# AWehenkel/Graphical-Normalizing-Flows

Hardware: NVIDIA B200
Metric: train_samples_per_s (higher is better)
Workload: dtype f32

## Files before the change

graphical-normalizing-flows_b200/_lib.py:

```python
import ctypes as C
import os

import torch

_HERE = os.path.dirname(os.path.abspath(__file__))
LIB_NAME = "libgnf_sm100.so"
LIB_PATH = os.path.join(_HERE, LIB_NAME)

GNF_MAX_LAYERS = 8
GATE_TABLE, GATE_GUMBEL, GATE_NOISER = 0, 1, 2
IMP_RAW, IMP_SOFT, IMP_HARD_SOFT, IMP_HARD_SQ = 0, 1, 2, 3

_lib = None
_SIMULATOR = False


class GateT(C.Structure):
    _fields_ = [("mode", C.c_int32), ("temperature", C.c_float), ("seed", C.c_uint64), ("offset", C.c_uint64),
                ("noise1", C.c_void_p), ("noise2", C.c_void_p), ("offset_dev", C.c_void_p)]


class MlpT(C.Structure):
    _fields_ = [("n_layers", C.c_int32), ("dims", C.c_int32 * (GNF_MAX_LAYERS + 1)),
                ("W", C.c_void_p * GNF_MAX_LAYERS), ("b", C.c_void_p * GNF_MAX_LAYERS)]


class AdamTensorT(C.Structure):
    _fields_ = [("param", C.c_void_p), ("grad", C.c_void_p), ("exp_avg", C.c_void_p), ("exp_avg_sq", C.c_void_p),
                ("numel", C.c_int64)]


class MlpGradT(C.Structure):
    _fields_ = [("dW", C.c_void_p * GNF_MAX_LAYERS), ("db", C.c_void_p * GNF_MAX_LAYERS)]


_P, _I, _F, _SZ = C.c_void_p, C.c_int, C.c_float, C.c_size_t

_PROTOS = {
    "gnf_version": ([], C.c_int),
    "gnf_last_error": ([], C.c_char_p),
    "gnf_has_device_code": ([], C.c_int),
    "gnf_affine_fwd": ([_P, _P, _I, _P, _P, _P, _P, _P, _I, _I, _P], C.c_int),
    "gnf_affine_bwd": ([_P, _P, _I, _P, _P, _P, _P, _P, _P, _P, _I, _I, _P], C.c_int),
    "gnf_normal_ll_fwd": ([_P, _P, _P, _I, _I, _P], C.c_int),
    "gnf_normal_ll_bwd": ([_P, _P, _P, _I, _I, _P], C.c_int),
    "gnf_power_trace_workspace_bytes": ([_I], _SZ),
    "gnf_power_trace_fwd": ([_P, _I, _F, _I, _P, _P, _SZ, _P], C.c_int),
    "gnf_power_trace_bwd": ([_P, _I, _F, _I, _P, _P, _P, _SZ, _P], C.c_int),
    "gnf_power_trace_fwd_save": ([_P, _I, _F, _I, _P, _P, _P], C.c_int),
    "gnf_power_trace_bwd_saved": ([_P, _P, _I, _F, _I, _P, _P, _P], C.c_int),
    "gnf_linear_fwd": ([_P, _I, _P, _I, _P, _I, _P, _I, _I, _I, _I, _I, _P], C.c_int),
    "gnf_linear_dgrad": ([_P, _I, _P, _I, _P, _I, _P, _I, _I, _I, _I, _P], C.c_int),
    "gnf_linear_wgrad": ([_P, _I, _P, _I, _P, _I, _I, _I, _I, _P], C.c_int),
    "gnf_linear_fwd_tc": ([_P, _I, _P, _I, _P, _I, _P, _I, _I, _I, _I, _I, _I, _P], C.c_int),
    "gnf_linear_dgrad_tc": ([_P, _I, _P, _I, _P, _I, _P, _I, _I, _I, _I, _I, _P], C.c_int),
    "gnf_linear_wgrad_tc": ([_P, _I, _P, _I, _P, _I, _I, _I, _I, _I, _P], C.c_int),
    "gnf_linear_wgrad_bias_tc": ([_P, _I, _P, _I, _P, _I, _P, _I, _I, _I, _P], C.c_int),
    "gnf_split_tf32": ([_P, _I, _P, _P, _I, _I, _I, _P], C.c_int),
    "gnf_linear_fwd_tc_ps": ([_P, _I, _P, _P, _I, _P, _I, _P, _I, _I, _I, _I, _I, _P], C.c_int),
    "gnf_linear_dgrad_tc_ps": ([_P, _I, _P, _P, _I, _P, _I, _P, _I, _I, _I, _I, _P], C.c_int),
    "gnf_colsum": ([_P, _I, _P, _I, _I, _I, _P], C.c_int),
    "gnf_pack_rows": ([_P, _P, _P, _P, _I, _I, _P], C.c_int),
    "gnf_unpack_rows": ([_P, _P, _P, _P, _I, _I, _I, _P], C.c_int),
    "gnf_unpack_vec": ([_P, _P, _P, _I, _I, _P], C.c_int),
    "gnf_dag_importance": ([_P, _I, _I, _F, _P, _P, _P], C.c_int),
    "gnf_dag_bias_table": ([_P, _I, _P, _P, _I, _I, _I, _P], C.c_int),
    "gnf_dag_bias_table_bwd": ([_P, _P, _I, _P, _I, _I, _I, _P], C.c_int),
    "gnf_dag_l1_fwd": ([_P, _P, C.POINTER(GateT), _P, _I, _P, _I, _P, _I, _I, _I, _I, _I, _P], C.c_int),
    "gnf_dag_l1_wgrad": ([_P, _I, _P, _P, C.POINTER(GateT), _P, _I, _I, _I, _I, _P], C.c_int),
    "gnf_dag_l1_dgrad": ([_P, _I, _P, _I, _P, _P, C.POINTER(GateT), _P, _P, _I, _I, _I, _P], C.c_int),
    "gnf_dag_l1_fwd_save": ([_P, _P, C.POINTER(GateT), _P, _I, _P, _I, _P, _I, _P, _P, _P, _I, _I, _I, _I, _P], C.c_int),
    "gnf_dag_l1_wgrad_saved": ([_P, _I, _P, _P, _I, _I, _I, _I, _P], C.c_int),
    "gnf_dag_l1_dgrad_saved": ([_P, _I, _P, _I, _P, _P, _P, _P, _I, _I, _I, _P], C.c_int),
    "gnf_linear_fwd_splitk_workspace_bytes": ([_I, _I, _I], _SZ),
    "gnf_linear_fwd_splitk": ([_P, _I, _P, _I, _P, _P, _I, _I, _I, _I, _I, _P, _SZ, _P], C.c_int),
    "gnf_dag_bias_table_ld": ([_P, _I, _P, _P, _I, _I, _I, _I, _P], C.c_int),
    "gnf_linear_fwd_tc_ps_tb": ([_P, _I, _P, _P, _I, _P, _I, _I, _P, _I, _I, _I, _I, _I, _P], C.c_int),
    "gnf_dag_gate_planes": ([_P, _P, C.POINTER(GateT), _P, _P, _P, _I, _I, _P], C.c_int),
    "gnf_dag_l1_reduce_saved": ([_P, _P, _P, _P, _P, _I, _I, _P], C.c_int),
    "gnf_nll_loss_work_floats": ([_I], _SZ),
    "gnf_nll_loss_fwd": ([_P, _P, _P, _P, _P, _I, _I, _P], C.c_int),
    "gnf_nll_loss_bwd": ([_P, _P, _P, _P, _I, _I, _P], C.c_int),
    "gnf_peer_alloc": ([_SZ, C.POINTER(C.c_void_p)], C.c_int),
    "gnf_peer_free": ([_P], C.c_int),
    "gnf_peer_export": ([_P, C.c_char_p], C.c_int),
    "gnf_peer_import": ([C.c_char_p, C.POINTER(C.c_void_p)], C.c_int),
    "gnf_peer_close": ([_P], C.c_int),
    "gnf_peer_flag_bytes": ([], _SZ),
    "gnf_peer_allreduce_avg": ([C.POINTER(C.c_void_p), C.POINTER(C.c_void_p), _I, _I, C.c_longlong, _P], C.c_int),
    "gnf_dag_embed_fwd": ([_P, _P, C.POINTER(GateT), _P, _P, _P, _I, _I, _I, _P], C.c_int),
    "gnf_dag_embed_bwd": ([_P, _I, _P, _P, C.POINTER(GateT), _P, _P, _P, _P, _I, _I, _P], C.c_int),
    "gnf_dag_finish_dA": ([_P, _P, _P, _I, _I, _P], C.c_int),
    "gnf_dag_dump_noise": ([C.POINTER(GateT), _P, _P, _I, _I, _P], C.c_int),
    "gnf_umnn_workspace_bytes": ([C.POINTER(MlpT)], _SZ),
    "gnf_umnn_saved_floats_per_node_row": ([C.POINTER(MlpT)], _SZ),
    "gnf_umnn_fwd": ([_P, _P, C.POINTER(MlpT), _I, _P, _P, _P, _P, _P, _P, _P, _I, _I, _P, _SZ, _P], C.c_int),
    "gnf_umnn_invert": ([_P, _P, C.POINTER(MlpT), _I, _P, _P, _P, _I, _F, _F, _I, _P, _SZ, _P], C.c_int),
    "gnf_umnn_bwd": ([_P, _P, C.POINTER(MlpT), _I, _P, _P, _P, _P, _P, _P, _P, _P, _P, _P, C.POINTER(MlpGradT), _I, _I,
                      _P, _SZ, _P], C.c_int),
    "gnf_umnn_tc_workspace_bytes": ([C.POINTER(MlpT)], _SZ),
    "gnf_umnn_fwd_tc": ([_P, _P, C.POINTER(MlpT), _I, _P, _P, _P, _P, _P, _P, _I, _I, _P, _SZ, _P], C.c_int),
    "gnf_umnn_lw_saved_floats": ([C.POINTER(MlpT), _I, _I, _I], _SZ),
    "gnf_umnn_lw_workspace_bytes": ([C.POINTER(MlpT), _I, _I, _I], _SZ),
    "gnf_umnn_fwd_lw": ([_P, _P, C.POINTER(MlpT), _I, _P, _P, _P, _P, _P, _P, _P, _I, _I, _I, _I, _P, _SZ, _P], C.c_int),
    "gnf_umnn_bwd_lw": ([_P, _P, C.POINTER(MlpT), _I, _P, _P, _P, _P, _P, _P, _P, _P, _P, _P, C.POINTER(MlpGradT), _I, _I, _I,
                         _P, _SZ, _P], C.c_int),
    "gnf_umnn_tc3_workspace_bytes": ([C.POINTER(MlpT), _I], _SZ),
    "gnf_umnn_tc3_saved_floats": ([C.POINTER(MlpT), _I, _I], _SZ),
    "gnf_umnn_bwd_tc3_workspace_bytes": ([C.POINTER(MlpT), _I, _I], _SZ),
    "gnf_umnn_bwd_tc3": ([_P, _P, C.POINTER(MlpT), _I, _P, _P, _P, _P, _P, _P, _P, _P, _P, _P, C.POINTER(MlpGradT), _I, _I,
                          _P, _SZ, _P], C.c_int),
    "gnf_umnn_fwd_tc3": ([_P, _P, C.POINTER(MlpT), _I, _P, _P, _P, _P, _P, _P, _P, _I, _I, _I, _I, _P, _SZ, _P], C.c_int),
    "gnf_linear_rw_workspace_bytes": ([_I, _I], _SZ),
    "gnf_linear_wgrad_rw_workspace_bytes": ([_I, _I], _SZ),
    "gnf_linear_wgrad_rw": ([_P, _I, _P, _I, _P, _I, _I, _I, _I, _I, _P, _SZ, _P], C.c_int),
    "gnf_linear_fwd_rw": ([_P, _I, _P, _I, _P, _P, _I, _P, _I, _I, _I, _I, _I, _P, _SZ, _P], C.c_int),
    "gnf_linear_dgrad_rw": ([_P, _I, _P, _I, _P, _I, _P, _P, _I, _I, _I, _I, _I, _P, _SZ, _P], C.c_int),
    "gnf_tc_gemm_plan": ([_I, _I, _I, _I, _I, _P, _P], C.c_int),
    "gnf_tc_selftest": ([_P, _P, _P, _I, _I, _I, _P], C.c_int),
    "gnf_reverse_cols": ([_P, _P, _I, _I, _P], C.c_int),
    "gnf_broadcast_rows": ([_P, _P, _I, _I, _I, _I, _P], C.c_int),
    "gnf_counter_add": ([_P, C.c_uint64, _P], C.c_int),
    "gnf_adam_step": ([C.POINTER(AdamTensorT), _I, _P, _F, _F, _F, _F, _F, _P], C.c_int),
    "gnf_dag_loss_fwd": ([_P, _I, _P, _P, _P, _P, _P, _P, _P], C.c_int),
    "gnf_dag_loss_bwd": ([_P, _I, _P, _P, _P, _P, _P, _P, _P, _P, _P], C.c_int),
}

EXPORTED_SYMBOLS = tuple(_PROTOS)


def _bind(lib):
    for name, (argtypes, restype) in _PROTOS.items():
        fn = getattr(lib, name)
        fn.argtypes = argtypes
        fn.restype = restype
    return lib


def load_library(path=LIB_PATH):
    if not os.path.isfile(path):
        raise RuntimeError(
            f"{LIB_NAME} not found at {path}: the CUDA library is the only backend of this package "
            f"(no CPU / eager fallback). Build it with `python -c 'import __graft_entry__ as g; g.build()'`.")
    return _bind(C.CDLL(path))


def lib():
    global _lib
    if _lib is None:
        _lib = load_library()
    return _lib


def check(rc):
    if rc != 0:
        msg = lib().gnf_last_error()
        raise RuntimeError(f"libgnf error {rc}: {msg.decode() if msg else '?'}")


def stream_ptr():
    if _SIMULATOR:
        return None
    return C.c_void_p(torch.cuda.current_stream().cuda_stream)


def ptr(t):
    if t is None:
        return None
    return C.c_void_p(t.data_ptr())


def require(t, name, dtype=torch.float32):
    if not isinstance(t, torch.Tensor):
        raise TypeError(f"{name}: expected a torch.Tensor, got {type(t).__name__}")
    if t.dtype != dtype:
        raise TypeError(f"{name}: expected dtype {dtype}, got {t.dtype}")
    if not _SIMULATOR and not t.is_cuda:
        raise TypeError(f"{name}: expected a CUDA tensor (this package has no CPU path)")
    if not t.is_contiguous():
        raise TypeError(f"{name}: expected a contiguous tensor")
    return t
```

graphical-normalizing-flows_b200/csrc/tc_umnn3.cu:

```cuda
#include "tc_common.cuh"

#ifndef GNF_EMU
namespace gnf {

constexpr int kU3Rows = 128;
constexpr int kU3Stages = 4;
constexpr int kU3StageBlock = 32 * 16;
constexpr int kU3PRows = 12;
constexpr int kU3MaxNodes = 256;

__device__ __forceinline__ uint32_t u3_rn_tf32(uint32_t u) { return (u + 0x1000u) & 0xffffe000u; }
__device__ __forceinline__ void u3_arrive(uint64_t* bar) {
  asm volatile("mbarrier.arrive.shared::cta.b64 _, [%0];" ::"r"(tc::smem_u32(bar)) : "memory");
}

struct U3Plan {
  int L, NP, E, N1;
  int kp[GNF_MAX_LAYERS], nch[GNF_MAX_LAYERS];
  size_t off_img[GNF_MAX_LAYERS];
  size_t chunk_floats, off_tail, image_floats, off_P, total_floats;
};

static int u3_plan(const gnf_mlp_t* net, int R, U3Plan* pl) {
  if (!net || net->n_layers < 3 || net->n_layers > GNF_MAX_LAYERS) return fail(GNF_ERR_UNSUPPORTED, "umnn tc3: integrand needs 3..%d linear layers", GNF_MAX_LAYERS);
  if (net->dims[net->n_layers] != 1) return fail(GNF_ERR_UNSUPPORTED, "umnn tc3: integrand output size must be 1");
  if (net->dims[0] < 2) return fail(GNF_ERR_UNSUPPORTED, "umnn tc3: needs at least one conditioning feature");
  const int L = net->n_layers - 1;
  int maxh = 0;
  for (int l = 1; l <= L; ++l) maxh = net->dims[l] > maxh ? net->dims[l] : maxh;
  const int NP = (maxh + 31) / 32 * 32;
  if (NP > 160) return fail(GNF_ERR_UNSUPPORTED, "umnn tc3: hidden width %d > 160 (A_hi + A_lo + D must fit 512 TMEM columns)", maxh);
  pl->L = L; pl->NP = NP; pl->E = net->dims[0] - 1; pl->N1 = net->dims[1];
  pl->chunk_floats = (size_t)2 * 8 * NP * 4;
  size_t off = 0;
  for (int l = 0; l < GNF_MAX_LAYERS; ++l) { pl->kp[l] = 0; pl->nch[l] = 0; pl->off_img[l] = 0; }
  for (int l = 1; l < L; ++l) {
    pl->kp[l] = (net->dims[l] + 7) / 8 * 8;
    pl->nch[l] = (pl->kp[l] + 31) / 32;
    pl->off_img[l] = off;
    off += (size_t)pl->nch[l] * pl->chunk_floats;
  }
  pl->off_tail = off;
  off += (size_t)(L + 1) * NP;
  pl->image_floats = off;
  pl->off_P = (off + 3) / 4 * 4;
  pl->total_floats = pl->off_P + (size_t)(R > 0 ? R : 0) * NP;
  return 0;
}

struct U3PackArgs {
  const float* W[GNF_MAX_LAYERS];
  const float* b[GNF_MAX_LAYERS];
  int dims[GNF_MAX_LAYERS + 1], nch[GNF_MAX_LAYERS];
  unsigned off_img[GNF_MAX_LAYERS], chunk_floats, off_tail, total;
  int L, NP;
};

__global__ void u3_pack_kernel(U3PackArgs a, float* __restrict__ img) {
  for (unsigned i = blockIdx.x * blockDim.x + threadIdx.x; i < a.total; i += gridDim.x * blockDim.x) {
    float out = 0.f;
    if (i >= a.off_tail) {
      const int e = (int)(i - a.off_tail), j = e / a.NP, n = e % a.NP;
      if (j < a.L - 1) { if (n < a.dims[j + 2]) out = a.b[j + 1][n]; }
      else if (j == a.L - 1) { if (n < a.dims[a.L]) out = a.W[a.L][n]; }
      else { if (n < a.dims[1]) out = a.W[0][(size_t)n * a.dims[0]]; }
    } else {
      int l = 1;
      while (l + 1 < a.L && i >= a.off_img[l + 1]) ++l;
      const unsigned e = i - a.off_img[l];
      const unsigned c = e / a.chunk_floats, e2 = e % a.chunk_floats;
      const unsigned half = 8u * a.NP * 4u;
      const unsigned part = e2 / half, e3 = e2 % half;
      const int k4 = (int)(e3 / (a.NP * 4u)), n = (int)((e3 / 4u) % a.NP), kk = (int)(e3 % 4u);
      const int k = (int)c * 32 + k4 * 4 + kk;
      float v = 0.f;
      if (n < a.dims[l + 1] && k < a.dims[l]) v = a.W[l][(size_t)n * a.dims[l] + k];
      const float hi = __uint_as_float(u3_rn_tf32(__float_as_uint(v)));
      out = part ? __uint_as_float(u3_rn_tf32(__float_as_uint(v - hi))) : hi;
    }
    img[i] = out;
  }
}

struct U3Params {
  const float *x, *h, *ccw, *ccn, *P, *image, *blast;
  float *z, *zrev, *jac, *logdet, *saved;
  int R, d, E, S, nodes, L, N1, train, order, p_smem, debug;
  long long Q;
  int kp[GNF_MAX_LAYERS], nch[GNF_MAX_LAYERS];
  unsigned off_img[GNF_MAX_LAYERS], off_tail, chunk_floats;
  long long* trace;
};

#ifdef GNF_DEVTOOLS
#define U3_STAMP(row) do { if (tr_on && tr_n < 256) p.trace[(row) * 256 + tr_n++] = clock64(); } while (0)
#else
#define U3_STAMP(row) do { } while (0)
#endif

template <int NB>
__global__ void __launch_bounds__((4 * NB + 2) * 32, 1) umnn_fwd_tc3_kernel(U3Params p) {
  using namespace tc;
  constexpr int NP = NB * 32;
  constexpr int EW = 4 * NB;
  constexpr int NT = (EW + 2) * 32;
  constexpr uint32_t kChunkBytes = 2u * 8u * NP * 16u;
  constexpr uint32_t kHalfBytes = 8u * NP * 16u;
  GNF_SMEM(float, smem);
  float* ring = smem;
  float* tail = ring + (size_t)kU3Stages * (kChunkBytes / 4);
  float* stage_all = tail + (GNF_MAX_LAYERS + 1) * NP;
  float* pbuf = stage_all + EW * kU3StageBlock;
  float* ypart = pbuf + 2 * kU3PRows * NP;
  float* red = ypart + NB * kU3Rows;
  float* ccs = red + kU3Rows;
  uint64_t* bars = reinterpret_cast<uint64_t*>(ccs + 2 * kU3MaxNodes);
  uint64_t* w_full = bars;
  uint64_t* w_empty = w_full + kU3Stages;
  uint64_t* a_full = w_empty + kU3Stages;
  uint64_t* a_free = a_full + NB;
  uint64_t* d_full = a_free + NB;
  uint64_t* d_empty = d_full + 1;
  uint64_t* p_full = d_empty + 1;
  uint64_t* p_empty = p_full + 2;
  uint32_t* tmem_slot = reinterpret_cast<uint32_t*>(p_empty + 2);
  const int tid = threadIdx.x, warp = tid >> 5, lane = tid & 31;

  if (warp == 0) tmem_alloc(tmem_slot, 512);
  if (tid == 32) {
    for (int s = 0; s < kU3Stages; ++s) { mbar_init(&w_full[s], 1); mbar_init(&w_empty[s], 1); }
    for (int c = 0; c < NB; ++c) { mbar_init(&a_full[c], 4); mbar_init(&a_free[c], 1); }
    mbar_init(d_full, 1);
    mbar_init(d_empty, EW);
    for (int b = 0; b < 2; ++b) { mbar_init(&p_full[b], 1); mbar_init(&p_empty[b], EW); }
    fence_mbar_init();
  }
  pdl_prologue_done();
  for (int i = tid; i < (p.L + 1) * NP; i += NT) tail[i] = __ldg(p.image + p.off_tail + i);
  for (int i = tid; i <= p.S; i += NT) { ccs[i] = __ldg(p.ccn + i); ccs[kU3MaxNodes + i] = __ldg(p.ccw + i); }
  fence_before_sync();
  __syncthreads();
  fence_after_sync();
  const uint32_t tmem_base = *tmem_slot;

  const int Q = (int)p.Q, nodes = p.nodes;
  const int ntiles = (Q + kU3Rows - 1) / kU3Rows;
  const int n_local = (ntiles > (int)blockIdx.x) ? (ntiles - (int)blockIdx.x + (int)gridDim.x - 1) / (int)gridDim.x : 0;
  const int L = p.L;
#ifdef GNF_DEVTOOLS
  int tr_n = 0;
  const bool tr_on = p.trace != nullptr && blockIdx.x == 0 && lane == 0 && (warp == 0 || warp == 4 * (NB - 1) || warp >= EW);
#endif

  if (warp == EW + 1) {
    if (lane == 0) {
      auto issue_P = [&](int tl) {
        const int q0 = ((int)blockIdx.x + tl * (int)gridDim.x) * kU3Rows;
        const int q1 = (q0 + kU3Rows - 1 < Q - 1) ? q0 + kU3Rows - 1 : Q - 1;
        const int r0 = q0 / nodes, r1 = q1 / nodes;
        const uint32_t bytes = (uint32_t)(r1 - r0 + 1) * NP * 4u;
        const int b = tl & 1;
        if (tl >= 2) mbar_wait(&p_empty[b], (uint32_t)(((tl >> 1) - 1) & 1));
        mbar_expect_tx(&p_full[b], bytes);
        bulk_g2s(pbuf + (size_t)b * kU3PRows * NP, p.P + (size_t)r0 * NP, bytes, &p_full[b]);
      };
      if (p.p_smem && n_local > 0) issue_P(0);
      int g = 0;
      for (int tl = 0; tl < n_local; ++tl) {
        if (p.p_smem && tl + 1 < n_local) issue_P(tl + 1);
        for (int l = 1; l < L; ++l) {
          const int nch = p.nch[l], nseq = p.order ? 2 * nch : nch, nk = p.kp[l] / 8;
          const char* src0 = reinterpret_cast<const char*>(p.image + p.off_img[l]);
          for (int i = 0; i < nseq; ++i, ++g) {
            const int c = i < nch ? i : i - nch;
            const bool want_lo = !(p.order && i >= nch);
            const int ks = (nk - c * 4 < 4) ? nk - c * 4 : 4;
            const uint32_t bytes = (uint32_t)ks * 2u * NP * 16u;
            const int s = g % kU3Stages;
            if (g >= kU3Stages) mbar_wait(&w_empty[s], (uint32_t)(((g / kU3Stages) - 1) & 1));
            char* dst = reinterpret_cast<char*>(ring) + (size_t)s * kChunkBytes;
            const char* src = src0 + (size_t)c * kChunkBytes;
            mbar_expect_tx(&w_full[s], want_lo ? 2u * bytes : bytes);
            bulk_g2s(dst, src, bytes, &w_full[s]);
            if (want_lo) bulk_g2s(dst + kHalfBytes, src + kHalfBytes, bytes, &w_full[s]);
            U3_STAMP(2);
          }
        }
      }
    }
  } else if (warp == EW) {
    constexpr uint32_t idesc = make_idesc_tf32(kU3Rows, NP);
    constexpr uint32_t dstep = (2u * NP * 16u) >> 4;
    const uint32_t tAhi = tmem_base, tAlo = tmem_base + NP, tD = tmem_base + 2 * NP;
    const uint32_t ring_addr = smem_u32(ring);
    int g = 0, it = 0;
    for (int tl = 0; tl < n_local; ++tl)
      for (int l = 1; l < L; ++l, ++it) {
        const int nch = p.nch[l], nseq = p.order ? 2 * nch : nch, nk = p.kp[l] / 8;
        const bool release_a = (l == L - 1) && (tl + 1 < n_local);
        if (it > 0) mbar_wait(d_empty, (uint32_t)((it - 1) & 1));
        U3_STAMP(0);
        uint32_t acc = 0u;
        for (int i = 0; i < nseq; ++i, ++g) {
          const int c = i < nch ? i : i - nch;
          const int kind = p.order ? (i < nch ? 0 : 1) : 2;
          const int ks = (nk - c * 4 < 4) ? nk - c * 4 : 4;
          const int s = g % kU3Stages;
          if (i < nch) mbar_wait(&a_full[c], (uint32_t)(it & 1));
          mbar_wait(&w_full[s], (uint32_t)((g / kU3Stages) & 1));
          fence_after_sync();
          U3_STAMP(0);
          const uint32_t base = ring_addr + (uint32_t)s * kChunkBytes;
          const uint64_t dhi = make_smem_desc(base, NP * 16u, 128u), dlo = make_smem_desc(base + kHalfBytes, NP * 16u, 128u);
          const uint32_t a0 = (uint32_t)c * 32u;
          if (kind != 1) {
#pragma unroll 4
            for (int kk = 0; kk < ks; ++kk) { mma_tf32_ts_w(tD, tAlo + a0 + kk * 8, dhi + (uint64_t)(dstep * kk), idesc, acc); acc = 1u; }
#pragma unroll 4
            for (int kk = 0; kk < ks; ++kk) mma_tf32_ts_w(tD, tAhi + a0 + kk * 8, dlo + (uint64_t)(dstep * kk), idesc, 1u);
          }
          if (kind != 0) {
#pragma unroll 4
            for (int kk = 0; kk < ks; ++kk) { mma_tf32_ts_w(tD, tAhi + a0 + kk * 8, dhi + (uint64_t)(dstep * kk), idesc, acc); acc = 1u; }
          }
          mma_commit_w(&w_empty[s]);
          if (release_a && kind != 0) mma_commit_w(&a_free[c]);
        }
        if (release_a)
          for (int c = nch; c < NB; ++c) mma_commit_w(&a_free[c]);
        mma_commit_w(d_full);
        U3_STAMP(0);
      }
  } else {
    const int quarter = warp & 3, ci = warp >> 2, c = ci * 32;
    const int t = quarter * 32 + lane;
    const uint32_t lane_sel = (uint32_t)(quarter * 32) << 16;
    const uint32_t tAhi = tmem_base + lane_sel + c, tAlo = tAhi + NP, tD = tAhi + 2 * NP;
    float* stage = stage_all + warp * kU3StageBlock;
    const float* bias = tail + c;
    const float* wlast = tail + (L - 1) * NP + c;
    const float* w0col = tail + L * NP + c;
    const float blast = __ldg(p.blast);
    const size_t plane = (size_t)Q * NP;
    float* ysave = p.saved ? p.saved + (size_t)L * plane : nullptr;
    uint32_t* bits = (p.saved && p.train && L > 1) ? reinterpret_cast<uint32_t*>(p.saved + (size_t)L * plane + Q) : nullptr;
#ifdef GNF_DEVTOOLS
    if (p.debug & 4) { bits = nullptr; ysave = nullptr; }
#endif
    const bool full_block = c + 32 <= p.N1;

    struct Row { int q, r, kn, r_first; float xv; };
    auto row_of = [&](int tl) {
      Row w;
      const int q0 = ((int)blockIdx.x + tl * (int)gridDim.x) * kU3Rows;
      w.q = q0 + t;
      const int qc = w.q < Q ? w.q : Q - 1;
      w.r = qc / nodes; w.kn = qc - w.r * nodes;
      w.r_first = q0 / nodes;
      w.xv = ldg_pinned(p.x + w.r);
      return w;
    };
    auto store_block = [&](float* dstplane, const uint32_t* v, int q_row) {
#ifdef GNF_DEVTOOLS
      if (p.debug & 2) return;
#endif
      const int sub = lane >> 2, piece = lane & 3;
      const int row0 = q_row - lane + sub;
#pragma unroll
      for (int hb = 0; hb < 2; ++hb) {
#pragma unroll
        for (int j4 = 0; j4 < 4; ++j4)
          *reinterpret_cast<uint4*>(stage + lane * 16 + 4 * (j4 ^ ((lane >> 1) & 3))) =
              make_uint4(v[16 * hb + 4 * j4], v[16 * hb + 4 * j4 + 1], v[16 * hb + 4 * j4 + 2], v[16 * hb + 4 * j4 + 3]);
        __syncwarp();
#pragma unroll
        for (int i = 0; i < 4; ++i) {
          const int Rr = 8 * i + sub;
          const uint4 o = *reinterpret_cast<const uint4*>(stage + Rr * 16 + 4 * (piece ^ ((Rr >> 1) & 3)));
#ifdef GNF_DEVTOOLS
          if (p.debug & 1) continue;
#endif
          if (row0 + 8 * i < Q) *reinterpret_cast<uint4*>(dstplane + (size_t)(row0 + 8 * i) * NP + c + 16 * hb + 4 * piece) = o;
        }
        __syncwarp();
      }
    };
    auto split_store = [&](const uint32_t* v) {
#pragma unroll
      for (int hb = 0; hb < 2; ++hb) {
        uint32_t hi[16], lo[16];
#pragma unroll
        for (int j = 0; j < 16; ++j) {
          hi[j] = u3_rn_tf32(v[16 * hb + j]);
          lo[j] = __float_as_uint(__uint_as_float(v[16 * hb + j]) - __uint_as_float(hi[j])) + 0x1000u;
        }
        tmem_st16p(tAhi + 16 * hb, hi);
        tmem_st16p(tAlo + 16 * hb, lo);
      }
    };
    auto mask_word = [&](const uint32_t* v) {
      uint32_t w = 0u;
#pragma unroll
      for (int j = 0; j < 32; ++j) w |= (v[j] != 0u ? 1u : 0u) << j;
      return w;
    };
    auto gen_a1 = [&](int tl, const Row& w) {
      const float tq = (w.kn <= p.S) ? (w.xv * (ccs[w.kn] + 1.f)) / 2.f : w.xv;
      const float* Prow;
      if (p.p_smem) {
        mbar_wait(&p_full[tl & 1], (uint32_t)((tl >> 1) & 1));
        Prow = pbuf + (size_t)(tl & 1) * kU3PRows * NP + (size_t)(w.r - w.r_first) * NP + c;
      } else {
        Prow = p.P + (size_t)w.r * NP + c;
      }
      uint32_t v[32];
#pragma unroll
      for (int j4 = 0; j4 < 8; ++j4) {
        const float4 pv = p.p_smem ? *reinterpret_cast<const float4*>(Prow + 4 * j4) : __ldg(reinterpret_cast<const float4*>(Prow + 4 * j4));
        const float4 w4 = *reinterpret_cast<const float4*>(w0col + 4 * j4);
        v[4 * j4 + 0] = __float_as_uint(fmaxf(fmaf(tq, w4.x, pv.x), 0.f));
        v[4 * j4 + 1] = __float_as_uint(fmaxf(fmaf(tq, w4.y, pv.y), 0.f));
        v[4 * j4 + 2] = __float_as_uint(fmaxf(fmaf(tq, w4.z, pv.z), 0.f));
        v[4 * j4 + 3] = __float_as_uint(fmaxf(fmaf(tq, w4.w, pv.w), 0.f));
      }
      if (!full_block) {
#pragma unroll
        for (int j = 0; j < 32; ++j) v[j] = (c + j < p.N1) ? v[j] : 0u;
      }
      split_store(v);
      tmem_wait_st();
      fence_before_sync();
      __syncwarp();
      if (lane == 0) {
        u3_arrive(&a_full[ci]);
        if (p.p_smem) u3_arrive(&p_empty[tl & 1]);
      }
      if (bits && w.q < Q) bits[(size_t)w.q * NB + ci] = mask_word(v);
      if (p.saved) store_block(p.saved, v, w.q);
    };

    Row cur = {0, 0, 0, 0, 0.f};
    if (n_local > 0) { cur = row_of(0); gen_a1(0, cur); }
    int it = 0;
    for (int tl = 0; tl < n_local; ++tl) {
      for (int l = 1; l < L; ++l, ++it) {
        const float* bl = bias + (l - 1) * NP;
        Row nxt = cur;
        const bool gen_next = (l == L - 1) && (tl + 1 < n_local);
        const bool gen_late = gen_next && ci >= p.nch[l] - 1;
        if (gen_next) nxt = row_of(tl + 1);
        if (gen_next && !gen_late) {
          mbar_wait(&a_free[ci], (uint32_t)(tl & 1));
          fence_after_sync();
          gen_a1(tl + 1, nxt);
        }
        mbar_wait(d_full, (uint32_t)(it & 1));
        fence_after_sync();
        U3_STAMP(warp == 0 ? 1 : 3);
        uint32_t v[32];
        tmem_ld32p(tD, v);
        tmem_wait_ld();
        fence_before_sync();
        __syncwarp();
        if (lane == 0) u3_arrive(d_empty);
        if (gen_late) {
          mbar_wait(&a_free[ci], (uint32_t)(tl & 1));
          fence_after_sync();
          gen_a1(tl + 1, nxt);
        }
        if (l < L - 1) {
#pragma unroll
          for (int j4 = 0; j4 < 32; j4 += 4) {
            const float4 b4 = *reinterpret_cast<const float4*>(bl + j4);
            v[j4 + 0] = __float_as_uint(fmaxf(__uint_as_float(v[j4 + 0]) + b4.x, 0.f));
            v[j4 + 1] = __float_as_uint(fmaxf(__uint_as_float(v[j4 + 1]) + b4.y, 0.f));
            v[j4 + 2] = __float_as_uint(fmaxf(__uint_as_float(v[j4 + 2]) + b4.z, 0.f));
            v[j4 + 3] = __float_as_uint(fmaxf(__uint_as_float(v[j4 + 3]) + b4.w, 0.f));
          }
          split_store(v);
          tmem_wait_st();
          fence_before_sync();
          __syncwarp();
          if (lane == 0) u3_arrive(&a_full[ci]);
          U3_STAMP(warp == 0 ? 1 : 3);
          if (bits && cur.q < Q) bits[(size_t)l * Q * NB + (size_t)cur.q * NB + ci] = mask_word(v);
          if (p.saved) store_block(p.saved + (size_t)l * plane, v, cur.q);
        } else {
          float y0 = 0.f, y1 = 0.f, y2 = 0.f, y3 = 0.f;
#pragma unroll
          for (int j4 = 0; j4 < 32; j4 += 4) {
            const float4 b4 = *reinterpret_cast<const float4*>(bl + j4);
            const float4 w4 = *reinterpret_cast<const float4*>(wlast + j4);
            const float a0 = fmaxf(__uint_as_float(v[j4 + 0]) + b4.x, 0.f), a1 = fmaxf(__uint_as_float(v[j4 + 1]) + b4.y, 0.f);
            const float a2 = fmaxf(__uint_as_float(v[j4 + 2]) + b4.z, 0.f), a3 = fmaxf(__uint_as_float(v[j4 + 3]) + b4.w, 0.f);
            y0 = fmaf(a0, w4.x, y0); y1 = fmaf(a1, w4.y, y1); y2 = fmaf(a2, w4.z, y2); y3 = fmaf(a3, w4.w, y3);
            v[j4 + 0] = __float_as_uint(a0); v[j4 + 1] = __float_as_uint(a1); v[j4 + 2] = __float_as_uint(a2); v[j4 + 3] = __float_as_uint(a3);
          }
          ypart[ci * kU3Rows + t] = (y0 + y1) + (y2 + y3);
          if (bits && cur.q < Q) bits[(size_t)l * Q * NB + (size_t)cur.q * NB + ci] = mask_word(v);
          if (p.saved) store_block(p.saved + (size_t)l * plane, v, cur.q);
          named_bar_sync(1, EW * 32);
          const bool cur_valid = cur.q < Q;
          if (ci == 0) {
            float y = blast;
#pragma unroll
            for (int k = 0; k < NB; ++k) y += ypart[k * kU3Rows + t];
            const float f = (y > 0.f ? y : expm1f(y)) + 1.05f;
            float wv = 0.f;
            if (cur_valid) {
              if (ysave) ysave[cur.q] = y;
              if (cur.kn <= p.S) wv = ccs[kU3MaxNodes + cur.kn] * f;
              if (cur.kn == 0) {
                p.jac[cur.r] = f;
                if (p.logdet) atomicAdd(p.logdet + cur.r / p.d, logf(f));
              }
            }
            red[t] = wv;
          }
          named_bar_sync(1, EW * 32);
          if (ci == 0 && cur_valid && (cur.kn == 0 || t == 0)) {
            float sacc = 0.f;
            int rem = nodes - cur.kn;
            if (rem > kU3Rows - t) rem = kU3Rows - t;
            for (int k = 0; k < rem; ++k) sacc += red[t + k];
            float cz = sacc * cur.xv / 2.f;
            if (cur.kn == 0) cz += __ldg(p.h + (size_t)cur.r * p.E);
            atomicAdd(p.z + cur.r, cz);
            if (p.zrev) { const int b = cur.r / p.d, ii = cur.r % p.d; atomicAdd(p.zrev + (size_t)b * p.d + (p.d - 1 - ii), cz); }
          }
          U3_STAMP(warp == 0 ? 1 : 3);
        }
        cur = nxt;
      }
    }
  }
  fence_before_sync();
  __syncthreads();
  if (warp == 0) tmem_dealloc(tmem_base, 512);
}

struct U3BParams {
  const float *x, *ccw, *ccn, *jac, *gz, *gzrev, *gjac, *glogdet, *image, *saved;
  float* dplanes;
  float *D, *dx, *dW0;
  float* db[GNF_MAX_LAYERS];
  int R, d, E, S, nodes, L, ldw0;
  long long Q;
  int dims[GNF_MAX_LAYERS + 1];
  int kp[GNF_MAX_LAYERS], nch[GNF_MAX_LAYERS];
  unsigned off_img[GNF_MAX_LAYERS], off_tail, chunk_floats;
};

__device__ __forceinline__ float u3_colsum16(float (&w)[16], int lane) {
#pragma unroll
  for (int i = 0; i < 16; ++i) w[i] += __shfl_xor_sync(0xffffffffu, w[i], 16);
#pragma unroll
  for (int o = 8; o >= 1; o >>= 1) {
    const bool up = (lane & o) != 0;
#pragma unroll
    for (int i = 0; i < o; ++i) {
      const float send = up ? w[i] : w[i + o];
      const float keep = up ? w[i + o] : w[i];
      w[i] = keep + __shfl_xor_sync(0xffffffffu, send, o);
    }
  }
  return w[0];
}

template <int NB>
__global__ void __launch_bounds__((4 * NB + 2) * 32, 1) umnn_bwd_tc3_kernel(U3BParams p) {
  using namespace tc;
  constexpr int NP = NB * 32;
  constexpr int EW = 4 * NB;
  constexpr int NT = (EW + 2) * 32;
  constexpr uint32_t kChunkBytes = 2u * 8u * NP * 16u;
  constexpr uint32_t kHalfBytes = 8u * NP * 16u;
  GNF_SMEM(float, smem);
  float* ring = smem;
  float* tail = ring + (size_t)kU3Stages * (kChunkBytes / 4);
  float* stage_all = tail + 2 * NP;
  float* ccs = stage_all + EW * kU3StageBlock;
  uint64_t* bars = reinterpret_cast<uint64_t*>(ccs + 2 * kU3MaxNodes);
  uint64_t* w_full = bars;
  uint64_t* w_empty = w_full + kU3Stages;
  uint64_t* a_full = w_empty + kU3Stages;
  uint64_t* a_free = a_full + NB;
  uint64_t* d_full = a_free + NB;
  uint64_t* d_empty = d_full + 1;
  uint32_t* tmem_slot = reinterpret_cast<uint32_t*>(d_empty + 1);
  const int tid = threadIdx.x, warp = tid >> 5, lane = tid & 31;

  if (warp == 0) tmem_alloc(tmem_slot, 512);
  if (tid == 32) {
    for (int s = 0; s < kU3Stages; ++s) { mbar_init(&w_full[s], 1); mbar_init(&w_empty[s], 1); }
    for (int c = 0; c < NB; ++c) { mbar_init(&a_full[c], 4); mbar_init(&a_free[c], 1); }
    mbar_init(d_full, 1);
    mbar_init(d_empty, EW);
    fence_mbar_init();
  }
  pdl_prologue_done();
  for (int i = tid; i < 2 * NP; i += NT) tail[i] = __ldg(p.image + p.off_tail + i);
  for (int i = tid; i <= p.S; i += NT) { ccs[i] = __ldg(p.ccn + i); ccs[kU3MaxNodes + i] = __ldg(p.ccw + i); }
  fence_before_sync();
  __syncthreads();
  fence_after_sync();
  const uint32_t tmem_base = *tmem_slot;

  const int Q = (int)p.Q, nodes = p.nodes;
  const int ntiles = (Q + kU3Rows - 1) / kU3Rows;
  const int n_local = (ntiles > (int)blockIdx.x) ? (ntiles - (int)blockIdx.x + (int)gridDim.x - 1) / (int)gridDim.x : 0;
  const int L = p.L;

  if (warp == EW + 1) {
    if (lane == 0) {
      int g = 0;
      for (int tl = 0; tl < n_local; ++tl)
        for (int l = L - 1; l >= 1; --l) {
          const int nch = p.nch[l], nk = p.kp[l] / 8;
          const char* src0 = reinterpret_cast<const char*>(p.image + p.off_img[l]);
          for (int i = 0; i < 2 * nch; ++i, ++g) {
            const int c = i < nch ? i : i - nch;
            const bool want_lo = i < nch;
            const int ks = (nk - c * 4 < 4) ? nk - c * 4 : 4;
            const uint32_t bytes = (uint32_t)ks * 2u * NP * 16u;
            const int s = g % kU3Stages;
            if (g >= kU3Stages) mbar_wait(&w_empty[s], (uint32_t)(((g / kU3Stages) - 1) & 1));
            char* dst = reinterpret_cast<char*>(ring) + (size_t)s * kChunkBytes;
            const char* src = src0 + (size_t)c * kChunkBytes;
            mbar_expect_tx(&w_full[s], want_lo ? 2u * bytes : bytes);
            bulk_g2s(dst, src, bytes, &w_full[s]);
            if (want_lo) bulk_g2s(dst + kHalfBytes, src + kHalfBytes, bytes, &w_full[s]);
          }
        }
    }
  } else if (warp == EW) {
    constexpr uint32_t idesc = make_idesc_tf32(kU3Rows, NP);
    constexpr uint32_t dstep = (2u * NP * 16u) >> 4;
    const uint32_t tAhi = tmem_base, tAlo = tmem_base + NP, tD = tmem_base + 2 * NP;
    const uint32_t ring_addr = smem_u32(ring);
    int g = 0, it = 0;
    for (int tl = 0; tl < n_local; ++tl)
      for (int l = L - 1; l >= 1; --l, ++it) {
        const int nch = p.nch[l], nk = p.kp[l] / 8;
        const bool release_a = (l == 1) && (tl + 1 < n_local);
        if (it > 0) mbar_wait(d_empty, (uint32_t)((it - 1) & 1));
        uint32_t acc = 0u;
        for (int i = 0; i < 2 * nch; ++i, ++g) {
          const int c = i < nch ? i : i - nch;
          const bool corr = i < nch;
          const int ks = (nk - c * 4 < 4) ? nk - c * 4 : 4;
          const int s = g % kU3Stages;
          if (corr) mbar_wait(&a_full[c], (uint32_t)(it & 1));
          mbar_wait(&w_full[s], (uint32_t)((g / kU3Stages) & 1));
          fence_after_sync();
          const uint32_t base = ring_addr + (uint32_t)s * kChunkBytes;
          const uint64_t dhi = make_smem_desc(base, NP * 16u, 128u), dlo = make_smem_desc(base + kHalfBytes, NP * 16u, 128u);
          const uint32_t a0 = (uint32_t)c * 32u;
          if (corr) {
#pragma unroll 4
            for (int kk = 0; kk < ks; ++kk) { mma_tf32_ts_w(tD, tAlo + a0 + kk * 8, dhi + (uint64_t)(dstep * kk), idesc, acc); acc = 1u; }
#pragma unroll 4
            for (int kk = 0; kk < ks; ++kk) mma_tf32_ts_w(tD, tAhi + a0 + kk * 8, dlo + (uint64_t)(dstep * kk), idesc, 1u);
          } else {
#pragma unroll 4
            for (int kk = 0; kk < ks; ++kk) mma_tf32_ts_w(tD, tAhi + a0 + kk * 8, dhi + (uint64_t)(dstep * kk), idesc, 1u);
          }
          mma_commit_w(&w_empty[s]);
          if (release_a && !corr) mma_commit_w(&a_free[c]);
        }
        if (release_a)
          for (int c = nch; c < NB; ++c) mma_commit_w(&a_free[c]);
        mma_commit_w(d_full);
      }
  } else {
    const int quarter = warp & 3, ci = warp >> 2, c = ci * 32;
    const int t = quarter * 32 + lane;
    const uint32_t lane_sel = (uint32_t)(quarter * 32) << 16;
    const uint32_t tAhi = tmem_base + lane_sel + c, tAlo = tAhi + NP, tD = tAhi + 2 * NP;
    float* stage = stage_all + warp * kU3StageBlock;
    const float* wL = tail + c;
    const float* w0col = tail + NP + c;
    const size_t plane = (size_t)Q * NP;
    const float* ysave = p.saved + (size_t)L * plane;
    const uint32_t* bits = reinterpret_cast<const uint32_t*>(p.saved + (size_t)L * plane + Q);
    const size_t bplane = (size_t)Q * NB;

    struct Row { int q, r, kn; float gq, tq, jg; uint32_t mtop; };
    auto row_of = [&](int tl) {
      Row w;
      const int q0 = ((int)blockIdx.x + tl * (int)gridDim.x) * kU3Rows;
      w.q = q0 + t;
      const bool valid = w.q < Q;
      const int qc = valid ? w.q : Q - 1;
      w.r = qc / nodes; w.kn = qc - w.r * nodes;
      const int r = w.r;
      const float xv = ldg_pinned(p.x + r);
      float gzt = p.gz ? ldg_pinned(p.gz + r) : 0.f;
      if (p.gzrev) { const int b = r / p.d, i = r - b * p.d; gzt += ldg_pinned(p.gzrev + (size_t)b * p.d + (p.d - 1 - i)); }
      const float y = ldg_pinned(ysave + qc);
      float gq;
      if (w.kn <= p.S) {
        gq = (gzt * xv / 2.f) * ccs[kU3MaxNodes + w.kn];
        w.tq = (xv * (ccs[w.kn] + 1.f)) / 2.f;
      } else {
        gq = p.gjac ? ldg_pinned(p.gjac + r) : 0.f;
        if (p.glogdet) gq += ldg_pinned(p.glogdet + r / p.d) / ldg_pinned(p.jac + r);
        w.tq = xv;
      }
      gq *= (y > 0.f) ? 1.f : expf(y);
      w.gq = valid ? gq : 0.f;
      w.jg = ldg_pinned(p.jac + r) * gzt;
      w.mtop = valid ? __ldg(bits + (size_t)(L - 1) * bplane + (size_t)qc * NB + ci) : 0u;
      return w;
    };
    auto store_block = [&](float* dstplane, const uint32_t* v, int q_row) {
      const int sub = lane >> 2, piece = lane & 3;
      const int row0 = q_row - lane + sub;
#pragma unroll
      for (int hb = 0; hb < 2; ++hb) {
#pragma unroll
        for (int j4 = 0; j4 < 4; ++j4)
          *reinterpret_cast<uint4*>(stage + lane * 16 + 4 * (j4 ^ ((lane >> 1) & 3))) =
              make_uint4(v[16 * hb + 4 * j4], v[16 * hb + 4 * j4 + 1], v[16 * hb + 4 * j4 + 2], v[16 * hb + 4 * j4 + 3]);
        __syncwarp();
#pragma unroll
        for (int i = 0; i < 4; ++i) {
          const int Rr = 8 * i + sub;
          const uint4 o = *reinterpret_cast<const uint4*>(stage + Rr * 16 + 4 * (piece ^ ((Rr >> 1) & 3)));
          if (row0 + 8 * i < Q) *reinterpret_cast<uint4*>(dstplane + (size_t)(row0 + 8 * i) * NP + c + 16 * hb + 4 * piece) = o;
        }
        __syncwarp();
      }
    };
    auto split_store = [&](const uint32_t* v) {
#pragma unroll
      for (int hb = 0; hb < 2; ++hb) {
        uint32_t hi[16], lo[16];
#pragma unroll
        for (int j = 0; j < 16; ++j) {
          hi[j] = u3_rn_tf32(v[16 * hb + j]);
          lo[j] = __float_as_uint(__uint_as_float(v[16 * hb + j]) - __uint_as_float(hi[j])) + 0x1000u;
        }
        tmem_st16p(tAhi + 16 * hb, hi);
        tmem_st16p(tAlo + 16 * hb, lo);
      }
    };
    auto gen_top = [&](const Row& w) {
      uint32_t v[32];
#pragma unroll
      for (int j4 = 0; j4 < 8; ++j4) {
        const float4 w4 = *reinterpret_cast<const float4*>(wL + 4 * j4);
        v[4 * j4 + 0] = ((w.mtop >> (4 * j4 + 0)) & 1u) ? __float_as_uint(w.gq * w4.x) : 0u;
        v[4 * j4 + 1] = ((w.mtop >> (4 * j4 + 1)) & 1u) ? __float_as_uint(w.gq * w4.y) : 0u;
        v[4 * j4 + 2] = ((w.mtop >> (4 * j4 + 2)) & 1u) ? __float_as_uint(w.gq * w4.z) : 0u;
        v[4 * j4 + 3] = ((w.mtop >> (4 * j4 + 3)) & 1u) ? __float_as_uint(w.gq * w4.w) : 0u;
      }
      split_store(v);
      tmem_wait_st();
      fence_before_sync();
      __syncwarp();
      if (lane == 0) u3_arrive(&a_full[ci]);
    };

    Row cur;
    cur.q = 0; cur.r = 0; cur.kn = 0; cur.gq = 0.f; cur.tq = 0.f; cur.jg = 0.f; cur.mtop = 0u;
    if (n_local > 0) { cur = row_of(0); gen_top(cur); }
    int it = 0;
    for (int tl = 0; tl < n_local; ++tl) {
      for (int l = L - 1; l >= 1; --l, ++it) {
        Row nxt = cur;
        const bool gen_next = (l == 1) && (tl + 1 < n_local);
        const bool gen_late = gen_next && ci >= p.nch[l] - 1;
        const bool valid = cur.q < Q;
        const uint32_t m = valid ? __ldg(bits + (size_t)(l - 1) * bplane + (size_t)cur.q * NB + ci) : 0u;
        if (gen_next) nxt = row_of(tl + 1);
        if (gen_next && !gen_late) {
          mbar_wait(&a_free[ci], (uint32_t)(tl & 1));
          fence_after_sync();
          gen_top(nxt);
        }
        mbar_wait(d_full, (uint32_t)(it & 1));
        fence_after_sync();
        uint32_t v[32];
        tmem_ld32p(tD, v);
        tmem_wait_ld();
        fence_before_sync();
        __syncwarp();
        if (lane == 0) u3_arrive(d_empty);
        if (gen_late) {
          mbar_wait(&a_free[ci], (uint32_t)(tl & 1));
          fence_after_sync();
          gen_top(nxt);
        }
#pragma unroll
        for (int j = 0; j < 32; ++j) v[j] = ((m >> j) & 1u) ? v[j] : 0u;
        if (l > 1) {
          split_store(v);
          tmem_wait_st();
          fence_before_sync();
          __syncwarp();
          if (lane == 0) u3_arrive(&a_full[ci]);
#pragma unroll
          for (int hb = 0; hb < 2; ++hb) {
            float w16[16];
#pragma unroll
            for (int j = 0; j < 16; ++j) w16[j] = __uint_as_float(v[16 * hb + j]);
            const float sum = u3_colsum16(w16, lane);
            const int n = c + 16 * hb + (lane & 15);
            if (lane < 16 && n < p.dims[l]) atomicAdd(p.db[l - 1] + n, sum);
          }
          store_block(p.dplanes + (size_t)(L - 1 - l) * plane, v, cur.q);
        } else {
          float dot = 0.f;
#pragma unroll
          for (int j4 = 0; j4 < 8; ++j4) {
            const float4 w4 = *reinterpret_cast<const float4*>(w0col + 4 * j4);
            dot = fmaf(__uint_as_float(v[4 * j4 + 0]), w4.x, dot); dot = fmaf(__uint_as_float(v[4 * j4 + 1]), w4.y, dot);
            dot = fmaf(__uint_as_float(v[4 * j4 + 2]), w4.z, dot); dot = fmaf(__uint_as_float(v[4 * j4 + 3]), w4.w, dot);
          }
          if (valid && cur.kn == p.S + 1) atomicAdd(p.dx + cur.r, dot + (ci == 0 ? cur.jg : 0.f));
          const int r_lo = __shfl_sync(0xffffffffu, cur.r, 0), r_hi = __shfl_sync(0xffffffffu, cur.r, 31);
#pragma unroll
          for (int hb = 0; hb < 2; ++hb) {
            const int n = c + 16 * hb + (lane & 15);
            const bool col_ok = lane < 16 && n < p.dims[1];
            float w16[16];
#pragma unroll
            for (int j = 0; j < 16; ++j) w16[j] = __uint_as_float(v[16 * hb + j]) * cur.tq;
            const float st = u3_colsum16(w16, lane);
            if (col_ok) atomicAdd(p.dW0 + (size_t)n * p.ldw0, st);
            for (int rr = r_lo; rr <= r_hi; ++rr) {
#pragma unroll
              for (int j = 0; j < 16; ++j) w16[j] = (cur.r == rr) ? __uint_as_float(v[16 * hb + j]) : 0.f;
              const float sd = u3_colsum16(w16, lane);
              if (col_ok) atomicAdd(p.D + (size_t)rr * NP + n, sd);
            }
          }
        }
        cur = nxt;
      }
    }
  }
  fence_before_sync();
  __syncthreads();
  if (warp == 0) tmem_dealloc(tmem_base, 512);
}

static size_t u3b_smem_bytes(int NP) {
  const int NB = NP / 32, EW = 4 * NB;
  return ((size_t)kU3Stages * 2 * 8 * NP * 4 + (size_t)2 * NP + (size_t)EW * kU3StageBlock + 2 * kU3MaxNodes) * sizeof(float) +
         (2 * kU3Stages + 2 * NB + 2) * sizeof(uint64_t) + 16;
}

struct U3BPlan {
  int L, NP;
  int kp[GNF_MAX_LAYERS], nch[GNF_MAX_LAYERS];
  size_t off_img[GNF_MAX_LAYERS], chunk_floats, off_tail, image_floats;
};
static int u3b_plan(const gnf_mlp_t* net, U3BPlan* pl) {
  U3Plan f;
  if (int e = u3_plan(net, 0, &f)) return e;
  pl->L = f.L; pl->NP = f.NP; pl->chunk_floats = f.chunk_floats;
  size_t off = 0;
  for (int l = 0; l < GNF_MAX_LAYERS; ++l) { pl->kp[l] = 0; pl->nch[l] = 0; pl->off_img[l] = 0; }
  for (int l = 1; l < f.L; ++l) {
    pl->kp[l] = (net->dims[l + 1] + 7) / 8 * 8;
    pl->nch[l] = (pl->kp[l] + 31) / 32;
    pl->off_img[l] = off;
    off += (size_t)pl->nch[l] * pl->chunk_floats;
  }
  pl->off_tail = off;
  pl->image_floats = off + (size_t)2 * f.NP;
  return 0;
}

__global__ void u3_pack_bwd_kernel(U3PackArgs a, float* __restrict__ img) {
  for (unsigned i = blockIdx.x * blockDim.x + threadIdx.x; i < a.total; i += gridDim.x * blockDim.x) {
    float out = 0.f;
    if (i >= a.off_tail) {
      const int e = (int)(i - a.off_tail), j = e / a.NP, n = e % a.NP;
      if (j == 0) { if (n < a.dims[a.L]) out = a.W[a.L][n]; }
      else { if (n < a.dims[1]) out = a.W[0][(size_t)n * a.dims[0]]; }
    } else {
      int l = 1;
      while (l + 1 < a.L && i >= a.off_img[l + 1]) ++l;
      const unsigned e = i - a.off_img[l];
      const unsigned c = e / a.chunk_floats, e2 = e % a.chunk_floats;
      const unsigned half = 8u * a.NP * 4u;
      const unsigned part = e2 / half, e3 = e2 % half;
      const int k4 = (int)(e3 / (a.NP * 4u)), n = (int)((e3 / 4u) % a.NP), kk = (int)(e3 % 4u);
      const int k = (int)c * 32 + k4 * 4 + kk;
      float v = 0.f;
      if (n < a.dims[l] && k < a.dims[l + 1]) v = a.W[l][(size_t)k * a.dims[l] + n];
      const float hi = __uint_as_float(u3_rn_tf32(__float_as_uint(v)));
      out = part ? __uint_as_float(u3_rn_tf32(__float_as_uint(v - hi))) : hi;
    }
    img[i] = out;
  }
}

size_t u3_bwd_image_floats(const gnf_mlp_t* net) {
  U3BPlan pl;
  if (u3b_plan(net, &pl)) return 0;
  return (pl.image_floats + 3) / 4 * 4;
}

int launch_u3_bwd_chain(const float* x, const gnf_mlp_t* net, int S, const float* ccw, const float* ccn, const float* jac, const float* gz,
                        const float* gzrev, const float* gjac, const float* glogdet, const float* saved, float* image, float* dplanes, float* D,
                        float* dx, const gnf_mlp_grad_t* grads, int R, int d, cudaStream_t s, const Branches* br, int side, cudaStream_t pack_stream) {
  U3BPlan pl;
  if (int e = u3b_plan(net, &pl)) return e;
  const int NP = pl.NP, L = pl.L;
  const int nodes = S + 2;
  const long long Q = (long long)R * nodes;
  if (Q > 0x7fffffffLL - 2 * kU3Rows || S + 1 > kU3MaxNodes) return fail(GNF_ERR_UNSUPPORTED, "umnn tc3 backward: problem size out of range");
  U3PackArgs a;
  for (int l = 0; l < GNF_MAX_LAYERS; ++l) { a.W[l] = nullptr; a.b[l] = nullptr; a.nch[l] = pl.nch[l]; a.off_img[l] = (unsigned)pl.off_img[l]; }
  for (int l = 0; l <= L; ++l) { a.W[l] = net->W[l]; a.b[l] = net->b[l]; }
  for (int l = 0; l <= net->n_layers; ++l) a.dims[l] = net->dims[l];
  a.chunk_floats = (unsigned)pl.chunk_floats; a.off_tail = (unsigned)pl.off_tail; a.total = (unsigned)pl.image_floats; a.L = L; a.NP = NP;
  int blocks = (int)((pl.image_floats + 255) / 256);
  if (blocks > 2 * kNumSMs) blocks = 2 * kNumSMs;
  GNF_LAUNCH(u3_pack_bwd_kernel, blocks, 256, 0, (br && pack_stream) ? pack_stream : s, a, image);
  if (br && pack_stream) br->end(s, side);
  U3BParams p;
  p.x = x; p.ccw = ccw; p.ccn = ccn; p.jac = jac; p.gz = gz; p.gzrev = gzrev; p.gjac = gjac; p.glogdet = glogdet; p.image = image; p.saved = saved;
  p.dplanes = dplanes; p.D = D; p.dx = dx; p.dW0 = grads->dW[0]; p.ldw0 = net->dims[0];
  for (int l = 0; l < GNF_MAX_LAYERS; ++l) p.db[l] = grads->db[l];
  p.R = R; p.d = d; p.E = net->dims[0] - 1; p.S = S; p.nodes = nodes; p.L = L; p.Q = Q;
  for (int l = 0; l <= GNF_MAX_LAYERS; ++l) p.dims[l] = l <= net->n_layers ? net->dims[l] : 0;
  for (int l = 0; l < GNF_MAX_LAYERS; ++l) { p.kp[l] = pl.kp[l]; p.nch[l] = pl.nch[l]; p.off_img[l] = (unsigned)pl.off_img[l]; }
  p.off_tail = (unsigned)pl.off_tail; p.chunk_floats = (unsigned)pl.chunk_floats;
  const size_t smem = u3b_smem_bytes(NP);
  const long long ntiles = (Q + kU3Rows - 1) / kU3Rows;
  const int grid = (int)(ntiles < kNumSMs ? ntiles : kNumSMs);
#define U3B_CASE(nb)                                                                                             \
  case nb:                                                                                                       \
    cudaFuncSetAttribute(umnn_bwd_tc3_kernel<nb>, cudaFuncAttributeMaxDynamicSharedMemorySize, (int)smem);       \
    GNF_LAUNCH_PDL(umnn_bwd_tc3_kernel<nb>, grid, (4 * nb + 2) * 32, smem, s, p);                                    \
    break;
  switch (NP / 32) { U3B_CASE(1) U3B_CASE(2) U3B_CASE(3) U3B_CASE(4) U3B_CASE(5) default: return fail(GNF_ERR_UNSUPPORTED, "umnn tc3 backward: width"); }
#undef U3B_CASE
  return 0;
}

static size_t u3_smem_bytes(int NP) {
  const int NB = NP / 32, EW = 4 * NB;
  return ((size_t)kU3Stages * 2 * 8 * NP * 4 + (size_t)(GNF_MAX_LAYERS + 1) * NP + (size_t)EW * kU3StageBlock + (size_t)2 * kU3PRows * NP +
          (size_t)(NB + 1) * kU3Rows + 2 * kU3MaxNodes) * sizeof(float) + (2 * kU3Stages + 2 * NB + 6) * sizeof(uint64_t) + 16;
}

#ifdef GNF_DEVTOOLS
static long long* g_u3_trace = nullptr;
static int g_u3_debug = 0;
#endif

}
using namespace gnf;
#endif

extern "C" {

size_t gnf_umnn_tc3_workspace_bytes(const gnf_mlp_t* net, int R) {
#ifdef GNF_EMU
  (void)net; (void)R;
  gnf::set_error("tensor-core kernels have no host-simulator flavour");
  return 0;
#else
  U3Plan pl;
  if (u3_plan(net, R, &pl)) return 0;
  return pl.total_floats * sizeof(float);
#endif
}

int gnf_umnn_fwd_tc3(const float* x, const float* h, const gnf_mlp_t* net, int S, const float* ccw, const float* ccn, float* z,
                     float* zrev, float* jac, float* logdet, float* saved, int train, int order, int R, int d, void* work,
                     size_t work_bytes, gnf_stream_t stream) {
#ifdef GNF_EMU
  return gnf::fail(GNF_ERR_UNSUPPORTED, "tensor-core kernels have no host-simulator flavour");
#else
  if (!x || !h || !net || !ccw || !ccn || !z || !jac || R < 0 || d <= 0 || S < 1 || (R % d) != 0) return fail(GNF_ERR_INVALID, "gnf_umnn_fwd_tc3: bad arguments");
  if (train && !saved) return fail(GNF_ERR_INVALID, "gnf_umnn_fwd_tc3: training needs the saved-activation buffer");
  U3Plan pl;
  if (int e = u3_plan(net, R, &pl)) return e;
  if (!work || work_bytes < pl.total_floats * sizeof(float)) return fail(GNF_ERR_WORKSPACE, "gnf_umnn_fwd_tc3: workspace too small (%zu < %zu)", work_bytes, pl.total_floats * sizeof(float));
  if ((reinterpret_cast<uintptr_t>(work) & 15) != 0 || (saved && (reinterpret_cast<uintptr_t>(saved) & 15) != 0)) return fail(GNF_ERR_INVALID, "gnf_umnn_fwd_tc3: workspace / saved must be 16-byte aligned");
  const int nodes = S + 1 + (train ? 1 : 0);
  const long long Q = (long long)R * nodes;
  if (Q > 0x7fffffffLL - 2 * kU3Rows) return fail(GNF_ERR_UNSUPPORTED, "gnf_umnn_fwd_tc3: %lld node-rows exceed the index range", Q);
  if (S + 1 > kU3MaxNodes) return fail(GNF_ERR_UNSUPPORTED, "gnf_umnn_fwd_tc3: more than %d quadrature nodes", kU3MaxNodes);
  cudaStream_t s = (cudaStream_t)stream;
  if (R == 0) return 0;
  float* ws = (float*)work;
  const int NP = pl.NP, L = pl.L, E = pl.E;
  U3PackArgs a;
  for (int l = 0; l < GNF_MAX_LAYERS; ++l) { a.W[l] = nullptr; a.b[l] = nullptr; a.nch[l] = pl.nch[l]; a.off_img[l] = (unsigned)pl.off_img[l]; }
  for (int l = 0; l <= L; ++l) { a.W[l] = net->W[l]; a.b[l] = net->b[l]; }
  for (int l = 0; l <= net->n_layers; ++l) a.dims[l] = net->dims[l];
  a.chunk_floats = (unsigned)pl.chunk_floats; a.off_tail = (unsigned)pl.off_tail; a.total = (unsigned)pl.image_floats; a.L = L; a.NP = NP;
  int blocks = (int)((pl.image_floats + 255) / 256);
  if (blocks > 2 * kNumSMs) blocks = 2 * kNumSMs;
  const Branches& br = branches();
  cudaStream_t s0 = br.begin(s, 0);
  GNF_LAUNCH(u3_pack_kernel, blocks, 256, 0, s0, a, ws);
  ZeroList zl;
  zl.add(z, (size_t)R);
  zl.add(zrev, (size_t)R);
  zl.add(logdet, (size_t)(R / d));
  zero_many(zl, s0);
  float* P = ws + pl.off_P;
  if (int e = gnf_linear_fwd(h, E, net->W[0] + 1, 1 + E, net->b[0], 1, P, NP, R, net->dims[1], E, 0, stream)) return e;
  br.end(s, 0);
  U3Params p;
  p.x = x; p.h = h; p.ccw = ccw; p.ccn = ccn; p.P = P; p.image = ws; p.blast = net->b[L];
  p.z = z; p.zrev = zrev; p.jac = jac; p.logdet = logdet; p.saved = saved;
  p.R = R; p.d = d; p.E = E; p.S = S; p.nodes = nodes; p.L = L; p.N1 = pl.N1; p.train = train; p.order = order ? 1 : 0;
  p.Q = Q;
  p.p_smem = ((kU3Rows - 1) / nodes + 2 <= kU3PRows) ? 1 : 0;
  for (int l = 0; l < GNF_MAX_LAYERS; ++l) { p.kp[l] = pl.kp[l]; p.nch[l] = pl.nch[l]; p.off_img[l] = (unsigned)pl.off_img[l]; }
  p.off_tail = (unsigned)pl.off_tail; p.chunk_floats = (unsigned)pl.chunk_floats;
#ifdef GNF_DEVTOOLS
  p.trace = g_u3_trace; p.debug = g_u3_debug;
#else
  p.trace = nullptr; p.debug = 0;
#endif
  const size_t smem = u3_smem_bytes(NP);
  const long long ntiles = (Q + kU3Rows - 1) / kU3Rows;
  const int grid = (int)(ntiles < kNumSMs ? ntiles : kNumSMs);
#define U3_CASE(nb)                                                                                              \
  case nb:                                                                                                       \
    cudaFuncSetAttribute(umnn_fwd_tc3_kernel<nb>, cudaFuncAttributeMaxDynamicSharedMemorySize, (int)smem);       \
    GNF_LAUNCH_PDL(umnn_fwd_tc3_kernel<nb>, grid, (4 * nb + 2) * 32, smem, s, p);                                           \
    break;
  switch (NP / 32) { U3_CASE(1) U3_CASE(2) U3_CASE(3) U3_CASE(4) U3_CASE(5) default: return fail(GNF_ERR_UNSUPPORTED, "gnf_umnn_fwd_tc3: width"); }
#undef U3_CASE
  return check_launch("gnf_umnn_fwd_tc3");
#endif
}

#ifdef GNF_DEVTOOLS
int gnf_umnn_tc3_set_trace(long long* buf) {
#ifndef GNF_EMU
  gnf::g_u3_trace = buf;
#else
  (void)buf;
#endif
  return 0;
}
int gnf_umnn_tc3_set_debug(int bits) {
#ifndef GNF_EMU
  gnf::g_u3_debug = bits;
#else
  (void)bits;
#endif
  return 0;
}
#endif

}
```

graphical-normalizing-flows_b200/csrc/tc_umnn3.h:

```cpp
#pragma once
#include "common.cuh"

#ifndef GNF_EMU
namespace gnf {
size_t u3_bwd_image_floats(const gnf_mlp_t* net);
int launch_u3_bwd_chain(const float* x, const gnf_mlp_t* net, int S, const float* ccw, const float* ccn, const float* jac, const float* gz,
                        const float* gzrev, const float* gjac, const float* glogdet, const float* saved, float* image, float* dplanes, float* D,
                        float* dx, const gnf_mlp_grad_t* grads, int R, int d, cudaStream_t s, const Branches* br = nullptr, int side = 0,
                        cudaStream_t pack_stream = nullptr);
}
#endif
```

graphical-normalizing-flows_b200/csrc/umnn_lw.cu:

```cuda
#include "common.cuh"
#include "tc_gemm.h"
#include "tc_rw.h"
#include "tc_umnn3.h"

namespace gnf {

constexpr int kLwRL = 8;
constexpr int kOutBwdU = 3;

struct LwGeom {
  int R, d, E, S, nodes, NP, L;
  long long Q;
};

__device__ __forceinline__ float lw_node_abscissa(float xv, const float* __restrict__ ccn, int kn, int S) {
  return (kn <= S) ? (xv * (__ldg(ccn + kn) + 1.f)) / 2.f : xv;
}

__global__ void lw_pad_weight_kernel(const float* __restrict__ W, int N, int K, float* __restrict__ Wp, int NP, int rows) {
  const int total = rows * NP;
  for (int i = blockIdx.x * blockDim.x + threadIdx.x; i < total; i += gridDim.x * blockDim.x) {
    const int n = i / NP, k = i % NP;
    Wp[i] = (n < N && k < K) ? W[(size_t)n * K + k] : 0.f;
  }
}

__global__ void lw_layer1_fwd_kernel(const float* __restrict__ x, const float* __restrict__ ccn, const float* __restrict__ P,
                                     const float* __restrict__ W0, int ldw0, int N1, float* __restrict__ a1,
                                     uint32_t* __restrict__ bits, LwGeom g) {
  const int C4 = g.NP / 4;
  const int c4 = threadIdx.x % C4, rl = threadIdx.x / C4, c = 4 * c4;
  float w[4];
#pragma unroll
  for (int e = 0; e < 4; ++e) w[e] = (c + e < N1) ? __ldg(W0 + (size_t)(c + e) * ldw0) : 0.f;
  const int Q = (int)g.Q;
  for (int q0 = blockIdx.x * kLwRL; q0 < Q; q0 += gridDim.x * kLwRL) {
    const int q = q0 + rl;
    const bool valid = q < Q;
    float4 o = make_float4(0.f, 0.f, 0.f, 0.f);
    if (valid) {
      const int r = q / g.nodes, kn = q - r * g.nodes;
      const float t = lw_node_abscissa(__ldg(x + r), ccn, kn, g.S);
      const float4 pv = __ldg(reinterpret_cast<const float4*>(P + (size_t)r * g.NP + c));
      o.x = (c + 0 < N1) ? fmaxf(fmaf(t, w[0], pv.x), 0.f) : 0.f;
      o.y = (c + 1 < N1) ? fmaxf(fmaf(t, w[1], pv.y), 0.f) : 0.f;
      o.z = (c + 2 < N1) ? fmaxf(fmaf(t, w[2], pv.z), 0.f) : 0.f;
      o.w = (c + 3 < N1) ? fmaxf(fmaf(t, w[3], pv.w), 0.f) : 0.f;
      *reinterpret_cast<float4*>(a1 + (size_t)q * g.NP + c) = o;
    }
    if (bits) {
      uint32_t wv = ((o.x > 0.f ? 1u : 0u) | (o.y > 0.f ? 2u : 0u) | (o.z > 0.f ? 4u : 0u) | (o.w > 0.f ? 8u : 0u)) << (4 * (threadIdx.x & 7));
      wv |= __shfl_xor_sync(0xffffffffu, wv, 1);
      wv |= __shfl_xor_sync(0xffffffffu, wv, 2);
      wv |= __shfl_xor_sync(0xffffffffu, wv, 4);
      if (valid && (threadIdx.x & 7) == 0) bits[(size_t)q * (g.NP / 32) + (c >> 5)] = wv;
    }
  }
}

template <int J>
__global__ void __launch_bounds__(256, 4) lw_out_fwd_kernel(const float* __restrict__ aL, const float* __restrict__ wl, const float* __restrict__ bl,
                                                             int NL, const float* __restrict__ x, const float* __restrict__ h,
                                                             const float* __restrict__ ccw, float* __restrict__ z, float* __restrict__ zrev,
                                                             float* __restrict__ jac, float* __restrict__ logdet, float* __restrict__ ysave,
                                                             LwGeom g) {
  const int lane = threadIdx.x & 31, grp = lane >> 3, sub = lane & 7;
  float4 w[J];
#pragma unroll
  for (int j = 0; j < J; ++j) {
    const int c = (j * 8 + sub) * 4;
    w[j].x = (c + 0 < NL) ? __ldg(wl + c + 0) : 0.f;
    w[j].y = (c + 1 < NL) ? __ldg(wl + c + 1) : 0.f;
    w[j].z = (c + 2 < NL) ? __ldg(wl + c + 2) : 0.f;
    w[j].w = (c + 3 < NL) ? __ldg(wl + c + 3) : 0.f;
  }
  const float blast = __ldg(bl);
  const int wpb = blockDim.x >> 5;
  for (int r = blockIdx.x * wpb + (threadIdx.x >> 5); r < g.R; r += gridDim.x * wpb) {
    const float xv = __ldg(x + r);
    float s = 0.f;
    for (int kn0 = 0; kn0 < g.nodes; kn0 += 4) {
      const int kn = kn0 + grp;
      const bool valid = kn < g.nodes;
      const long long q = (long long)r * g.nodes + kn;
      float4 v[J];
      if (valid) {
        const float4* row = reinterpret_cast<const float4*>(aL + (size_t)q * g.NP) + sub;
#pragma unroll
        for (int j = 0; j < J; ++j) v[j] = __ldg(row + 8 * j);
      } else {
#pragma unroll
        for (int j = 0; j < J; ++j) v[j] = make_float4(0.f, 0.f, 0.f, 0.f);
      }
      float acc = 0.f;
#pragma unroll
      for (int j = 0; j < J; ++j) {
        const int c = (j * 8 + sub) * 4;
        if (c + 0 < NL) acc = fmaf(v[j].x, w[j].x, acc);
        if (c + 1 < NL) acc = fmaf(v[j].y, w[j].y, acc);
        if (c + 2 < NL) acc = fmaf(v[j].z, w[j].z, acc);
        if (c + 3 < NL) acc = fmaf(v[j].w, w[j].w, acc);
      }
      acc += __shfl_xor_sync(0xffffffffu, acc, 1);
      acc += __shfl_xor_sync(0xffffffffu, acc, 2);
      acc += __shfl_xor_sync(0xffffffffu, acc, 4);
      if (valid && sub == 0) {
        const float y = acc + blast;
        const float f = (y > 0.f ? y : expm1f(y)) + 1.05f;
        if (ysave) ysave[q] = y;
        if (kn <= g.S) s = fmaf(__ldg(ccw + kn), f, s);
        if (kn == 0) {
          jac[r] = f;
          if (logdet) atomicAdd(logdet + r / g.d, logf(f));
        }
      }
    }
    s += __shfl_xor_sync(0xffffffffu, s, 8);
    s += __shfl_xor_sync(0xffffffffu, s, 16);
    if (lane == 0) {
      const float zv = s * xv / 2.f + __ldg(h + (size_t)r * g.E);
      z[r] = zv;
      if (zrev) { const int b = r / g.d, i = r % g.d; zrev[(size_t)b * g.d + (g.d - 1 - i)] = zv; }
    }
  }
}

__device__ __forceinline__ float lw_gz_total(const float* __restrict__ gz, const float* __restrict__ gzrev, int r, int d) {
  float v = gz ? __ldg(gz + r) : 0.f;
  if (gzrev) { const int b = r / d, i = r % d; v += __ldg(gzrev + (size_t)b * d + (d - 1 - i)); }
  return v;
}

__global__ void lw_out_bwd_kernel(const float* __restrict__ aL, const float* __restrict__ ysave, const float* __restrict__ wl, int NL,
                                  const float* __restrict__ x, const float* __restrict__ ccw, const float* __restrict__ jac,
                                  const float* __restrict__ gz, const float* __restrict__ gzrev, const float* __restrict__ gjac,
                                  const float* __restrict__ glogdet, float* __restrict__ dL, float* __restrict__ gq_out, float* __restrict__ dWl,
                                  float* __restrict__ dbl, float* __restrict__ dbprev, LwGeom g) {
  GNF_SMEM(float, red);
  const int C4 = g.NP / 4;
  const int c4 = threadIdx.x % C4, rl = threadIdx.x / C4, c = 4 * c4;
  float w[4], sW[4] = {0.f, 0.f, 0.f, 0.f}, sB[4] = {0.f, 0.f, 0.f, 0.f}, sy = 0.f;
#pragma unroll
  for (int e = 0; e < 4; ++e) w[e] = (c + e < NL) ? __ldg(wl + c + e) : 0.f;
  const int Q = (int)g.Q;
  const int per = (Q + gridDim.x - 1) / gridDim.x;
  const int q0 = blockIdx.x * per;
  const int q1 = (q0 + per < Q) ? q0 + per : Q;
  int q = q0 + rl;
  int r = q / g.nodes, kn = q - r * g.nodes;
  const int dr = kLwRL / g.nodes, dk = kLwRL - dr * g.nodes;
  for (; q < q1; q += kOutBwdU * kLwRL) {
    int rr[kOutBwdU], kk[kOutBwdU];
    float4 av[kOutBwdU];
    float ys[kOutBwdU];
    bool ok[kOutBwdU];
#pragma unroll
    for (int u = 0; u < kOutBwdU; ++u) {
      rr[u] = r; kk[u] = kn;
      ok[u] = q + u * kLwRL < q1;
      const int qq = ok[u] ? q + u * kLwRL : q;
      av[u] = __ldg(reinterpret_cast<const float4*>(aL + (size_t)qq * g.NP + c));
      ys[u] = __ldg(ysave + qq);
      r += dr; kn += dk;
      if (kn >= g.nodes) { kn -= g.nodes; ++r; }
    }
#pragma unroll
    for (int u = 0; u < kOutBwdU; ++u) {
      if (!ok[u]) continue;
      const int ru = rr[u];
      float gq;
      if (kk[u] <= g.S) {
        gq = (lw_gz_total(gz, gzrev, ru, g.d) * __ldg(x + ru) / 2.f) * __ldg(ccw + kk[u]);
      } else {
        gq = gjac ? __ldg(gjac + ru) : 0.f;
        if (glogdet) gq += __ldg(glogdet + ru / g.d) / __ldg(jac + ru);
      }
      const float y = ys[u];
      gq *= (y > 0.f) ? 1.f : expf(y);
      const float a[4] = {c + 0 < NL ? av[u].x : 0.f, c + 1 < NL ? av[u].y : 0.f, c + 2 < NL ? av[u].z : 0.f, c + 3 < NL ? av[u].w : 0.f};
      float o[4];
#pragma unroll
      for (int e = 0; e < 4; ++e) {
        sW[e] = fmaf(gq, a[e], sW[e]);
        o[e] = a[e] > 0.f ? gq * w[e] : 0.f;
        sB[e] += o[e];
      }
      if (gq_out) { if (c4 == 0) gq_out[q + u * kLwRL] = gq; }
      else *reinterpret_cast<float4*>(dL + (size_t)(q + u * kLwRL) * g.NP + c) = make_float4(o[0], o[1], o[2], o[3]);
      if (c4 == 0) sy += gq;
    }
  }
  float* ry = red + kLwRL * g.NP;
  for (int pass = 0; pass < 2; ++pass) {
    const float* src = pass == 0 ? sW : sB;
#pragma unroll
    for (int e = 0; e < 4; ++e) red[rl * g.NP + c + e] = src[e];
    if (pass == 0 && c4 == 0) ry[rl] = sy;
    __syncthreads();
    if (rl == 0) {
      float* dst = pass == 0 ? dWl : dbprev;
#pragma unroll
      for (int e = 0; e < 4; ++e) {
        if (c + e < NL) {
          float s = 0.f;
          for (int k = 0; k < kLwRL; ++k) s += red[k * g.NP + c + e];
          atomicAdd(dst + c + e, s);
        }
      }
      if (pass == 0 && c4 == 0) {
        float s = 0.f;
        for (int k = 0; k < kLwRL; ++k) s += ry[k];
        atomicAdd(dbl, s);
      }
    }
    __syncthreads();
  }
}

__global__ void lw_layer1_bwd_kernel(const float* __restrict__ d1, const float* __restrict__ x, const float* __restrict__ ccn,
                                     const float* __restrict__ W0, int ldw0, int N1, const float* __restrict__ jac,
                                     const float* __restrict__ gz, const float* __restrict__ gzrev, float* __restrict__ D,
                                     float* __restrict__ dW0, float* __restrict__ db0, float* __restrict__ dx, LwGeom g) {
  GNF_SMEM(float, red);
  const int C4 = g.NP / 4;
  const int c4 = threadIdx.x % C4, rl = threadIdx.x / C4, c = 4 * c4;
  float w[4], sT[4] = {0.f, 0.f, 0.f, 0.f}, sD[4] = {0.f, 0.f, 0.f, 0.f};
#pragma unroll
  for (int e = 0; e < 4; ++e) w[e] = (c + e < N1) ? __ldg(W0 + (size_t)(c + e) * ldw0) : 0.f;
  const bool m0 = c + 0 < N1, m1 = c + 1 < N1, m2 = c + 2 < N1, m3 = c + 3 < N1;
  const int per = ((g.R + gridDim.x - 1) / gridDim.x + kLwRL - 1) / kLwRL * kLwRL;
  const int r0 = blockIdx.x * per, r1 = (r0 + per < g.R) ? r0 + per : g.R;
  int it = 0;
  for (int rb = r0; rb < r1; rb += kLwRL, ++it) {
    const int r = rb + rl;
    const bool valid = r < r1;
    float dot = 0.f;
    if (valid) {
      const float xv = __ldg(x + r);
      const float* row = d1 + (size_t)r * g.nodes * g.NP + c;
      float Dp[4] = {0.f, 0.f, 0.f, 0.f};
      for (int kn0 = 0; kn0 < g.nodes; kn0 += 4) {
        float4 dv[4];
#pragma unroll
        for (int u = 0; u < 4; ++u) {
          const int kn = (kn0 + u < g.nodes) ? kn0 + u : g.nodes - 1;
          dv[u] = __ldg(reinterpret_cast<const float4*>(row + (size_t)kn * g.NP));
        }
#pragma unroll
        for (int u = 0; u < 4; ++u) {
          const int kn = kn0 + u;
          if (kn < g.nodes) {
            const float t = lw_node_abscissa(xv, ccn, kn, g.S);
            const float v[4] = {m0 ? dv[u].x : 0.f, m1 ? dv[u].y : 0.f, m2 ? dv[u].z : 0.f, m3 ? dv[u].w : 0.f};
#pragma unroll
            for (int e = 0; e < 4; ++e) { Dp[e] += v[e]; sT[e] = fmaf(v[e], t, sT[e]); }
            if (kn == g.S + 1) dot = (v[0] * w[0] + v[1] * w[1]) + (v[2] * w[2] + v[3] * w[3]);
          }
        }
      }
#pragma unroll
      for (int e = 0; e < 4; ++e) sD[e] += Dp[e];
      *reinterpret_cast<float4*>(D + (size_t)r * g.NP + c) = make_float4(Dp[0], Dp[1], Dp[2], Dp[3]);
    }
    float* part = red + (it & 1) * (kLwRL * C4);
    part[rl * C4 + c4] = dot;
    __syncthreads();
    if (valid && c4 == 0) {
      float s = 0.f;
      for (int k = 0; k < C4; ++k) s += part[rl * C4 + k];
      dx[r] = s + __ldg(jac + r) * lw_gz_total(gz, gzrev, r, g.d);
    }
  }
  for (int pass = 0; pass < 2; ++pass) {
    __syncthreads();
    const float* src = pass == 0 ? sT : sD;
#pragma unroll
    for (int e = 0; e < 4; ++e) red[rl * g.NP + c + e] = src[e];
    __syncthreads();
    if (rl == 0) {
#pragma unroll
      for (int e = 0; e < 4; ++e) {
        if (c + e < N1) {
          float s = 0.f;
          for (int k = 0; k < kLwRL; ++k) s += red[k * g.NP + c + e];
          if (pass == 0) atomicAdd(dW0 + (size_t)(c + e) * ldw0, s);
          else atomicAdd(db0 + c + e, s);
        }
      }
    }
  }
}

__global__ void lw_finish_dh_kernel(float* __restrict__ dh, int E, const float* __restrict__ gz, const float* __restrict__ gzrev, int R, int d) {
  for (int r = blockIdx.x * blockDim.x + threadIdx.x; r < R; r += gridDim.x * blockDim.x) dh[(size_t)r * E] += lw_gz_total(gz, gzrev, r, d);
}

static int g_lw_use_rw_wgrad = 1;
static int g_lw_use_rw = 1;

struct LwPlan {
  int L, NP, E, nodes;
  int rw;
  long long Q;
  size_t off_P, off_Wp[GNF_MAX_LAYERS], off_dA, off_dB, off_D, off_part, total;
};

static int lw_plan(const gnf_mlp_t* net, int R, int S, int train, int backward, LwPlan* pl) {
  if (!net || net->n_layers < 2 || net->n_layers > GNF_MAX_LAYERS) return fail(GNF_ERR_UNSUPPORTED, "umnn (layer-wise): integrand needs 2..%d linear layers", GNF_MAX_LAYERS);
  if (net->dims[net->n_layers] != 1) return fail(GNF_ERR_UNSUPPORTED, "umnn (layer-wise): integrand output size must be 1");
  if (net->dims[0] < 2) return fail(GNF_ERR_UNSUPPORTED, "umnn (layer-wise): needs at least one conditioning feature");
  if (R < 0 || S < 1) return fail(GNF_ERR_INVALID, "umnn (layer-wise): bad R / S");
  const int L = net->n_layers - 1;
  int maxh = 0;
  for (int l = 1; l <= L; ++l) maxh = net->dims[l] > maxh ? net->dims[l] : maxh;
  if (maxh < 1 || maxh > 256) return fail(GNF_ERR_UNSUPPORTED, "umnn (layer-wise): hidden widths must be in 1..256 (got %d)", maxh);
  pl->L = L;
  pl->NP = (maxh + 31) / 32 * 32;
  pl->E = net->dims[0] - 1;
  pl->nodes = S + 1 + (train ? 1 : 0);
  pl->Q = (long long)R * pl->nodes;
  if (pl->Q > 0x7fffffffLL) return fail(GNF_ERR_UNSUPPORTED, "umnn (layer-wise): %lld node-rows exceed the GEMM engine's row index range", pl->Q);
  size_t off = 0;
  const size_t plane = (size_t)pl->Q * pl->NP;
  pl->off_P = off; off += (size_t)R * pl->NP;
  pl->off_D = pl->off_P;
#ifdef GNF_EMU
  pl->rw = 0;
#else
  pl->rw = 1;
  for (int l = 1; l < L; ++l)
    if (!rw_supported(net->dims[l + 1], net->dims[l]) || !rw_supported(net->dims[l], net->dims[l + 1])) pl->rw = 0;
#endif
  for (int l = 1; l < L; ++l) { pl->off_Wp[l] = off; off += (size_t)2 * pl->NP * pl->NP + pl->NP; }
  pl->off_dA = pl->off_dB = 0;
  pl->off_part = 0;
  if (backward) {
    pl->off_dA = off; off += plane;
    pl->off_dB = off; off += plane;
#ifndef GNF_EMU
    if (pl->rw) { pl->off_part = off; off += rw_wgrad_partial_floats(pl->NP); }
#endif
  }
  pl->total = off;
  return 0;
}

static inline int lw_blocks(long long work_items, int per_block, int max_per_sm) {
  long long b = (work_items + per_block - 1) / per_block;
  const long long cap = (long long)kNumSMs * max_per_sm;
  if (b > cap) b = cap;
  return b < 1 ? 1 : (int)b;
}

static int lw_fwd_gemm(const float* X, int ldx, const float* W, int ldw, const float* bias, float* Y, int ldy, int M, int N, int K,
                       int relu, uint32_t* bits_out, int bits_ld, int passes, int rw_np, cudaStream_t s) {
  if (passes == 0) return gnf_linear_fwd(X, ldx, W, ldw, bias, 1, Y, ldy, M, N, K, relu, (gnf_stream_t)s);
#ifdef GNF_EMU
  return fail(GNF_ERR_UNSUPPORTED, "tensor-core kernels have no host-simulator flavour");
#else
  if (rw_np) {
    RwGemmParams r = {};
    r.A = X; r.lda = ldx; r.C = Y; r.ldc = ldy; r.image = W;
    r.M = M; r.NP = rw_np; r.KP = (K + 7) / 8 * 8; r.passes = passes; r.epi = RW_EPI_BIAS_ACT; r.relu = relu;
    r.bits_out = bits_out; r.bits_ld = bits_ld;
    if (int e = launch_rw_gemm(r, s)) return e;
    return check_launch("gnf_umnn_fwd_lw (resident-weight GEMM)");
  }
  TcGemmParams p = {};
  p.A = X; p.lda = ldx; p.a_src = TCG_SRC_K;
  p.B = W; p.ldb = ldw; p.b_src = TCG_SRC_K;
  p.M = M; p.N = N; p.K = K; p.passes = passes;
  p.epi = TCG_EPI_BIAS_ACT; p.C = Y; p.ldc = ldy; p.bias = bias; p.bias_ld = N; p.bias_period = 1; p.relu = relu;
  p.bits_out = bits_out; p.bits_ld = bits_ld;
  if (int e = launch_tc_gemm(p, s)) return e;
  return check_launch("gnf_umnn_fwd_lw (GEMM)");
#endif
}
static int lw_dgrad_gemm(const float* dY, int lddy, const float* W, int ldw, const float* act, int ldact, const uint32_t* mask_bits,
                         int mask_ld, float* dX, int lddx, int M, int N, int K, int passes, int rw_np, cudaStream_t s) {
  if (passes == 0) return gnf_linear_dgrad(dY, lddy, W, ldw, act, ldact, dX, lddx, M, N, K, (gnf_stream_t)s);
#ifdef GNF_EMU
  return fail(GNF_ERR_UNSUPPORTED, "tensor-core kernels have no host-simulator flavour");
#else
  if (rw_np) {
    RwGemmParams r = {};
    r.A = dY; r.lda = lddy; r.C = dX; r.ldc = lddx; r.image = W;
    r.M = M; r.NP = rw_np; r.KP = (N + 7) / 8 * 8; r.passes = passes; r.epi = RW_EPI_MASK;
    r.mask_bits = mask_bits; r.mask_ld = mask_ld; r.act = act; r.ldact = ldact;
    if (int e = launch_rw_gemm(r, s)) return e;
    return check_launch("gnf_umnn_bwd_lw (resident-weight GEMM)");
  }
  TcGemmParams p = {};
  p.A = dY; p.lda = lddy; p.a_src = TCG_SRC_K;
  p.B = W; p.ldb = ldw; p.b_src = TCG_SRC_MN;
  p.M = M; p.N = K; p.K = N; p.passes = passes;
  p.epi = TCG_EPI_MASK; p.C = dX; p.ldc = lddx; p.act = act; p.ldact = ldact; p.mask_bits = mask_bits; p.mask_ld = mask_ld;
  if (int e = launch_tc_gemm(p, s)) return e;
  return check_launch("gnf_umnn_bwd_lw (GEMM)");
#endif
}
static int lw_wgrad_gemm(const float* dY, int lddy, const float* X, int ldx, float* dW, int lddw, int M, int N, int K, int passes,
                         float* rw_partial, cudaStream_t s) {
  if (passes == 0) return gnf_linear_wgrad(dY, lddy, X, ldx, dW, lddw, M, N, K, (gnf_stream_t)s);
#ifndef GNF_EMU
  if (rw_partial) {
    if (int e = launch_rw_wgrad(dY, lddy, X, ldx, dW, lddw, M, N, K, passes, rw_partial, s)) return e;
    return check_launch("gnf_umnn_bwd_lw (resident wgrad)");
  }
#endif
  return gnf_linear_wgrad_tc(dY, lddy, X, ldx, dW, lddw, M, N, K, passes, (gnf_stream_t)s);
}

static void lw_pad_weights(const gnf_mlp_t* net, const LwPlan& pl, float* ws, int use_rw, int transpose, cudaStream_t s) {
  for (int l = 1; l < pl.L; ++l) {
#ifndef GNF_EMU
    if (use_rw) {
      if (transpose) rw_pack_image(net->W[l], net->dims[l], net->dims[l], net->dims[l + 1], 1, nullptr, ws + pl.off_Wp[l], pl.NP, (net->dims[l + 1] + 7) / 8 * 8, s);
      else rw_pack_image(net->W[l], net->dims[l], net->dims[l + 1], net->dims[l], 0, net->b[l], ws + pl.off_Wp[l], pl.NP, (net->dims[l] + 7) / 8 * 8, s);
      continue;
    }
#endif
    GNF_LAUNCH(lw_pad_weight_kernel, lw_blocks((long long)pl.NP * pl.NP, 256, 2), 256, 0, s, net->W[l], net->dims[l + 1], net->dims[l],
               ws + pl.off_Wp[l], pl.NP, pl.NP);
  }
}

}

using namespace gnf;

extern "C" {

#ifdef GNF_DEVTOOLS
int gnf_umnn_lw_set_rw(int enable) {
  g_lw_use_rw = (enable & 1) != 0;
  g_lw_use_rw_wgrad = (enable & 1) != 0 && (enable & 2) == 0;
  return 0;
}
#endif

size_t gnf_umnn_lw_saved_floats(const gnf_mlp_t* net, int R, int S, int train) {
  LwPlan pl;
  if (lw_plan(net, R, S, train, 0, &pl)) return 0;
  return (size_t)pl.L * pl.Q * pl.NP + (size_t)pl.Q + (train ? (size_t)(pl.L - 1) * pl.Q * (pl.NP / 32) : 0);
}

size_t gnf_umnn_lw_workspace_bytes(const gnf_mlp_t* net, int R, int S, int backward) {
  LwPlan pl;
  if (lw_plan(net, R, S, 1, backward, &pl)) return 0;
  return (pl.total + 4) * sizeof(float);
}

int gnf_umnn_fwd_lw(const float* x, const float* h, const gnf_mlp_t* net, int S, const float* ccw, const float* ccn, float* z,
                    float* zrev, float* jac, float* logdet, float* saved, int train, int passes, int R, int d, void* work,
                    size_t work_bytes, gnf_stream_t stream) {
  if (!x || !h || !net || !ccw || !ccn || !z || !jac || !saved || R < 0 || d <= 0 || S < 1 || (R % d) != 0) return fail(GNF_ERR_INVALID, "gnf_umnn_fwd_lw: bad arguments");
  if (passes != 0 && passes != 1 && passes != 3) return fail(GNF_ERR_INVALID, "gnf_umnn_fwd_lw: passes must be 0 (FFMA), 1 (TF32) or 3 (3xTF32)");
  LwPlan pl;
  if (int e = lw_plan(net, R, S, train, 0, &pl)) return e;
  if (!work || work_bytes < pl.total * sizeof(float)) return fail(GNF_ERR_WORKSPACE, "gnf_umnn_fwd_lw: workspace too small (%zu < %zu)", work_bytes, pl.total * sizeof(float));
  cudaStream_t s = (cudaStream_t)stream;
  if (R == 0) return 0;
  float* ws = (float*)work;
  const int NP = pl.NP, L = pl.L, E = pl.E;
  const size_t plane = (size_t)pl.Q * NP;
  LwGeom g;
  g.R = R; g.d = d; g.E = E; g.S = S; g.nodes = pl.nodes; g.NP = NP; g.L = L; g.Q = pl.Q;
  if (logdet) cudaMemsetAsync(logdet, 0, (size_t)(R / d) * sizeof(float), s);
  float* P = ws + pl.off_P;
  if (int e = gnf_linear_fwd(h, E, net->W[0] + 1, 1 + E, net->b[0], 1, P, NP, R, net->dims[1], E, 0, stream)) return e;
  const int use_rw = (pl.rw && passes != 0 && g_lw_use_rw) ? 1 : 0;
  lw_pad_weights(net, pl, ws, use_rw, 0, s);
  const int WB = NP / 32;
  const size_t bplane = (size_t)pl.Q * WB;
  uint32_t* bits = (train && passes != 0 && L > 1) ? reinterpret_cast<uint32_t*>(saved + (size_t)L * plane + pl.Q) : nullptr;
  GNF_LAUNCH(lw_layer1_fwd_kernel, lw_blocks(pl.Q, kLwRL * 4, 6), (NP / 4) * kLwRL, 0, s, x, ccn, P, net->W[0], 1 + E,
             net->dims[1], saved, bits, g);
  for (int l = 1; l < L; ++l) {
    uint32_t* bo = (bits && l + 1 < L) ? bits + (size_t)l * bplane : nullptr;
    if (int e = lw_fwd_gemm(saved + (size_t)(l - 1) * plane, NP, ws + pl.off_Wp[l], NP, net->b[l], saved + (size_t)l * plane, NP,
                            (int)pl.Q, net->dims[l + 1], net->dims[l], 1, bo, WB, passes, use_rw ? NP : 0, s)) return e;
  }
  float* ysave = saved + (size_t)L * plane;
  {
    const float* aLp = saved + (size_t)(L - 1) * plane;
    const int nb = lw_blocks(R, 8, 8);
#define LW_OUT_FWD(J) case J: GNF_LAUNCH(lw_out_fwd_kernel<J>, nb, 256, 0, s, aLp, net->W[L], net->b[L], net->dims[L], x, h, ccw, z, zrev, jac, logdet, ysave, g); break;
    switch (NP / 32) { LW_OUT_FWD(1) LW_OUT_FWD(2) LW_OUT_FWD(3) LW_OUT_FWD(4) LW_OUT_FWD(5) LW_OUT_FWD(6) LW_OUT_FWD(7) default: LW_OUT_FWD(8) }
#undef LW_OUT_FWD
  }
  return check_launch("gnf_umnn_fwd_lw");
}

int gnf_umnn_bwd_lw(const float* x, const float* h, const gnf_mlp_t* net, int S, const float* ccw, const float* ccn, const float* jac,
                    const float* gz, const float* gzrev, const float* gjac, const float* glogdet, const float* saved, float* dx,
                    float* dh, const gnf_mlp_grad_t* grads, int passes, int R, int d, void* work, size_t work_bytes,
                    gnf_stream_t stream) {
  if (!x || !h || !net || !ccw || !ccn || !jac || !saved || !dx || !dh || !grads || R < 0 || d <= 0 || S < 1 || (R % d) != 0) return fail(GNF_ERR_INVALID, "gnf_umnn_bwd_lw: bad arguments");
  if (passes != 0 && passes != 1 && passes != 3) return fail(GNF_ERR_INVALID, "gnf_umnn_bwd_lw: passes must be 0 (FFMA), 1 (TF32) or 3 (3xTF32)");
  LwPlan pl;
  if (int e = lw_plan(net, R, S, 1, 1, &pl)) return e;
  if (!work || work_bytes < pl.total * sizeof(float)) return fail(GNF_ERR_WORKSPACE, "gnf_umnn_bwd_lw: workspace too small (%zu < %zu)", work_bytes, pl.total * sizeof(float));
  cudaStream_t s = (cudaStream_t)stream;
  const int NP = pl.NP, L = pl.L, E = pl.E;
  for (int l = 0; l < net->n_layers; ++l) {
    if (!grads->dW[l] || !grads->db[l]) return fail(GNF_ERR_INVALID, "gnf_umnn_bwd_lw: gradient pointer %d is NULL", l);
    cudaMemsetAsync(grads->dW[l], 0, (size_t)net->dims[l] * net->dims[l + 1] * sizeof(float), s);
    cudaMemsetAsync(grads->db[l], 0, (size_t)net->dims[l + 1] * sizeof(float), s);
  }
  if (R == 0) return check_launch("gnf_umnn_bwd_lw");
  float* ws = (float*)work;
  const size_t plane = (size_t)pl.Q * NP;
  LwGeom g;
  g.R = R; g.d = d; g.E = E; g.S = S; g.nodes = pl.nodes; g.NP = NP; g.L = L; g.Q = pl.Q;
  const int use_rw = (pl.rw && passes != 0 && g_lw_use_rw) ? 1 : 0;
  lw_pad_weights(net, pl, ws, use_rw, 1, s);
  float* dcur = ws + pl.off_dA;
  float* dnxt = ws + pl.off_dB;
  const int red_threads = (NP / 4) * kLwRL;
  const size_t red_smem = ((size_t)kLwRL * NP + kLwRL + 4) * sizeof(float);
  const float* ysave = saved + (size_t)L * plane;
  const int out_bwd_per_sm = 65536 / (64 * red_threads) < 1 ? 1 : (65536 / (64 * red_threads) > 4 ? 4 : 65536 / (64 * red_threads));
  GNF_LAUNCH(lw_out_bwd_kernel, lw_blocks(pl.Q, 64, out_bwd_per_sm), red_threads, red_smem, s, saved + (size_t)(L - 1) * plane, ysave, net->W[L],
             net->dims[L], x, ccw, jac, gz, gzrev, gjac, glogdet, dcur, (float*)nullptr, grads->dW[L], grads->db[L], grads->db[L - 1], g);
  for (int l = L - 1; l >= 1; --l) {
    const float* a_l = saved + (size_t)(l - 1) * plane;
    if (int e = lw_wgrad_gemm(dcur, NP, a_l, NP, grads->dW[l], net->dims[l], (int)pl.Q, net->dims[l + 1], net->dims[l], passes,
                              (use_rw && g_lw_use_rw_wgrad) ? ws + pl.off_part : nullptr, s)) return e;
    const uint32_t* mb = passes != 0 ? reinterpret_cast<const uint32_t*>(saved + (size_t)L * plane + pl.Q) + (size_t)(l - 1) * pl.Q * (NP / 32) : nullptr;
    if (int e = lw_dgrad_gemm(dcur, NP, ws + pl.off_Wp[l], NP, a_l, NP, mb, NP / 32, dnxt, NP, (int)pl.Q, net->dims[l + 1], net->dims[l], passes, use_rw ? NP : 0, s)) return e;
    if (l > 1) {
      if (int e = gnf_colsum(dnxt, NP, grads->db[l - 1], (int)pl.Q, net->dims[l], 1, stream)) return e;
    }
    float* t = dcur; dcur = dnxt; dnxt = t;
  }
  float* D = ws + pl.off_D;
  cudaMemsetAsync(grads->db[0], 0, (size_t)net->dims[1] * sizeof(float), s);
  GNF_LAUNCH(lw_layer1_bwd_kernel, lw_blocks(R, kLwRL, 6), red_threads, red_smem, s, dcur, x, ccn, net->W[0], 1 + E, net->dims[1], jac, gz,
             gzrev, D, grads->dW[0], grads->db[0], dx, g);
  if (int e = gnf_linear_wgrad(D, NP, h, E, grads->dW[0] + 1, 1 + E, R, net->dims[1], E, stream)) return e;
  if (int e = gnf_linear_dgrad(D, NP, net->W[0] + 1, 1 + E, nullptr, 0, dh, E, R, net->dims[1], E, stream)) return e;
  GNF_LAUNCH(lw_finish_dh_kernel, lw_blocks(R, 256, 4), 256, 0, s, dh, E, gz, gzrev, R, d);
  return check_launch("gnf_umnn_bwd_lw");
}


size_t gnf_umnn_bwd_tc3_workspace_bytes(const gnf_mlp_t* net, int R, int S) {
#ifdef GNF_EMU
  (void)net; (void)R; (void)S;
  gnf::set_error("tensor-core kernels have no host-simulator flavour");
  return 0;
#else
  LwPlan pl;
  if (lw_plan(net, R, S, 1, 1, &pl)) return 0;
  const size_t img = u3_bwd_image_floats(net);
  if (img == 0) return 0;
  if (!pl.rw) { set_error("umnn tc3 backward: the hidden layers do not fit the resident weight-gradient kernel"); return 0; }
  const size_t plane = (size_t)pl.Q * pl.NP;
  return ((size_t)R * pl.NP + (size_t)(pl.L - 1) * plane + 2 * (rw_wgrad_partial_floats(pl.NP) + 4) + img + 8) * sizeof(float);
#endif
}

int gnf_umnn_bwd_tc3(const float* x, const float* h, const gnf_mlp_t* net, int S, const float* ccw, const float* ccn, const float* jac,
                     const float* gz, const float* gzrev, const float* gjac, const float* glogdet, const float* saved, float* dx,
                     float* dh, const gnf_mlp_grad_t* grads, int R, int d, void* work, size_t work_bytes, gnf_stream_t stream) {
#ifdef GNF_EMU
  return gnf::fail(GNF_ERR_UNSUPPORTED, "tensor-core kernels have no host-simulator flavour");
#else
  if (!x || !h || !net || !ccw || !ccn || !jac || !saved || !dx || !dh || !grads || R < 0 || d <= 0 || S < 1 || (R % d) != 0) return fail(GNF_ERR_INVALID, "gnf_umnn_bwd_tc3: bad arguments");
  LwPlan pl;
  if (int e = lw_plan(net, R, S, 1, 1, &pl)) return e;
  const size_t need = gnf_umnn_bwd_tc3_workspace_bytes(net, R, S);
  if (need == 0) return GNF_ERR_UNSUPPORTED;
  if (!work || work_bytes < need) return fail(GNF_ERR_WORKSPACE, "gnf_umnn_bwd_tc3: workspace too small (%zu < %zu)", work_bytes, need);
  if ((reinterpret_cast<uintptr_t>(work) & 15) != 0) return fail(GNF_ERR_INVALID, "gnf_umnn_bwd_tc3: workspace must be 16-byte aligned");
  cudaStream_t s = (cudaStream_t)stream;
  const int NP = pl.NP, L = pl.L, E = pl.E;
  ZeroList zl;
  for (int l = 0; l < net->n_layers; ++l) {
    if (!grads->dW[l] || !grads->db[l]) return fail(GNF_ERR_INVALID, "gnf_umnn_bwd_tc3: gradient pointer %d is NULL", l);
    zl.add(grads->dW[l], (size_t)net->dims[l] * net->dims[l + 1]);
    zl.add(grads->db[l], (size_t)net->dims[l + 1]);
  }
  if (R == 0) { zero_many(zl, s); return check_launch("gnf_umnn_bwd_tc3"); }
  float* ws = (float*)work;
  const size_t plane = (size_t)pl.Q * NP;
  float* D = ws;
  float* dplanes = ws + (((size_t)R * NP + 3) / 4) * 4;
  float* part = dplanes + (size_t)(L - 1) * plane;
  const size_t part_floats = ((rw_wgrad_partial_floats(NP) + 3) / 4) * 4;
  float* image = part + 2 * part_floats;
  LwGeom g;
  g.R = R; g.d = d; g.E = E; g.S = S; g.nodes = pl.nodes; g.NP = NP; g.L = L; g.Q = pl.Q;
  const int red_threads = (NP / 4) * kLwRL;
  const size_t red_smem = ((size_t)kLwRL * NP + kLwRL + 4) * sizeof(float);
  const float* ysave = saved + (size_t)L * plane;
  zl.add(D, (size_t)R * NP);
  zl.add(dx, (size_t)R);
  const Branches& br = branches();
  cudaStream_t pack_stream = br.ok ? br.begin(s, 0) : nullptr;
  zero_many(zl, s);
  float* gq = dplanes;
  const uint32_t* bits_top = reinterpret_cast<const uint32_t*>(saved + (size_t)L * plane + pl.Q) + (size_t)(L - 1) * pl.Q * (NP / 32);
  const int out_bwd_per_sm = 65536 / (64 * red_threads) < 1 ? 1 : (65536 / (64 * red_threads) > 4 ? 4 : 65536 / (64 * red_threads));
  GNF_LAUNCH(lw_out_bwd_kernel, lw_blocks(pl.Q, 64, out_bwd_per_sm), red_threads, red_smem, s, saved + (size_t)(L - 1) * plane, ysave, net->W[L],
             net->dims[L], x, ccw, jac, gz, gzrev, gjac, glogdet, dplanes, gq, grads->dW[L], grads->db[L], grads->db[L - 1], g);
  if (int e = launch_u3_bwd_chain(x, net, S, ccw, ccn, jac, gz, gzrev, gjac, glogdet, saved, image, dplanes + plane, D, dx, grads, R, d, s, &br, 0, pack_stream)) return e;
  {
    cudaStream_t s0 = br.begin(s, 0);
    gnf_stream_t st0 = (gnf_stream_t)s0;
    if (int e = gnf_colsum(D, NP, grads->db[0], R, net->dims[1], 1, st0)) return e;
    if (int e = gnf_linear_wgrad(D, NP, h, E, grads->dW[0] + 1, 1 + E, R, net->dims[1], E, st0)) return e;
    if (int e = gnf_linear_dgrad(D, NP, net->W[0] + 1, 1 + E, nullptr, 0, dh, E, R, net->dims[1], E, st0)) return e;
    GNF_LAUNCH(lw_finish_dh_kernel, lw_blocks(R, 256, 4), 256, 0, s0, dh, E, gz, gzrev, R, d);
  }
  int k = 0;
  for (int l = L - 1; l >= 1; --l, ++k) {
    const float* dnext = dplanes + (size_t)(L - 1 - l) * plane;
    const float* a_l = saved + (size_t)(l - 1) * plane;
    if (k >= 2) br.end(s, 1);
    const RwRankOne top = {gq, net->W[L], bits_top, NP / 32};
    if (int e = launch_rw_wgrad(dnext, NP, a_l, NP, grads->dW[l], net->dims[l], (int)pl.Q, net->dims[l + 1], net->dims[l], 3,
                                part + (size_t)(k & 1) * part_floats, s, &br, 1, l == L - 1 ? &top : nullptr)) return e;
  }
  br.end(s, 1);
  br.end(s, 0);
  return check_launch("gnf_umnn_bwd_tc3");
#endif
}

size_t gnf_umnn_tc3_saved_floats(const gnf_mlp_t* net, int R, int S) {
  LwPlan pl;
  if (lw_plan(net, R, S, 1, 0, &pl)) return 0;
  return gnf_umnn_lw_saved_floats(net, R, S, 1) + (size_t)pl.Q * (pl.NP / 32);
}

}
```

graphical-normalizing-flows_b200/ops.py:

```python
import ctypes as C
import math
import weakref

import numpy as np
import torch

from . import _lib as L
from ._lib import check, lib, ptr, require, stream_ptr

_LAUNCHES = 0


def _count(n=1):
    global _LAUNCHES
    _LAUNCHES += n


_TIMING = False
_TIMES = {}


def enable_kernel_timing(flag):
    global _TIMING
    _TIMING = bool(flag)
    if flag:
        _TIMES.clear()
        _FLOPS.clear()
        _SHAPES.clear()


def collect_kernel_timing():
    torch.cuda.synchronize()
    return {k: [a.elapsed_time(b) for a, b in v] for k, v in _TIMES.items()}


_FLOPS = {}


def collect_call_flops():
    return {k: list(v) for k, v in _FLOPS.items()}


_SHAPES = {}


def collect_call_shapes():
    return {k: list(v) for k, v in _SHAPES.items()}


def _note_flops(name, flops, shape=None):
    if _TIMING:
        _FLOPS.setdefault(name, []).append(float(flops))
        _SHAPES.setdefault(name, []).append(shape)


def tc_kernel_name(op, M, N, K, passes=3):
    if passes == 3:
        if op == "wgrad":
            return "tc_wgrad2_kernel" if (N >= 256 and (K >= 256 or 32 <= K <= 64) and M >= 2048) else "tc_gemm_kernel"
        n, k = (N, K) if op == "fwd" else (K, N)
        return "tc_gemm2_kernel" if (M >= 1024 and ((n >= 256 and k >= 128) or (32 <= k <= 64 and n >= 256) or (32 <= n <= 64 and k >= 256))) else "tc_gemm_kernel"
    return "tc_gemm_kernel"


_TIMES_ALIAS = {}


def _call(name, *args):
    fn = getattr(lib(), name)
    if _TIMING and not L._SIMULATOR:
        e0, e1 = torch.cuda.Event(enable_timing=True), torch.cuda.Event(enable_timing=True)
        e0.record()
        rc = fn(*args)
        e1.record()
        _TIMES.setdefault(_TIMES_ALIAS.get(name, name), []).append((e0, e1))
    else:
        rc = fn(*args)
    check(rc)


def launch_count():
    return _LAUNCHES


PARALLEL_BRANCHES = True
_SIDE_STREAMS = {}


class _Fork:
    def __init__(self, k, like):
        self.on = PARALLEL_BRANCHES and like.is_cuda and not L._SIMULATOR
        if self.on:
            key = (like.device.index, k)
            if key not in _SIDE_STREAMS:
                _SIDE_STREAMS[key] = torch.cuda.Stream(device=like.device)
            self.side = _SIDE_STREAMS[key]

    def __enter__(self):
        if self.on:
            self.cur = torch.cuda.current_stream()
            self.side.wait_stream(self.cur)
            self.ctx = torch.cuda.stream(self.side)
            self.ctx.__enter__()
        return self

    def __exit__(self, *a):
        if self.on:
            self.ctx.__exit__(*a)

    def join(self):
        if self.on:
            self.cur.wait_stream(self.side)


def _contig(t):
    return t if t.is_contiguous() else t.contiguous()


class AffineFn(torch.autograd.Function):

    @staticmethod
    def forward(ctx, x, h, want_rev):
        require(x, "x"), require(h, "h")
        B, d = x.shape
        H = h.shape[2]
        if h.shape[0] != B or h.shape[1] != d or H < 2:
            raise ValueError(f"AffineNormalizer: h must be [B, d, >=2], got {tuple(h.shape)} for x {tuple(x.shape)}")
        z = torch.empty_like(x)
        jac = torch.empty_like(x)
        zrev = torch.empty_like(x) if want_rev else None
        logdet = torch.empty(B, device=x.device, dtype=x.dtype)
        mask = torch.empty(B, d, device=x.device, dtype=torch.uint8)
        _call("gnf_affine_fwd", ptr(x), ptr(h), H, ptr(z), ptr(zrev), ptr(jac), ptr(logdet), ptr(mask), B, d, stream_ptr())
        _count()
        torch.autograd.graph.increment_version(h)
        ctx.save_for_backward(x, h, mask)
        ctx.want_rev = want_rev
        ctx.set_materialize_grads(False)
        if zrev is None:
            zrev = x.new_empty(0)
            ctx.mark_non_differentiable(zrev)
        return z, jac, logdet, zrev

    @staticmethod
    def backward(ctx, gz, gjac, glogdet, gzrev):
        x, h, mask = ctx.saved_tensors
        B, d = x.shape
        H = h.shape[2]
        gz = _contig(gz) if gz is not None else None
        gjac = _contig(gjac) if gjac is not None else None
        glogdet = _contig(glogdet) if glogdet is not None else None
        gzrev = _contig(gzrev) if (gzrev is not None and ctx.want_rev) else None
        gx = torch.empty_like(x)
        gh = torch.empty_like(h)
        _call("gnf_affine_bwd", ptr(x), ptr(h), H, ptr(mask), ptr(gz), ptr(gzrev), ptr(gjac), ptr(glogdet), ptr(gx), ptr(gh),
                                   B, d, stream_ptr())
        _count()
        return gx, gh, None


class NormalLLFn(torch.autograd.Function):

    @staticmethod
    def forward(ctx, z, logdet):
        require(z, "z")
        B, d = z.shape
        if logdet is not None:
            require(logdet, "logdet")
        out = torch.empty(B, device=z.device, dtype=z.dtype)
        _call("gnf_normal_ll_fwd", ptr(z), ptr(logdet), ptr(out), B, d, stream_ptr())
        _count()
        ctx.save_for_backward(z)
        ctx.has_logdet = logdet is not None
        return out

    @staticmethod
    def backward(ctx, gout):
        (z,) = ctx.saved_tensors
        gout = _contig(gout)
        gz = torch.empty_like(z)
        _call("gnf_normal_ll_bwd", ptr(z), ptr(gout), ptr(gz), z.shape[0], z.shape[1], stream_ptr())
        _count()
        return gz, (gout if ctx.has_logdet else None)


_NLL_WORK = {}


class NllLossFn(torch.autograd.Function):

    @staticmethod
    def forward(ctx, z, logdet, constraint):
        require(z, "z"), require(logdet, "logdet")
        B, d = z.shape
        if constraint is not None:
            require(constraint, "constraint")
        key = (z.device, torch.cuda.current_stream().cuda_stream if z.is_cuda else 0)
        n = lib().gnf_nll_loss_work_floats(B)
        work = _NLL_WORK.get(key)
        if work is None or work.numel() < n or L._SIMULATOR:
            work = torch.zeros(max(n, 256), device=z.device, dtype=torch.float32)
            _NLL_WORK[key] = work
        out = torch.empty((), device=z.device, dtype=z.dtype)
        _call("gnf_nll_loss_fwd", ptr(z), ptr(logdet), ptr(constraint), ptr(out), ptr(work[work.numel() - n:]), B, d, stream_ptr())
        _count()
        ctx.save_for_backward(z)
        ctx.has_constraint = constraint is not None
        return out

    @staticmethod
    def backward(ctx, g):
        (z,) = ctx.saved_tensors
        g = _contig(g)
        gz = torch.empty_like(z)
        glogdet = torch.empty(z.shape[0], device=z.device, dtype=z.dtype)
        _call("gnf_nll_loss_bwd", ptr(z), ptr(g), ptr(gz), ptr(glogdet), z.shape[0], z.shape[1], stream_ptr())
        _count()
        return gz, glogdet, (g if ctx.has_constraint else None)


def reverse_cols(z):
    require(z, "z")
    out = torch.empty_like(z)
    _call("gnf_reverse_cols", ptr(z), ptr(out), z.shape[0], z.shape[1], stream_ptr())
    _count()
    return out


class ReverseColsFn(torch.autograd.Function):
    @staticmethod
    def forward(ctx, z):
        return reverse_cols(z)

    @staticmethod
    def backward(ctx, g):
        return reverse_cols(_contig(g))


def _pt_workspace(d, device):
    n = lib().gnf_power_trace_workspace_bytes(d)
    return torch.empty((n + 3) // 4, device=device, dtype=torch.float32), n


POWER_TRACE_SAVE_MAX_D = 64


class PowerTraceFn(torch.autograd.Function):

    @staticmethod
    def forward(ctx, A, alpha, p):
        require(A, "A")
        d = A.shape[0]
        t = torch.empty((), device=A.device, dtype=A.dtype)
        ctx.alpha, ctx.p = float(alpha), int(p)
        if d <= POWER_TRACE_SAVE_MAX_D and ctx.needs_input_grad[0]:
            G = torch.empty(d, d, device=A.device, dtype=A.dtype)
            _TIMES_ALIAS["gnf_power_trace_fwd_save"] = "gnf_power_trace_fwd"
            _call("gnf_power_trace_fwd_save", ptr(A), d, float(alpha), int(p), ptr(t), ptr(G), stream_ptr())
            _count()
            ctx.save_for_backward(A, G)
            return t
        ws, n = _pt_workspace(d, A.device)
        _call("gnf_power_trace_fwd", ptr(A), d, float(alpha), int(p), ptr(t), ptr(ws), n, stream_ptr())
        _count()
        ctx.save_for_backward(A)
        return t

    @staticmethod
    def backward(ctx, gt):
        A = ctx.saved_tensors[0]
        d = A.shape[0]
        gt = _contig(gt)
        dA = torch.empty_like(A)
        if len(ctx.saved_tensors) == 2:
            _TIMES_ALIAS["gnf_power_trace_bwd_saved"] = "gnf_power_trace_bwd"
            _call("gnf_power_trace_bwd_saved", ptr(A), ptr(ctx.saved_tensors[1]), d, ctx.alpha, ctx.p, ptr(gt), ptr(dA), stream_ptr())
            _count()
            return dA, None, None
        ws, n = _pt_workspace(d, A.device)
        _call("gnf_power_trace_bwd", ptr(A), d, ctx.alpha, ctx.p, ptr(gt), ptr(dA), ptr(ws), n, stream_ptr())
        _count()
        return dA, None, None


class DagLossFn(torch.autograd.Function):

    @staticmethod
    def forward(ctx, A, t, lambd, c, dag_const, l1_weight):
        require(A, "A"), require(t, "t")
        duals = [require(_contig(v.detach()), "dual variable") for v in (lambd, c, dag_const, l1_weight)]
        out = torch.empty((), device=A.device, dtype=A.dtype)
        _call("gnf_dag_loss_fwd", ptr(A), A.shape[0], ptr(t), *[ptr(v) for v in duals], ptr(out), stream_ptr())
        _count()
        ctx.save_for_backward(A, t, *duals)
        return out

    @staticmethod
    def backward(ctx, g):
        A, t, lambd, c, dag_const, l1_weight = ctx.saved_tensors
        g = _contig(g)
        dA = torch.empty_like(A)
        dt = torch.empty_like(t)
        _call("gnf_dag_loss_bwd", ptr(A), A.shape[0], ptr(t), ptr(lambd), ptr(c), ptr(dag_const), ptr(l1_weight), ptr(g), ptr(dA),
              ptr(dt), stream_ptr())
        _count()
        return dA, dt, None, None, None, None


_GEMM_MODE = "ffma"
_GEMM_MODES = ("ffma", "tf32", "tf32x3", "auto", "auto-fast")


def set_gemm_mode(mode):
    global _GEMM_MODE
    if mode not in _GEMM_MODES:
        raise ValueError(f"gemm mode must be one of {_GEMM_MODES}")
    _GEMM_MODE = mode


def get_gemm_mode():
    return _GEMM_MODE


def _gemm_passes(M, N, K, op="fwd"):
    if _GEMM_MODE == "ffma":
        return 0
    if _GEMM_MODE == "tf32":
        return 1
    if _GEMM_MODE == "tf32x3":
        return 3
    if _GEMM_MODE == "auto":
        if op == "wgrad":
            return 3 if (min(N, K) >= 128 and M >= 4096) else 0
        return 3 if (min(N, K) >= 128 and float(M) * N * K >= 4e8) else 0
    return 1 if min(N, K) >= 128 else 0


def _pad4(n):
    return (n + 3) // 4 * 4


def _rows(M, N, like):
    t = torch.empty(M, _pad4(N), device=like.device, dtype=like.dtype)
    return t if t.shape[1] == N else t[:, :N]


def _tma_weight(W):
    if W.stride(0) % 4 == 0 and W.data_ptr() % 16 == 0:
        return W
    Wp = _rows(W.shape[0], W.shape[1], W)
    Wp.copy_(W)
    return Wp


SPLITK_SKINNY = True


_SPLIT_CACHE = {}


def _split_weight(W):
    key = (W.data_ptr(), W._version, tuple(W.shape), torch.cuda.is_current_stream_capturing() if W.is_cuda else False)
    hit = _SPLIT_CACHE.get(key)
    if hit is not None and hit[2]() is W:
        return hit[0], hit[1]
    N, K = W.shape
    hi = torch.empty(N, _pad4(K), device=W.device, dtype=W.dtype)
    lo = torch.empty_like(hi)
    _call("gnf_split_tf32", ptr(W), W.stride(0), ptr(hi), ptr(lo), hi.stride(0), N, K, stream_ptr())
    _count()
    if len(_SPLIT_CACHE) >= 16:
        _SPLIT_CACHE.clear()
    _SPLIT_CACHE[key] = (hi, lo, weakref.ref(W))
    return hi, lo


def _tma_ok(t, ld):
    return t.data_ptr() % 16 == 0 and ld % 4 == 0


def linear_fwd(X, W, bias, relu, bias_period=1, out=None, ldy=None, K=None, ldx=None):
    M = X.shape[0]
    N = W.shape[0]
    K = W.shape[1] if K is None else K
    ldx = X.stride(0) if ldx is None else ldx
    if out is None:
        out = _rows(M, N, X)
        ldy = out.stride(0)
    passes = _gemm_passes(M, N, K)
    if passes == 3 and _tma_ok(X, ldx) and K == W.shape[1]:
        hi, lo = _split_weight(W)
        _note_flops("gnf_linear_fwd_tc", 2. * M * N * K, (M, N, K))
        _TIMES_ALIAS["gnf_linear_fwd_tc_ps"] = "gnf_linear_fwd_tc"
        _call("gnf_linear_fwd_tc_ps", ptr(X), ldx, ptr(hi), ptr(lo), hi.stride(0), ptr(bias), bias_period, ptr(out), ldy, M, N, K,
              int(relu), stream_ptr())
    elif passes:
        W = _tma_weight(W)
        _note_flops("gnf_linear_fwd_tc", 2. * M * N * K, (M, N, K))
        _call("gnf_linear_fwd_tc", ptr(X), ldx, ptr(W), W.stride(0), ptr(bias), bias_period, ptr(out), ldy, M, N, K, int(relu),
              passes, stream_ptr())
    else:
        nbytes = lib().gnf_linear_fwd_splitk_workspace_bytes(M, N, K) if (SPLITK_SKINNY and bias_period <= 1 and (X.is_cuda or L._SIMULATOR)) else 0
        if nbytes:
            work = torch.empty(nbytes // 4, device=X.device, dtype=torch.float32)
            _TIMES_ALIAS["gnf_linear_fwd_splitk"] = "gnf_linear_fwd"
            _call("gnf_linear_fwd_splitk", ptr(X), ldx, ptr(W), W.stride(0), ptr(bias), ptr(out), ldy, M, N, K, int(relu), ptr(work), nbytes,
                  stream_ptr())
            _count()
        else:
            _call("gnf_linear_fwd", ptr(X), ldx, ptr(W), W.stride(0), ptr(bias), bias_period, ptr(out), ldy, M, N, K, int(relu),
                  stream_ptr())
    _count()
    return out


def linear_dgrad(dY, lddy, W, act, M, out=None, lddx=None):
    N, K = W.shape
    if out is None:
        out = _rows(M, K, dY)
        lddx = out.stride(0)
    passes = _gemm_passes(M, N, K)
    if passes == 3 and _tma_ok(dY, lddy):
        hi, lo = _split_weight(W)
        _note_flops("gnf_linear_dgrad_tc", 2. * M * N * K, (M, N, K))
        _TIMES_ALIAS["gnf_linear_dgrad_tc_ps"] = "gnf_linear_dgrad_tc"
        _call("gnf_linear_dgrad_tc_ps", ptr(dY), lddy, ptr(hi), ptr(lo), hi.stride(0), ptr(act), (act.stride(0) if act is not None else 0),
              ptr(out), lddx, M, N, K, stream_ptr())
    elif passes:
        W = _tma_weight(W)
        _note_flops("gnf_linear_dgrad_tc", 2. * M * N * K, (M, N, K))
        _call("gnf_linear_dgrad_tc", ptr(dY), lddy, ptr(W), W.stride(0), ptr(act), (act.stride(0) if act is not None else 0),
              ptr(out), lddx, M, N, K, passes, stream_ptr())
    else:
        _call("gnf_linear_dgrad", ptr(dY), lddy, ptr(W), W.stride(0), ptr(act), (act.stride(0) if act is not None else 0),
              ptr(out), lddx, M, N, K, stream_ptr())
    _count()
    return out


def linear_wgrad(dY, lddy, X, ldx, M, N, K, out=None, lddw=None):
    dW = torch.empty(N, K, device=dY.device, dtype=dY.dtype) if out is None else out
    lddw = K if out is None else lddw
    passes = _gemm_passes(M, N, K, "wgrad")
    if passes:
        _note_flops("gnf_linear_wgrad_tc", 2. * M * N * K, (M, N, K))
        _call("gnf_linear_wgrad_tc", ptr(dY), lddy, ptr(X), ldx, ptr(dW), lddw, M, N, K, passes, stream_ptr())
    else:
        _call("gnf_linear_wgrad", ptr(dY), lddy, ptr(X), ldx, ptr(dW), lddw, M, N, K, stream_ptr())
    _count()
    return dW


def linear_wgrad_bias(dY, lddy, X, ldx, M, N, K):
    if _gemm_passes(M, N, K, "wgrad") == 3 and M > 0:
        dW = torch.empty(N, K, device=dY.device, dtype=dY.dtype)
        db = torch.empty(N, device=dY.device, dtype=dY.dtype)
        _note_flops("gnf_linear_wgrad_tc", 2. * M * N * K, (M, N, K))
        _TIMES_ALIAS["gnf_linear_wgrad_bias_tc"] = "gnf_linear_wgrad_tc"
        _call("gnf_linear_wgrad_bias_tc", ptr(dY), lddy, ptr(X), ldx, ptr(dW), K, ptr(db), M, N, K, stream_ptr())
        _count()
        return dW, db
    db = colsum(dY, lddy, M, N).view(N)
    return linear_wgrad(dY, lddy, X, ldx, M, N, K), db


def colsum(Y, ldy, M, N, period=1):
    out = torch.empty(period, N, device=Y.device, dtype=Y.dtype)
    _call("gnf_colsum", ptr(Y), ldy, ptr(out), M, N, period, stream_ptr())
    _count()
    return out


def _mlp_backward(gout, ldg, acts, x_in, ldx, K0, weights, need_dx, first_layer_done=False):
    n = len(weights)
    M = gout.shape[0]
    dWs, dbs = [None] * n, [None] * n
    delta, ldd = gout, ldg
    for l in range(n - 1, 0, -1):
        W = weights[l]
        N, K = W.shape
        a_prev = acts[l - 1]
        if _gemm_passes(M, N, K, "wgrad") == 0 and M > 0:
            with _Fork(0, delta) as f:
                dWs[l], dbs[l] = linear_wgrad_bias(delta, ldd, a_prev, a_prev.stride(0), M, N, K)
            delta_in, delta = delta, linear_dgrad(delta, ldd, W, a_prev, M)
            f.join()
            del delta_in
        else:
            dWs[l], dbs[l] = linear_wgrad_bias(delta, ldd, a_prev, a_prev.stride(0), M, N, K)
            delta = linear_dgrad(delta, ldd, W, a_prev, M)
        ldd = delta.stride(0)
    if first_layer_done:
        return dWs, dbs, None, delta
    W = weights[0]
    N = W.shape[0]
    dbs[0] = colsum(delta, ldd, M, N).view(N)
    dWs[0] = linear_wgrad(delta, ldd, x_in, ldx, M, N, K0)
    dx = linear_dgrad(delta, ldd, W, None, M) if need_dx else None
    return dWs, dbs, dx, delta


class MlpFn(torch.autograd.Function):

    @staticmethod
    def forward(ctx, x, K0, *params):
        require(x, "x")
        weights = [require(_contig(p), "weight") for p in params[0::2]]
        biases = [require(_contig(p), "bias") for p in params[1::2]]
        n = len(weights)
        _SPLIT_CACHE.clear()
        if weights[0].shape[1] != K0 or x.shape[1] < K0:
            raise ValueError(f"MLP: first layer expects {weights[0].shape[1]} inputs, got {K0} (x has {x.shape[1]} columns)")
        acts = []
        cur, ldx, K = x, x.stride(0), K0
        for l in range(n):
            out = None
            if l == n - 1:
                out = torch.empty(x.shape[0], weights[l].shape[0], device=x.device, dtype=x.dtype)
            cur = linear_fwd(cur, weights[l], biases[l], relu=(l < n - 1), K=K, ldx=ldx, out=out, ldy=weights[l].shape[0])
            ldx, K = cur.stride(0), cur.shape[1]
            if l < n - 1:
                acts.append(cur)
        ctx.save_for_backward(x, *weights, *acts)
        ctx.n, ctx.K0 = n, K0
        ctx.need_dx = x.requires_grad
        return cur

    @staticmethod
    def backward(ctx, gout):
        saved = ctx.saved_tensors
        n = ctx.n
        x, weights, acts = saved[0], list(saved[1:1 + n]), list(saved[1 + n:])
        gout = _contig(gout)
        dWs, dbs, dx, _ = _mlp_backward(gout, gout.stride(0), acts, x, x.stride(0), ctx.K0, weights, ctx.need_dx)
        gx = None
        if dx is not None:
            if x.shape[1] == ctx.K0:
                gx = dx
            else:
                gx = torch.zeros_like(x)
                gx[:, :ctx.K0] = dx
        out = [gx, None]
        for l in range(n):
            out += [dWs[l], dbs[l]]
        return tuple(out)


def pack_rows(W, mask=None, perm=None, R=None):
    R = W.shape[0] if R is None else R
    K = W.shape[1]
    out = torch.empty(R, K, device=W.device, dtype=W.dtype)
    _call("gnf_pack_rows", ptr(W), ptr(mask), ptr(perm), ptr(out), R, K, stream_ptr())
    _count()
    return out


class PackRowsFn(torch.autograd.Function):

    @staticmethod
    def forward(ctx, W, mask, perm):
        W = require(_contig(W), "W")
        ctx.mask, ctx.perm, ctx.shape = mask, perm, W.shape
        return pack_rows(W, mask, perm, R=(perm.numel() if perm is not None else None))

    @staticmethod
    def backward(ctx, g):
        g = _contig(g)
        N, K = ctx.shape
        dW = torch.empty(N, K, device=g.device, dtype=g.dtype)
        _call("gnf_unpack_rows", ptr(g), ptr(ctx.mask), ptr(ctx.perm), ptr(dW), g.shape[0], N, K, stream_ptr())
        _count()
        return dW, None, None


class PackVecFn(torch.autograd.Function):

    @staticmethod
    def forward(ctx, b, perm):
        b = require(_contig(b), "bias")
        ctx.perm, ctx.n = perm, b.numel()
        return pack_rows(b.view(-1, 1), None, perm, R=perm.numel()).view(-1)

    @staticmethod
    def backward(ctx, g):
        g = _contig(g)
        db = torch.empty(ctx.n, device=g.device, dtype=g.dtype)
        _call("gnf_unpack_vec", ptr(g), ptr(ctx.perm), ptr(db), g.numel(), ctx.n, stream_ptr())
        _count()
        return db, None


def broadcast_rows(constants, h, indep):
    B, d, H = h.shape
    _call("gnf_broadcast_rows", ptr(constants), ptr(h), B, d, indep, H, stream_ptr())
    _count()


class GateSpec:

    def __init__(self, mode, imp, h_thresh=0., T=1., seed=0, offset=0, noise=None, offset_dev=None):
        self.mode, self.imp, self.h_thresh, self.T = mode, imp, float(h_thresh), float(T)
        self.seed, self.offset, self.noise = int(seed), int(offset), noise
        self.offset_dev = offset_dev

    def c_struct(self):
        g = L.GateT()
        g.mode, g.temperature, g.seed, g.offset = self.mode, self.T, self.seed, self.offset
        n = self.noise or ()
        g.noise1 = n[0].data_ptr() if len(n) > 0 else None
        g.noise2 = n[1].data_ptr() if len(n) > 1 else None
        g.offset_dev = self.offset_dev.data_ptr() if self.offset_dev is not None else None
        return g


def dag_dump_noise(gate, B, d, device):
    n1 = torch.empty(B, d, d, device=device, dtype=torch.float32)
    n2 = torch.empty(B, d, d, device=device, dtype=torch.float32) if gate.mode == L.GATE_GUMBEL else None
    g = GateSpec(gate.mode, gate.imp, gate.h_thresh, gate.T, gate.seed, gate.offset, None, gate.offset_dev).c_struct()
    _call("gnf_dag_dump_noise", C.byref(g), ptr(n1), ptr(n2), B, d, stream_ptr())
    _count()
    return (n1, n2) if n2 is not None else (n1,)


DAG_L1_PLANE = True
DAG_L1_PLANE_MIN_D = 65
DAG_L1_PLANE_KEEP_DERIVATIVES = True


DAG_L1_KEEP_GATES = True


def _narrow_l1_tc(M, N1, delta):
    return (DAG_L1_NARROW_TC and _GEMM_MODE in ("auto", "tf32x3") and not L._SIMULATOR and M >= 2048 and N1 >= 128
            and _tma_ok(delta, delta.stride(0)))


DAG_L1_NARROW_TC = True
DAG_L1_NARROW_TC_FWD = True


def _dag_l1_plane(M, N1, d):
    return DAG_L1_PLANE and d >= DAG_L1_PLANE_MIN_D and M > 0 and _gemm_passes(M, N1, d) != 0 and not L._SIMULATOR


class DagMlpFn(torch.autograd.Function):

    @staticmethod
    def forward(ctx, x, A, gate, hot, *params):
        require(x, "x")
        A = require(_contig(A), "A")
        weights = [require(_contig(p), "weight") for p in params[0::2]]
        biases = [require(_contig(p), "bias") for p in params[1::2]]
        B, d = x.shape
        n = len(weights)
        _SPLIT_CACHE.clear()
        if weights[0].shape[1] != (2 * d if hot else d):
            raise ValueError(f"DAGConditioner: first layer expects {weights[0].shape[1]} inputs, d={d}, hot_encoding={hot}")
        for t in (gate.noise or ()):
            require(t, "noise")
            if tuple(t.shape) != (B, d, d):
                raise ValueError("replayed gate noise must be [B, d, d]")
        st = stream_ptr()
        P = torch.empty_like(A)
        dPdA = torch.empty_like(A)
        _call("gnf_dag_importance", ptr(A), d, gate.imp, gate.h_thresh, ptr(P), ptr(dPdA), st)
        N1 = weights[0].shape[0]
        tc_fwd = (DAG_L1_NARROW_TC_FWD and DAG_L1_KEEP_GATES and d <= 64 and gate.mode != L.GATE_TABLE and B > 0 and n > 1 and hot
                  and DAG_L1_NARROW_TC and _GEMM_MODE in ("auto", "tf32x3", "auto-fast", "tf32") and not L._SIMULATOR
                  and B * d >= 2048 and N1 >= 256 and d >= 32)
        if tc_fwd:
            T = torch.empty(d, _pad4(N1), device=x.device, dtype=x.dtype)
            _call("gnf_dag_bias_table_ld", ptr(weights[0]), weights[0].stride(0), ptr(biases[0]), ptr(T), T.stride(0), d, N1, 1, st)
        else:
            T = torch.empty(d if hot else 1, N1, device=x.device, dtype=x.dtype)
            _call("gnf_dag_bias_table", ptr(weights[0]), weights[0].stride(0), ptr(biases[0]), ptr(T), d, N1, int(hot), st)
        g = gate.c_struct()
        f_split = None
        if B > 0:
            todo = [weights[l] for l in range(1, n) if _gemm_passes(B * d, weights[l].shape[0], weights[l].shape[1]) == 3]
            if todo:
                with _Fork(0, x) as f_split:
                    for W in todo:
                        _split_weight(W)
        y = _rows(B * d, N1, x) if n > 1 else torch.empty(B * d, N1, device=x.device, dtype=x.dtype)
        E = W1e = narrow = None
        gate_planes = (None, None)
        if _dag_l1_plane(B * d, N1, d):
            E = _rows(B * d, d, x)
            if DAG_L1_PLANE_KEEP_DERIVATIVES and (ctx.needs_input_grad[0] or ctx.needs_input_grad[1]):
                gate_planes = (_rows(B * d, d, x), _rows(B * d, d, x))
            _call("gnf_dag_embed_fwd", ptr(x), ptr(P), C.byref(g), ptr(E), ptr(gate_planes[0]), ptr(gate_planes[1]), E.stride(0), B, d, st)
            W1e = weights[0][:, :d]
            linear_fwd(E, W1e, T, relu=(n > 1), bias_period=(d if hot else 1), out=y, ldy=y.stride(0), K=d, ldx=E.stride(0))
            _count(2)
        elif (DAG_L1_KEEP_GATES and d <= 64 and gate.mode != L.GATE_TABLE and B > 0 and (any(ctx.needs_input_grad) or tc_fwd)):
            narrow = tuple(torch.empty(B * d, 64, device=x.device, dtype=x.dtype) for _ in range(3))
            if tc_fwd:
                _TIMES_ALIAS["gnf_dag_gate_planes"] = "gnf_dag_l1_fwd"
                _call("gnf_dag_gate_planes", ptr(x), ptr(P), C.byref(g), ptr(narrow[0]), ptr(narrow[1]), ptr(narrow[2]), B, d, st)
                hi, lo = _split_weight(weights[0][:, :d])
                _TIMES_ALIAS["gnf_linear_fwd_tc_ps_tb"] = "gnf_dag_l1_fwd"
                _call("gnf_linear_fwd_tc_ps_tb", ptr(narrow[0]), 64, ptr(hi), ptr(lo), hi.stride(0), ptr(T), T.stride(0), d, ptr(y), y.stride(0),
                      B * d, N1, d, 1, st)
                _count(4)
            else:
                _TIMES_ALIAS["gnf_dag_l1_fwd_save"] = "gnf_dag_l1_fwd"
                _call("gnf_dag_l1_fwd_save", ptr(x), ptr(P), C.byref(g), ptr(weights[0]), weights[0].stride(0), ptr(T), (d if hot else 1),
                      ptr(y), y.stride(0), ptr(narrow[0]), ptr(narrow[1]), ptr(narrow[2]), B, d, N1, int(n > 1), st)
                _count(3)
        else:
            _call("gnf_dag_l1_fwd", ptr(x), ptr(P), C.byref(g), ptr(weights[0]), weights[0].stride(0), ptr(T), (d if hot else 1),
                                       ptr(y), y.stride(0), B, d, N1, int(n > 1), st)
            _count(3)
        if f_split is not None:
            f_split.join()
        acts = []
        cur = y
        for l in range(1, n):
            acts.append(cur)
            out = None
            if l == n - 1:
                out = torch.empty(B, d, weights[l].shape[0], device=x.device, dtype=x.dtype)
            cur = linear_fwd(cur, weights[l], biases[l], relu=(l < n - 1), out=out, ldy=weights[l].shape[0])
        ctx.E, ctx.W1e = (E, W1e) if any(ctx.needs_input_grad) else (None, None)
        ctx.gate_planes = gate_planes
        ctx.narrow = narrow if any(ctx.needs_input_grad) else None
        ctx.save_for_backward(x, A, P, dPdA, *weights, *acts)
        ctx.gate, ctx.hot, ctx.n = gate, hot, n
        if n == 1:
            cur = cur.view(B, d, -1).clone()
        return cur

    @staticmethod
    def backward(ctx, gh):
        saved = ctx.saved_tensors
        n, hot, gate = ctx.n, ctx.hot, ctx.gate
        needs = ctx.needs_input_grad
        x, A, P, dPdA = saved[:4]
        weights, acts = list(saved[4:4 + n]), list(saved[4 + n:])
        B, d = x.shape
        M = B * d
        gh = _contig(gh).view(M, -1)
        dWs, dbs, _, delta = _mlp_backward(gh, gh.stride(0), acts, None, 0, 0, weights, False, first_layer_done=True)
        W1 = weights[0]
        N1 = W1.shape[0]
        g = gate.c_struct()
        dW1 = torch.empty_like(W1)
        E, W1e = ctx.E, ctx.W1e
        DXp, DPp = ctx.gate_planes
        ctx.E = ctx.W1e = None
        ctx.gate_planes = (None, None)
        narrow, ctx.narrow = ctx.narrow, None
        narrow_tc = narrow is not None and _narrow_l1_tc(M, N1, delta)
        with _Fork(0, x) as f_w:
            st = stream_ptr()
            if E is not None:
                linear_wgrad(delta, delta.stride(0), E, E.stride(0), M, N1, d, out=dW1, lddw=dW1.stride(0))
            elif narrow_tc:
                _TIMES_ALIAS["gnf_linear_wgrad_tc"] = "gnf_dag_l1_wgrad"
                _call("gnf_linear_wgrad_tc", ptr(delta), delta.stride(0), ptr(narrow[0]), 64, ptr(dW1), W1.stride(0), M, N1, d, 3, st)
                _TIMES_ALIAS.pop("gnf_linear_wgrad_tc")
            elif narrow is not None:
                _TIMES_ALIAS["gnf_dag_l1_wgrad_saved"] = "gnf_dag_l1_wgrad"
                _call("gnf_dag_l1_wgrad_saved", ptr(delta), delta.stride(0), ptr(narrow[0]), ptr(dW1), W1.stride(0), B, d, N1, st)
            else:
                _call("gnf_dag_l1_wgrad", ptr(delta), delta.stride(0), ptr(x), ptr(P), C.byref(g), ptr(dW1), W1.stride(0), B, d, N1, st)
        with _Fork(1, x) as f_b:
            dT = colsum(delta, delta.stride(0), M, N1, period=(d if hot else 1))
            db1 = torch.empty(N1, device=x.device, dtype=x.dtype)
            _call("gnf_dag_bias_table_bwd", ptr(dT), ptr(dW1), W1.stride(0), ptr(db1), d, N1, int(hot), stream_ptr())
        _count(2)
        dWs[0], dbs[0] = dW1, db1
        st = stream_ptr()
        dx = dA = dE = dP = hi = lo = None
        if needs[0] or needs[1]:
            dx = torch.empty_like(x)
            dP = torch.empty_like(A)
            if E is not None:
                dE = linear_dgrad(delta, delta.stride(0), W1e, None, M)
                _call("gnf_dag_embed_bwd", ptr(dE), dE.stride(0), ptr(x), ptr(P), C.byref(g), ptr(DXp), ptr(DPp), ptr(dx), ptr(dP), B, d, st)
            elif narrow_tc:
                hi, lo = _split_weight(W1[:, :d])
                dE = torch.empty(M, 64, device=x.device, dtype=x.dtype)
                _TIMES_ALIAS["gnf_linear_dgrad_tc_ps"] = "gnf_dag_l1_dgrad"
                _call("gnf_linear_dgrad_tc_ps", ptr(delta), delta.stride(0), ptr(hi), ptr(lo), hi.stride(0), None, 0, ptr(dE), 64, M, N1, d, st)
                _TIMES_ALIAS["gnf_linear_dgrad_tc_ps"] = "gnf_linear_dgrad_tc"
                _TIMES_ALIAS["gnf_dag_l1_reduce_saved"] = "gnf_dag_l1_dgrad"
                _call("gnf_dag_l1_reduce_saved", ptr(dE), ptr(narrow[1]), ptr(narrow[2]), ptr(dx), ptr(dP), B, d, st)
                _count(2)
            elif narrow is not None:
                _TIMES_ALIAS["gnf_dag_l1_dgrad_saved"] = "gnf_dag_l1_dgrad"
                _call("gnf_dag_l1_dgrad_saved", ptr(delta), delta.stride(0), ptr(W1), W1.stride(0), ptr(narrow[1]), ptr(narrow[2]), ptr(dx),
                      ptr(dP), B, d, N1, st)
            else:
                _call("gnf_dag_l1_dgrad", ptr(delta), delta.stride(0), ptr(W1), W1.stride(0), ptr(x), ptr(P), C.byref(g), ptr(dx),
                                             ptr(dP), B, d, N1, st)
            dA = torch.empty_like(A)
            _call("gnf_dag_finish_dA", ptr(dP), ptr(dPdA), ptr(dA), d, 0, st)
            _count(2)
        f_w.join()
        f_b.join()
        del dE, DXp, DPp, narrow, E, dT, hi, lo
        out = [dx if needs[0] else None, dA if needs[1] else None, None, None]
        for l in range(n):
            out += [dWs[l], dbs[l]]
        return tuple(out)


_CC_CACHE = {}

SAVE_ACTIVATIONS_MAX_BYTES = 48 << 30
SAVE_ACTIVATIONS_FREE_FRACTION = 0.5


def _activation_budget(device):
    if SAVE_ACTIVATIONS_MAX_BYTES <= 0:
        return 0
    if L._SIMULATOR or torch.cuda.is_current_stream_capturing():
        return SAVE_ACTIVATIONS_MAX_BYTES
    free, _ = torch.cuda.mem_get_info(device)
    return min(SAVE_ACTIVATIONS_MAX_BYTES, int(free * SAVE_ACTIVATIONS_FREE_FRACTION))


UMNN_ENGINE = "auto"
UMNN_LAYERWISE_MIN_NODE_ROWS = 16384
UMNN_FWD_FUSED_TC3 = True


def _umnn_layerwise_passes(net, R, S, train, device=None):
    if UMNN_ENGINE == "fused" or net.dims[0] < 2:
        return None
    passes = {"ffma": 0, "tf32": 1, "tf32x3": 3, "auto": 3, "auto-fast": 3}[_GEMM_MODE]
    if UMNN_ENGINE == "auto":
        hidden = [net.dims[l] for l in range(1, net.n_layers)]
        if passes == 0 or net.n_layers < 3 or min(hidden) < 64 or R * (S + 2) < UMNN_LAYERWISE_MIN_NODE_ROWS:
            return None
    need = 4 * (lib().gnf_umnn_lw_saved_floats(C.byref(net), R, S, int(train)) +
                (lib().gnf_umnn_lw_workspace_bytes(C.byref(net), R, S, int(train)) // 4))
    if need == 0 or need > _activation_budget(device):
        if UMNN_ENGINE == "layerwise" and need == 0:
            raise RuntimeError("libgnf: " + lib().gnf_last_error().decode())
        return None
    return passes


def cc_weights(nb_steps, device):
    key = (int(nb_steps), str(device))
    if key not in _CC_CACHE:
        S = int(nb_steps)
        k = np.arange(S + 1, dtype=np.float64)
        lam = np.cos(np.outer(k, k) * math.pi / S)
        lam[:, 0] = .5
        lam[:, -1] = .5 * lam[:, -1]
        lam = lam * 2 / S
        W = np.zeros(S + 1, dtype=np.float64)
        even = np.arange(0, S + 1, 2)
        W[even] = 2. / (1. - even.astype(np.float64) ** 2)
        W[0] = 1.
        w = torch.tensor(lam.T @ W).float().to(device)
        t = torch.tensor(np.cos(k * math.pi / S)).float().to(device)
        _CC_CACHE[key] = (w, t)
    return _CC_CACHE[key]


def _mlp_struct(weights, biases):
    n = len(weights)
    if n > L.GNF_MAX_LAYERS:
        raise ValueError(f"integrand network deeper than {L.GNF_MAX_LAYERS} linear layers is not supported")
    m = L.MlpT()
    m.n_layers = n
    m.dims[0] = weights[0].shape[1]
    for l in range(n):
        m.dims[l + 1] = weights[l].shape[0]
        m.W[l] = weights[l].data_ptr()
        m.b[l] = biases[l].data_ptr()
    return m


class UmnnFn(torch.autograd.Function):

    @staticmethod
    def forward(ctx, x, h, S, want_rev, fast, *params):
        require(x, "x"), require(h, "h")
        weights = [require(_contig(p), "weight") for p in params[0::2]]
        biases = [require(_contig(p), "bias") for p in params[1::2]]
        B, d = x.shape
        E = h.shape[2]
        if weights[0].shape[1] != 1 + E:
            raise ValueError(f"integrand expects {weights[0].shape[1] - 1} conditioning features, h has {E}")
        R = B * d
        net = _mlp_struct(weights, biases)
        nbytes = (lib().gnf_umnn_tc_workspace_bytes if fast else lib().gnf_umnn_workspace_bytes)(C.byref(net))
        if nbytes == 0:
            raise RuntimeError("libgnf: " + lib().gnf_last_error().decode())
        ws = torch.empty((nbytes + 3) // 4, device=x.device, dtype=torch.float32)
        ccw, ccn = cc_weights(S, x.device)
        z = torch.empty_like(x)
        jac = torch.empty_like(x)
        zrev = torch.empty_like(x) if want_rev else None
        logdet = torch.empty(B, device=x.device, dtype=x.dtype)
        saved = None
        fused_bwd = False
        train = any(ctx.needs_input_grad)
        lw_passes = None if fast else _umnn_layerwise_passes(net, R, int(S), train, x.device)
        if fast:
            _call("gnf_umnn_fwd_tc", ptr(x), ptr(h), C.byref(net), int(S), ptr(ccw), ptr(ccn), ptr(z), ptr(zrev), ptr(jac),
                  ptr(logdet), R, d, ptr(ws), nbytes, stream_ptr())
        elif lw_passes == 3 and UMNN_FWD_FUSED_TC3 and lib().gnf_umnn_tc3_workspace_bytes(C.byref(net), R) != 0:
            if train:
                saved = torch.empty(lib().gnf_umnn_tc3_saved_floats(C.byref(net), R, int(S)), device=x.device, dtype=torch.float32)
                fused_bwd = lib().gnf_umnn_bwd_tc3_workspace_bytes(C.byref(net), R, int(S)) != 0
            nbytes = lib().gnf_umnn_tc3_workspace_bytes(C.byref(net), R)
            ws = torch.empty((nbytes + 3) // 4, device=x.device, dtype=torch.float32)
            _call("gnf_umnn_fwd_tc3", ptr(x), ptr(h), C.byref(net), int(S), ptr(ccw), ptr(ccn), ptr(z), ptr(zrev), ptr(jac),
                  ptr(logdet), ptr(saved), int(train), int(train), R, d, ptr(ws), nbytes, stream_ptr())
            _count(6)
        elif lw_passes is not None:
            saved = torch.empty(lib().gnf_umnn_lw_saved_floats(C.byref(net), R, int(S), int(train)), device=x.device,
                                dtype=torch.float32)
            nbytes = lib().gnf_umnn_lw_workspace_bytes(C.byref(net), R, int(S), 0)
            ws = torch.empty((nbytes + 3) // 4, device=x.device, dtype=torch.float32)
            _call("gnf_umnn_fwd_lw", ptr(x), ptr(h), C.byref(net), int(S), ptr(ccw), ptr(ccn), ptr(z), ptr(zrev), ptr(jac),
                  ptr(logdet), ptr(saved), int(train), lw_passes, R, d, ptr(ws), nbytes, stream_ptr())
            _count(3 + len(weights))
            if not train:
                saved = None
        else:
            if train and SAVE_ACTIVATIONS_MAX_BYTES > 0:
                per_row = lib().gnf_umnn_saved_floats_per_node_row(C.byref(net))
                need = R * (int(S) + 1) * per_row * 4
                if 0 < need <= _activation_budget(x.device):
                    saved = torch.empty(R * (int(S) + 1) * per_row, device=x.device, dtype=torch.float32)
            _call("gnf_umnn_fwd", ptr(x), ptr(h), C.byref(net), int(S), ptr(ccw), ptr(ccn), ptr(z), ptr(zrev), ptr(jac),
                  ptr(logdet), ptr(saved), R, d, ptr(ws), nbytes, stream_ptr())
        ctx.lw_passes = lw_passes if (lw_passes is not None and train) else None
        ctx.fused_bwd = fused_bwd
        _count(2)
        ctx.saved_acts = saved
        ctx.save_for_backward(x, h, jac, *weights, *biases)
        ctx.S, ctx.want_rev, ctx.n = int(S), want_rev, len(weights)
        ctx.set_materialize_grads(False)
        if zrev is None:
            zrev = x.new_empty(0)
            ctx.mark_non_differentiable(zrev)
        return z, jac, logdet, zrev

    @staticmethod
    def backward(ctx, gz, gjac, glogdet, gzrev):
        saved = ctx.saved_tensors
        n = ctx.n
        x, h, jac = saved[:3]
        weights, biases = list(saved[3:3 + n]), list(saved[3 + n:])
        B, d = x.shape
        R = B * d
        net = _mlp_struct(weights, biases)
        nbytes = lib().gnf_umnn_workspace_bytes(C.byref(net))
        ws = torch.empty((nbytes + 3) // 4, device=x.device, dtype=torch.float32)
        ccw, ccn = cc_weights(ctx.S, x.device)
        gz = _contig(gz) if gz is not None else None
        gjac = _contig(gjac) if gjac is not None else None
        glogdet = _contig(glogdet) if glogdet is not None else None
        gzrev = _contig(gzrev) if (gzrev is not None and ctx.want_rev) else None
        dx = torch.empty_like(x)
        dh = torch.empty_like(h)
        grads = L.MlpGradT()
        dWs = [torch.empty_like(w) for w in weights]
        dbs = [torch.empty_like(b) for b in biases]
        for l in range(n):
            grads.dW[l] = dWs[l].data_ptr()
            grads.db[l] = dbs[l].data_ptr()
        if ctx.lw_passes is not None and ctx.fused_bwd:
            nbytes = lib().gnf_umnn_bwd_tc3_workspace_bytes(C.byref(net), R, ctx.S)
            ws = torch.empty((nbytes + 3) // 4, device=x.device, dtype=torch.float32)
            _call("gnf_umnn_bwd_tc3", ptr(x), ptr(h), C.byref(net), ctx.S, ptr(ccw), ptr(ccn), ptr(jac), ptr(gz), ptr(gzrev),
                  ptr(gjac), ptr(glogdet), ptr(ctx.saved_acts), ptr(dx), ptr(dh), C.byref(grads), R, d, ptr(ws), nbytes, stream_ptr())
            _count(6 + 2 * n)
        elif ctx.lw_passes is not None:
            nbytes = lib().gnf_umnn_lw_workspace_bytes(C.byref(net), R, ctx.S, 1)
            ws = torch.empty((nbytes + 3) // 4, device=x.device, dtype=torch.float32)
            _call("gnf_umnn_bwd_lw", ptr(x), ptr(h), C.byref(net), ctx.S, ptr(ccw), ptr(ccn), ptr(jac), ptr(gz), ptr(gzrev),
                  ptr(gjac), ptr(glogdet), ptr(ctx.saved_acts), ptr(dx), ptr(dh), C.byref(grads), ctx.lw_passes, R, d, ptr(ws),
                  nbytes, stream_ptr())
            _count(4 + 3 * n)
        else:
            _call("gnf_umnn_bwd", ptr(x), ptr(h), C.byref(net), ctx.S, ptr(ccw), ptr(ccn), ptr(jac), ptr(gz), ptr(gzrev), ptr(gjac),
                  ptr(glogdet), ptr(ctx.saved_acts), ptr(dx), ptr(dh), C.byref(grads), R, d, ptr(ws), nbytes, stream_ptr())
        ctx.saved_acts = None
        _count(2)
        out = [dx, dh, None, None, None]
        for l in range(n):
            out += [dWs[l], dbs[l]]
        return tuple(out)


def umnn_forward_on_tensor_cores(params, R, S, device):
    if L._SIMULATOR:
        return False
    weights, biases = [p.detach() for p in params[0::2]], [p.detach() for p in params[1::2]]
    net = _mlp_struct(weights, biases)
    return (_umnn_layerwise_passes(net, R, int(S), False, device) == 3 and UMNN_FWD_FUSED_TC3
            and lib().gnf_umnn_tc3_workspace_bytes(C.byref(net), R) != 0)


def umnn_invert(z, h, S, weights, biases, iters=20, lo=-20., hi=20.):
    require(z, "z"), require(h, "h")
    weights = [require(_contig(w.detach()), "weight") for w in weights]
    biases = [require(_contig(b.detach()), "bias") for b in biases]
    B, d = z.shape
    if weights[0].shape[1] != 1 + h.shape[2]:
        raise ValueError(f"integrand expects {weights[0].shape[1] - 1} conditioning features, h has {h.shape[2]}")
    net = _mlp_struct(weights, biases)
    nbytes = lib().gnf_umnn_workspace_bytes(C.byref(net))
    if nbytes == 0:
        raise RuntimeError("libgnf: " + lib().gnf_last_error().decode())
    ws = torch.empty((nbytes + 3) // 4, device=z.device, dtype=torch.float32)
    ccw, ccn = cc_weights(S, z.device)
    x = torch.empty_like(z)
    _call("gnf_umnn_invert", ptr(z), ptr(h), C.byref(net), int(S), ptr(ccw), ptr(ccn), ptr(x), int(iters), float(lo), float(hi), B * d,
          ptr(ws), nbytes, stream_ptr())
    _count(2)
    return x


def _pad32(v):
    return (v + 31) // 32 * 32


def linear_fwd_rw(X, W, bias, relu, passes=3, want_bits=False):
    require(X, "X"), require(W, "W")
    N, K = W.shape
    M = X.shape[0]
    if X.shape[1] != _pad32(K):
        raise ValueError(f"X must have pad32(K) = {_pad32(K)} columns")
    nbytes = lib().gnf_linear_rw_workspace_bytes(N, K)
    if nbytes == 0:
        raise RuntimeError("libgnf: " + lib().gnf_last_error().decode())
    ws = torch.empty(nbytes // 4, device=X.device, dtype=torch.float32)
    Y = torch.empty(M, _pad32(N), device=X.device, dtype=torch.float32)
    bits = torch.empty(M, _pad32(N) // 32, device=X.device, dtype=torch.int32) if want_bits else None
    _call("gnf_linear_fwd_rw", ptr(X), X.stride(0), ptr(W), W.stride(0), ptr(bias), ptr(Y), Y.stride(0), ptr(bits), M, N, K,
          int(relu), int(passes), ptr(ws), nbytes, stream_ptr())
    _count(2)
    return (Y, bits) if want_bits else Y


def linear_dgrad_rw(dY, W, act=None, mask_bits=None, passes=3):
    require(dY, "dY"), require(W, "W")
    N, K = W.shape
    M = dY.shape[0]
    if dY.shape[1] != _pad32(N):
        raise ValueError(f"dY must have pad32(N) = {_pad32(N)} columns")
    nbytes = lib().gnf_linear_rw_workspace_bytes(K, N)
    if nbytes == 0:
        raise RuntimeError("libgnf: " + lib().gnf_last_error().decode())
    ws = torch.empty(nbytes // 4, device=dY.device, dtype=torch.float32)
    dX = torch.empty(M, _pad32(K), device=dY.device, dtype=torch.float32)
    _call("gnf_linear_dgrad_rw", ptr(dY), dY.stride(0), ptr(W), W.stride(0), ptr(act), act.stride(0) if act is not None else 0,
          ptr(mask_bits), ptr(dX), dX.stride(0), M, N, K, int(passes), ptr(ws), nbytes, stream_ptr())
    _count(2)
    return dX


def linear_wgrad_rw(dY, X, N, K, passes=3):
    require(dY, "dY"), require(X, "X")
    M = dY.shape[0]
    if X.shape[1] != _pad32(K) or X.shape[0] != M:
        raise ValueError(f"X must be [M, pad32(K) = {_pad32(K)}]")
    nbytes = lib().gnf_linear_wgrad_rw_workspace_bytes(N, K)
    if nbytes == 0:
        raise RuntimeError("libgnf: " + lib().gnf_last_error().decode())
    ws = torch.empty(nbytes // 4, device=dY.device, dtype=torch.float32)
    dW = torch.empty(N, K, device=dY.device, dtype=torch.float32)
    _call("gnf_linear_wgrad_rw", ptr(dY), dY.stride(0), ptr(X), X.stride(0), ptr(dW), K, M, N, K, int(passes), ptr(ws), nbytes,
          stream_ptr())
    _count(2)
    return dW


def counter_add(counter, inc=1):
    _call("gnf_counter_add", ptr(counter), int(inc), stream_ptr())
    _count()


def tc_selftest(A, W, mode):
    require(A, "A"), require(W, "W")
    Cm = torch.empty(128, W.shape[0], device=A.device, dtype=A.dtype)
    _call("gnf_tc_selftest", ptr(A), ptr(W), ptr(Cm), W.shape[0], W.shape[1], int(mode), stream_ptr())
    _count()
    return Cm
```

include/gnf.h:

```cpp
#ifndef GNF_H_
#define GNF_H_

#include <stddef.h>
#include <stdint.h>

#ifdef __cplusplus
extern "C" {
#endif

typedef void* gnf_stream_t;

#define GNF_ERR_INVALID 1001
#define GNF_ERR_UNSUPPORTED 1002
#define GNF_ERR_WORKSPACE 1003
#define GNF_ERR_PEER 1004

#define GNF_MAX_LAYERS 8

int gnf_version(void);
const char* gnf_last_error(void);
int gnf_has_device_code(void);


int gnf_affine_fwd(const float* x, float* h, int H, float* z, float* zrev, float* jac, float* logdet,
                   uint8_t* clampmask, int B, int d, gnf_stream_t stream);

int gnf_affine_bwd(const float* x, const float* h, int H, const uint8_t* clampmask, const float* gz,
                   const float* gzrev, const float* gjac, const float* glogdet, float* gx, float* gh, int B,
                   int d, gnf_stream_t stream);

int gnf_normal_ll_fwd(const float* z, const float* logdet, float* out, int B, int d, gnf_stream_t stream);
int gnf_normal_ll_bwd(const float* z, const float* gout, float* gz, int B, int d, gnf_stream_t stream);

size_t gnf_nll_loss_work_floats(int B);
int gnf_nll_loss_fwd(const float* z, const float* logdet, const float* constraint, float* out, float* work, int B, int d,
                     gnf_stream_t stream);
int gnf_nll_loss_bwd(const float* z, const float* g, float* gz, float* glogdet, int B, int d, gnf_stream_t stream);

size_t gnf_power_trace_workspace_bytes(int d);
int gnf_power_trace_fwd(const float* A, int d, float alpha, int p, float* t_out, void* work, size_t work_bytes,
                        gnf_stream_t stream);
int gnf_power_trace_bwd(const float* A, int d, float alpha, int p, const float* gt, float* dA, void* work,
                        size_t work_bytes, gnf_stream_t stream);

int gnf_power_trace_fwd_save(const float* A, int d, float alpha, int p, float* t_out, float* G_out, gnf_stream_t stream);
int gnf_power_trace_bwd_saved(const float* A, const float* G, int d, float alpha, int p, const float* gt, float* dA,
                              gnf_stream_t stream);


int gnf_linear_fwd(const float* X, int ldx, const float* W, int ldw, const float* bias, int bias_period, float* Y,
                   int ldy, int M, int N, int K, int relu, gnf_stream_t stream);
int gnf_linear_dgrad(const float* dY, int lddy, const float* W, int ldw, const float* act, int ldact, float* dX,
                     int lddx, int M, int N, int K, gnf_stream_t stream);
int gnf_linear_wgrad(const float* dY, int lddy, const float* X, int ldx, float* dW, int lddw, int M, int N, int K,
                     gnf_stream_t stream);
size_t gnf_linear_fwd_splitk_workspace_bytes(int M, int N, int K);
int gnf_linear_fwd_splitk(const float* X, int ldx, const float* W, int ldw, const float* bias, float* Y, int ldy, int M, int N, int K,
                          int relu, void* work, size_t work_bytes, gnf_stream_t stream);
int gnf_colsum(const float* Y, int ldy, float* out, int M, int N, int period, gnf_stream_t stream);

int gnf_linear_fwd_tc(const float* X, int ldx, const float* W, int ldw, const float* bias, int bias_period, float* Y,
                      int ldy, int M, int N, int K, int relu, int passes, gnf_stream_t stream);
int gnf_linear_dgrad_tc(const float* dY, int lddy, const float* W, int ldw, const float* act, int ldact, float* dX,
                        int lddx, int M, int N, int K, int passes, gnf_stream_t stream);
int gnf_linear_wgrad_tc(const float* dY, int lddy, const float* X, int ldx, float* dW, int lddw, int M, int N, int K,
                        int passes, gnf_stream_t stream);
int gnf_linear_wgrad_bias_tc(const float* dY, int lddy, const float* X, int ldx, float* dW, int lddw, float* db, int M, int N, int K,
                             gnf_stream_t stream);
int gnf_split_tf32(const float* W, int ldw, float* W_hi, float* W_lo, int ld, int N, int K, gnf_stream_t stream);
int gnf_linear_fwd_tc_ps(const float* X, int ldx, const float* W_hi, const float* W_lo, int ldw, const float* bias, int bias_period,
                         float* Y, int ldy, int M, int N, int K, int relu, gnf_stream_t stream);
int gnf_linear_fwd_tc_ps_tb(const float* X, int ldx, const float* W_hi, const float* W_lo, int ldw, const float* table, int ldt,
                            int period, float* Y, int ldy, int M, int N, int K, int relu, gnf_stream_t stream);
int gnf_linear_dgrad_tc_ps(const float* dY, int lddy, const float* W_hi, const float* W_lo, int ldw, const float* act, int ldact,
                           float* dX, int lddx, int M, int N, int K, gnf_stream_t stream);
int gnf_tc_gemm_plan(int M, int N, int K, int passes, int wgrad, int* bn, int* splits);

int gnf_pack_rows(const float* W, const float* mask, const int32_t* perm, float* out, int R, int K,
                  gnf_stream_t stream);
int gnf_unpack_rows(const float* dWp, const float* mask, const int32_t* perm, float* dW, int R, int N, int K,
                    gnf_stream_t stream);
int gnf_unpack_vec(const float* src, const int32_t* perm, float* dst, int R, int N, gnf_stream_t stream);

enum {
  GNF_GATE_TABLE = 0,
  GNF_GATE_GUMBEL = 1,
  GNF_GATE_NOISER = 2
};
enum { GNF_IMP_RAW = 0, GNF_IMP_SOFT = 1, GNF_IMP_HARD_SOFT = 2, GNF_IMP_HARD_SQ = 3 };

typedef struct {
  int32_t mode;
  float temperature;
  uint64_t seed;
  uint64_t offset;
  const float* noise1;
  const float* noise2;
  const uint64_t* offset_dev;
} gnf_gate_t;

int gnf_dag_importance(const float* A, int d, int imp, float h_thresh, float* P, float* dPdA, gnf_stream_t stream);
int gnf_dag_bias_table(const float* W1, int ldw, const float* b1, float* T, int d, int N, int hot,
                       gnf_stream_t stream);
int gnf_dag_bias_table_ld(const float* W1, int ldw, const float* b1, float* T, int ldt, int d, int N, int hot, gnf_stream_t stream);
int gnf_dag_bias_table_bwd(const float* dT, float* dW1, int ldw, float* db1, int d, int N, int hot,
                           gnf_stream_t stream);
int gnf_dag_l1_fwd(const float* x, const float* P, const gnf_gate_t* gate, const float* W1, int ldw, const float* T,
                   int bias_period, float* Y, int ldy, int B, int d, int N, int relu, gnf_stream_t stream);
int gnf_dag_l1_wgrad(const float* dY, int lddy, const float* x, const float* P, const gnf_gate_t* gate, float* dW1,
                     int ldw, int B, int d, int N, gnf_stream_t stream);
int gnf_dag_l1_dgrad(const float* dY, int lddy, const float* W1, int ldw, const float* x, const float* P,
                     const gnf_gate_t* gate, float* dx, float* dP, int B, int d, int N, gnf_stream_t stream);
int gnf_dag_l1_fwd_save(const float* x, const float* P, const gnf_gate_t* gate, const float* W1, int ldw, const float* T,
                        int bias_period, float* Y, int ldy, float* E, float* DX, float* DP, int B, int d, int N, int relu,
                        gnf_stream_t stream);
int gnf_dag_gate_planes(const float* x, const float* P, const gnf_gate_t* gate, float* E, float* DX, float* DP, int B, int d,
                        gnf_stream_t stream);
int gnf_dag_l1_wgrad_saved(const float* dY, int lddy, const float* E, float* dW1, int ldw, int B, int d, int N, gnf_stream_t stream);
int gnf_dag_l1_dgrad_saved(const float* dY, int lddy, const float* W1, int ldw, const float* DX, const float* DP, float* dx,
                           float* dP, int B, int d, int N, gnf_stream_t stream);
int gnf_dag_l1_reduce_saved(const float* dE, const float* DX, const float* DP, float* dx, float* dP, int B, int d, gnf_stream_t stream);
int gnf_dag_embed_fwd(const float* x, const float* P, const gnf_gate_t* gate, float* E, float* DX, float* DP, int lde, int B,
                      int d, gnf_stream_t stream);
int gnf_dag_embed_bwd(const float* dE, int lde, const float* x, const float* P, const gnf_gate_t* gate, const float* DX,
                      const float* DP, float* dx, float* dP, int B, int d, gnf_stream_t stream);
int gnf_dag_finish_dA(const float* dP, const float* dPdA, float* dA, int d, int accumulate, gnf_stream_t stream);
int gnf_dag_dump_noise(const gnf_gate_t* gate, float* n1, float* n2, int B, int d, gnf_stream_t stream);

typedef struct {
  int32_t n_layers;
  int32_t dims[GNF_MAX_LAYERS + 1];
  const float* W[GNF_MAX_LAYERS];
  const float* b[GNF_MAX_LAYERS];
} gnf_mlp_t;

typedef struct {
  float* dW[GNF_MAX_LAYERS];
  float* db[GNF_MAX_LAYERS];
} gnf_mlp_grad_t;

size_t gnf_umnn_workspace_bytes(const gnf_mlp_t* net);
size_t gnf_umnn_saved_floats_per_node_row(const gnf_mlp_t* net);
int gnf_umnn_fwd(const float* x, const float* h, const gnf_mlp_t* net, int S, const float* ccw, const float* ccn,
                 float* z, float* zrev, float* jac, float* logdet, float* saved, int R, int d, void* work,
                 size_t work_bytes, gnf_stream_t stream);
int gnf_umnn_invert(const float* z, const float* h, const gnf_mlp_t* net, int S, const float* ccw, const float* ccn, float* x,
                    int iters, float lo, float hi, int R, void* work, size_t work_bytes, gnf_stream_t stream);
int gnf_umnn_bwd(const float* x, const float* h, const gnf_mlp_t* net, int S, const float* ccw, const float* ccn,
                 const float* jac, const float* gz, const float* gzrev, const float* gjac, const float* glogdet,
                 const float* saved, float* dx, float* dh, const gnf_mlp_grad_t* grads, int R, int d, void* work,
                 size_t work_bytes, gnf_stream_t stream);

size_t gnf_umnn_tc_workspace_bytes(const gnf_mlp_t* net);
int gnf_umnn_fwd_tc(const float* x, const float* h, const gnf_mlp_t* net, int S, const float* ccw, const float* ccn,
                    float* z, float* zrev, float* jac, float* logdet, int R, int d, void* work, size_t work_bytes,
                    gnf_stream_t stream);
size_t gnf_umnn_lw_saved_floats(const gnf_mlp_t* net, int R, int S, int train);
size_t gnf_umnn_lw_workspace_bytes(const gnf_mlp_t* net, int R, int S, int backward);
int gnf_umnn_fwd_lw(const float* x, const float* h, const gnf_mlp_t* net, int S, const float* ccw, const float* ccn,
                    float* z, float* zrev, float* jac, float* logdet, float* saved, int train, int passes, int R, int d,
                    void* work, size_t work_bytes, gnf_stream_t stream);
int gnf_umnn_bwd_lw(const float* x, const float* h, const gnf_mlp_t* net, int S, const float* ccw, const float* ccn,
                    const float* jac, const float* gz, const float* gzrev, const float* gjac, const float* glogdet,
                    const float* saved, float* dx, float* dh, const gnf_mlp_grad_t* grads, int passes, int R, int d,
                    void* work, size_t work_bytes, gnf_stream_t stream);

size_t gnf_umnn_tc3_workspace_bytes(const gnf_mlp_t* net, int R);
size_t gnf_umnn_tc3_saved_floats(const gnf_mlp_t* net, int R, int S);
int gnf_umnn_fwd_tc3(const float* x, const float* h, const gnf_mlp_t* net, int S, const float* ccw, const float* ccn,
                     float* z, float* zrev, float* jac, float* logdet, float* saved, int train, int order, int R, int d,
                     void* work, size_t work_bytes, gnf_stream_t stream);

typedef struct {
  float* param;
  const float* grad;
  float* exp_avg;
  float* exp_avg_sq;
  int64_t numel;
} gnf_adam_tensor_t;
int gnf_adam_step(const gnf_adam_tensor_t* tensors, int n_tensors, const int64_t* step_dev, float lr, float beta1, float beta2,
                  float eps, float weight_decay, gnf_stream_t stream);

int gnf_peer_alloc(size_t bytes, void** out);
int gnf_peer_free(void* p);
int gnf_peer_export(const void* p, unsigned char* handle64);
int gnf_peer_import(const unsigned char* handle64, void** out);
int gnf_peer_close(void* p);
size_t gnf_peer_flag_bytes(void);
int gnf_peer_allreduce_avg(float* const* bufs, unsigned* const* flags, int rank, int world, long long numel,
                           gnf_stream_t stream);

size_t gnf_umnn_bwd_tc3_workspace_bytes(const gnf_mlp_t* net, int R, int S);
int gnf_umnn_bwd_tc3(const float* x, const float* h, const gnf_mlp_t* net, int S, const float* ccw, const float* ccn,
                     const float* jac, const float* gz, const float* gzrev, const float* gjac, const float* glogdet,
                     const float* saved, float* dx, float* dh, const gnf_mlp_grad_t* grads, int R, int d, void* work,
                     size_t work_bytes, gnf_stream_t stream);

int gnf_dag_loss_fwd(const float* A, int d, const float* t, const float* lambd, const float* c, const float* dag_const,
                     const float* l1_weight, float* out, gnf_stream_t stream);
int gnf_dag_loss_bwd(const float* A, int d, const float* t, const float* lambd, const float* c, const float* dag_const,
                     const float* l1_weight, const float* gout, float* dA, float* dt, gnf_stream_t stream);


size_t gnf_linear_rw_workspace_bytes(int N, int K);
int gnf_linear_fwd_rw(const float* X, int ldx, const float* W, int ldw, const float* bias, float* Y, int ldy, uint32_t* bits_out,
                      int M, int N, int K, int relu, int passes, void* work, size_t work_bytes, gnf_stream_t stream);
int gnf_linear_dgrad_rw(const float* dY, int lddy, const float* W, int ldw, const float* act, int ldact,
                        const uint32_t* mask_bits, float* dX, int lddx, int M, int N, int K, int passes, void* work,
                        size_t work_bytes, gnf_stream_t stream);

size_t gnf_linear_wgrad_rw_workspace_bytes(int N, int K);
int gnf_linear_wgrad_rw(const float* dY, int lddy, const float* X, int ldx, float* dW, int lddw, int M, int N, int K,
                        int passes, void* work, size_t work_bytes, gnf_stream_t stream);

int gnf_tc_selftest(const float* A, const float* W, float* C, int N, int K, int mode, gnf_stream_t stream);

int gnf_reverse_cols(const float* src, float* dst, int B, int d, gnf_stream_t stream);
int gnf_broadcast_rows(const float* constants, float* h, int B, int d, int indep, int H, gnf_stream_t stream);
int gnf_counter_add(uint64_t* counter, uint64_t inc, gnf_stream_t stream);

#ifdef __cplusplus
}
#endif
#endif
```

Measured before the change: 115,500.

## Accumulate per-row weighted top-layer activation sums in forward, drop top activation plane

In fused-backward training mode, the forward UMNN tensor-core kernel no longer writes the top hidden layer's activations per quadrature point. Instead it accumulates two per-row weighted sums (M and A) with segmented warp reductions and atomics, and a small kernel turns them into the last-layer weight gradient. The separate lw_out_bwd pass is removed: the backward chain kernel now emits the quadrature gradients and the two top bias gradients itself. This cuts saved-activation memory traffic and one full pass over Q×NP, at the cost of extra atomics and shared-memory staging in the forward kernel.

```diff
diff --git a/graphical-normalizing-flows_b200/_lib.py b/graphical-normalizing-flows_b200/_lib.py
--- a/graphical-normalizing-flows_b200/_lib.py
+++ b/graphical-normalizing-flows_b200/_lib.py
@@ -106,7 +106,7 @@
     "gnf_umnn_bwd_lw": ([_P, _P, C.POINTER(MlpT), _I, _P, _P, _P, _P, _P, _P, _P, _P, _P, _P, C.POINTER(MlpGradT), _I, _I, _I,
                          _P, _SZ, _P], C.c_int),
     "gnf_umnn_tc3_workspace_bytes": ([C.POINTER(MlpT), _I], _SZ),
-    "gnf_umnn_tc3_saved_floats": ([C.POINTER(MlpT), _I, _I], _SZ),
+    "gnf_umnn_tc3_saved_floats": ([C.POINTER(MlpT), _I, _I, _I], _SZ),
     "gnf_umnn_bwd_tc3_workspace_bytes": ([C.POINTER(MlpT), _I, _I], _SZ),
     "gnf_umnn_bwd_tc3": ([_P, _P, C.POINTER(MlpT), _I, _P, _P, _P, _P, _P, _P, _P, _P, _P, _P, C.POINTER(MlpGradT), _I, _I,
                           _P, _SZ, _P], C.c_int),
diff --git a/graphical-normalizing-flows_b200/csrc/tc_umnn3.cu b/graphical-normalizing-flows_b200/csrc/tc_umnn3.cu
--- a/graphical-normalizing-flows_b200/csrc/tc_umnn3.cu
+++ b/graphical-normalizing-flows_b200/csrc/tc_umnn3.cu
@@ -1,4 +1,5 @@
 #include "tc_common.cuh"
+#include "tc_umnn3.h"
 
 #ifndef GNF_EMU
 namespace gnf {
@@ -82,10 +83,30 @@
   }
 }
 
+__device__ __forceinline__ float u3_colsum16(float (&w)[16], int lane) {
+#pragma unroll
+  for (int i = 0; i < 16; ++i) w[i] += __shfl_xor_sync(0xffffffffu, w[i], 16);
+#pragma unroll
+  for (int o = 8; o >= 1; o >>= 1) {
+    const bool up = (lane & o) != 0;
+#pragma unroll
+    for (int i = 0; i < o; ++i) {
+      const float send = up ? w[i] : w[i + o];
+      const float keep = up ? w[i + o] : w[i];
+      w[i] = keep + __shfl_xor_sync(0xffffffffu, send, o);
+    }
+  }
+  return w[0];
+}
+
 struct U3Params {
   const float *x, *h, *ccw, *ccn, *P, *image, *blast;
-  float *z, *zrev, *jac, *logdet, *saved;
-  int R, d, E, S, nodes, L, N1, train, order, p_smem, debug;
+  float *z, *zrev, *jac, *logdet;
+  float* saved;
+  float* ysave;
+  uint32_t* bits;
+  float *M, *A;
+  int R, d, E, S, nodes, L, N1, NL, order, p_smem, debug;
   long long Q;
   int kp[GNF_MAX_LAYERS], nch[GNF_MAX_LAYERS];
   unsigned off_img[GNF_MAX_LAYERS], off_tail, chunk_floats;
@@ -113,7 +134,8 @@
   float* pbuf = stage_all + EW * kU3StageBlock;
   float* ypart = pbuf + 2 * kU3PRows * NP;
   float* red = ypart + NB * kU3Rows;
-  float* ccs = red + kU3Rows;
+  float* ewt = red + kU3Rows;
+  float* ccs = ewt + kU3Rows;
   uint64_t* bars = reinterpret_cast<uint64_t*>(ccs + 2 * kU3MaxNodes);
   uint64_t* w_full = bars;
   uint64_t* w_empty = w_full + kU3Stages;
@@ -242,10 +264,12 @@
     const float* w0col = tail + L * NP + c;
     const float blast = __ldg(p.blast);
     const size_t plane = (size_t)Q * NP;
-    float* ysave = p.saved ? p.saved + (size_t)L * plane : nullptr;
-    uint32_t* bits = (p.saved && p.train && L > 1) ? reinterpret_cast<uint32_t*>(p.saved + (size_t)L * plane + Q) : nullptr;
+    float* ysave = p.ysave;
+    uint32_t* bits = p.bits;
+    bool row_sums = p.M != nullptr;
 #ifdef GNF_DEVTOOLS
     if (p.debug & 4) { bits = nullptr; ysave = nullptr; }
+    if (p.debug & 8) row_sums = false;
 #endif
     const bool full_block = c + 32 <= p.N1;
 
@@ -398,7 +422,7 @@
           }
           ypart[ci * kU3Rows + t] = (y0 + y1) + (y2 + y3);
           if (bits && cur.q < Q) bits[(size_t)l * Q * NB + (size_t)cur.q * NB + ci] = mask_word(v);
-          if (p.saved) store_block(p.saved + (size_t)l * plane, v, cur.q);
+          if (p.saved && !p.M) store_block(p.saved + (size_t)l * plane, v, cur.q);
           named_bar_sync(1, EW * 32);
           const bool cur_valid = cur.q < Q;
           if (ci == 0) {
@@ -416,6 +440,10 @@
               }
             }
             red[t] = wv;
+            if (p.M) {
+              const float de = (y > 0.f) ? 1.f : expf(y);
+              ewt[t] = !cur_valid ? 0.f : (cur.kn <= p.S ? ccs[kU3MaxNodes + cur.kn] * de : de);
+            }
           }
           named_bar_sync(1, EW * 32);
           if (ci == 0 && cur_valid && (cur.kn == 0 || t == 0)) {
@@ -428,6 +456,38 @@
             atomicAdd(p.z + cur.r, cz);
             if (p.zrev) { const int b = cur.r / p.d, ii = cur.r % p.d; atomicAdd(p.zrev + (size_t)b * p.d + (p.d - 1 - ii), cz); }
           }
+          if (row_sums) {
+            const float wt = ewt[t];
+            const int tg = cur_valid ? 2 * cur.r + (cur.kn > p.S ? 1 : 0) : -1;
+            const int rh = lane & 16, col = lane & 15;
+#pragma unroll
+            for (int hb = 0; hb < 2; ++hb) {
+#pragma unroll
+              for (int j4 = 0; j4 < 4; ++j4) {
+                const uint32_t* vj = v + 16 * hb + 4 * j4;
+                *reinterpret_cast<float4*>(stage + lane * 16 + 4 * (j4 ^ ((lane >> 1) & 3))) =
+                    make_float4(__uint_as_float(vj[0]) * wt, __uint_as_float(vj[1]) * wt, __uint_as_float(vj[2]) * wt, __uint_as_float(vj[3]) * wt);
+              }
+              __syncwarp();
+              const int n = c + 16 * hb + col;
+              const bool col_ok = n < p.NL;
+              int cur_t = __shfl_sync(0xffffffffu, tg, rh);
+              float acc = 0.f;
+#pragma unroll
+              for (int i = 0; i < 16; ++i) {
+                const int row = rh + i;
+                const int rt = __shfl_sync(0xffffffffu, tg, row);
+                if (rt != cur_t) {
+                  if (cur_t >= 0 && col_ok) atomicAdd(((cur_t & 1) ? p.A : p.M) + (size_t)(cur_t >> 1) * NP + n, acc);
+                  acc = 0.f;
+                  cur_t = rt;
+                }
+                acc += stage[row * 16 + 4 * ((col >> 2) ^ ((row >> 1) & 3)) + (col & 3)];
+              }
+              if (cur_t >= 0 && col_ok) atomicAdd(((cur_t & 1) ? p.A : p.M) + (size_t)(cur_t >> 1) * NP + n, acc);
+              __syncwarp();
+            }
+          }
           U3_STAMP(warp == 0 ? 1 : 3);
         }
         cur = nxt;
@@ -440,7 +500,10 @@
 }
 
 struct U3BParams {
-  const float *x, *ccw, *ccn, *jac, *gz, *gzrev, *gjac, *glogdet, *image, *saved;
+  const float *x, *ccw, *ccn, *jac, *gz, *gzrev, *gjac, *glogdet, *image;
+  const float* ysave;
+  const uint32_t* bits;
+  float* gq;
   float* dplanes;
   float *D, *dx, *dW0;
   float* db[GNF_MAX_LAYERS];
@@ -450,22 +513,6 @@
   int kp[GNF_MAX_LAYERS], nch[GNF_MAX_LAYERS];
   unsigned off_img[GNF_MAX_LAYERS], off_tail, chunk_floats;
 };
-
-__device__ __forceinline__ float u3_colsum16(float (&w)[16], int lane) {
-#pragma unroll
-  for (int i = 0; i < 16; ++i) w[i] += __shfl_xor_sync(0xffffffffu, w[i], 16);
-#pragma unroll
-  for (int o = 8; o >= 1; o >>= 1) {
-    const bool up = (lane & o) != 0;
-#pragma unroll
-    for (int i = 0; i < o; ++i) {
-      const float send = up ? w[i] : w[i + o];
-      const float keep = up ? w[i + o] : w[i];
-      w[i] = keep + __shfl_xor_sync(0xffffffffu, send, o);
-    }
-  }
-  return w[0];
-}
 
 template <int NB>
 __global__ void __launch_bounds__((4 * NB + 2) * 32, 1) umnn_bwd_tc3_kernel(U3BParams p) {
@@ -581,8 +628,8 @@
     const float* wL = tail + c;
     const float* w0col = tail + NP + c;
     const size_t plane = (size_t)Q * NP;
-    const float* ysave = p.saved + (size_t)L * plane;
-    const uint32_t* bits = reinterpret_cast<const uint32_t*>(p.saved + (size_t)L * plane + Q);
+    const float* ysave = p.ysave;
+    const uint32_t* bits = p.bits;
     const size_t bplane = (size_t)Q * NB;
 
     struct Row { int q, r, kn; float gq, tq, jg; uint32_t mtop; };
@@ -661,6 +708,24 @@
       __syncwarp();
       if (lane == 0) u3_arrive(&a_full[ci]);
     };
+    auto top_sums = [&](const Row& w) {
+      if (ci == 0) {
+        if (w.q < Q) p.gq[w.q] = w.gq;
+        float sg = w.gq;
+#pragma unroll
+        for (int o = 16; o >= 1; o >>= 1) sg += __shfl_xor_sync(0xffffffffu, sg, o);
+        if (lane == 0) atomicAdd(p.db[L], sg);
+      }
+#pragma unroll
+      for (int hb = 0; hb < 2; ++hb) {
+        float w16[16];
+#pragma unroll
+        for (int j = 0; j < 16; ++j) w16[j] = ((w.mtop >> (16 * hb + j)) & 1u) ? w.gq * wL[16 * hb + j] : 0.f;
+        const float sum = u3_colsum16(w16, lane);
+        const int n = c + 16 * hb + (lane & 15);
+        if (lane < 16 && n < p.dims[L]) atomicAdd(p.db[L - 1] + n, sum);
+      }
+    };
 
     Row cur;
     cur.q = 0; cur.r = 0; cur.kn = 0; cur.gq = 0.f; cur.tq = 0.f; cur.jg = 0.f; cur.mtop = 0u;
@@ -673,6 +738,7 @@
         const bool gen_late = gen_next && ci >= p.nch[l] - 1;
         const bool valid = cur.q < Q;
         const uint32_t m = valid ? __ldg(bits + (size_t)(l - 1) * bplane + (size_t)cur.q * NB + ci) : 0u;
+        if (l == L - 1) top_sums(cur);
         if (gen_next) nxt = row_of(tl + 1);
         if (gen_next && !gen_late) {
           mbar_wait(&a_free[ci], (uint32_t)(tl & 1));
@@ -806,8 +872,9 @@
 }
 
 int launch_u3_bwd_chain(const float* x, const gnf_mlp_t* net, int S, const float* ccw, const float* ccn, const float* jac, const float* gz,
-                        const float* gzrev, const float* gjac, const float* glogdet, const float* saved, float* image, float* dplanes, float* D,
-                        float* dx, const gnf_mlp_grad_t* grads, int R, int d, cudaStream_t s, const Branches* br, int side, cudaStream_t pack_stream) {
+                        const float* gzrev, const float* gjac, const float* glogdet, const float* ysave, const uint32_t* bits, float* image,
+                        float* gq, float* dplanes, float* D, float* dx, const gnf_mlp_grad_t* grads, int R, int d, cudaStream_t s,
+                        const Branches* br, int side, cudaStream_t pack_stream) {
   U3BPlan pl;
   if (int e = u3b_plan(net, &pl)) return e;
   const int NP = pl.NP, L = pl.L;
@@ -824,8 +891,8 @@
   GNF_LAUNCH(u3_pack_bwd_kernel, blocks, 256, 0, (br && pack_stream) ? pack_stream : s, a, image);
   if (br && pack_stream) br->end(s, side);
   U3BParams p;
-  p.x = x; p.ccw = ccw; p.ccn = ccn; p.jac = jac; p.gz = gz; p.gzrev = gzrev; p.gjac = gjac; p.glogdet = glogdet; p.image = image; p.saved = saved;
-  p.dplanes = dplanes; p.D = D; p.dx = dx; p.dW0 = grads->dW[0]; p.ldw0 = net->dims[0];
+  p.x = x; p.ccw = ccw; p.ccn = ccn; p.jac = jac; p.gz = gz; p.gzrev = gzrev; p.gjac = gjac; p.glogdet = glogdet; p.image = image;
+  p.ysave = ysave; p.bits = bits; p.gq = gq; p.dplanes = dplanes; p.D = D; p.dx = dx; p.dW0 = grads->dW[0]; p.ldw0 = net->dims[0];
   for (int l = 0; l < GNF_MAX_LAYERS; ++l) p.db[l] = grads->db[l];
   p.R = R; p.d = d; p.E = net->dims[0] - 1; p.S = S; p.nodes = nodes; p.L = L; p.Q = Q;
   for (int l = 0; l <= GNF_MAX_LAYERS; ++l) p.dims[l] = l <= net->n_layers ? net->dims[l] : 0;
@@ -847,7 +914,7 @@
 static size_t u3_smem_bytes(int NP) {
   const int NB = NP / 32, EW = 4 * NB;
   return ((size_t)kU3Stages * 2 * 8 * NP * 4 + (size_t)(GNF_MAX_LAYERS + 1) * NP + (size_t)EW * kU3StageBlock + (size_t)2 * kU3PRows * NP +
-          (size_t)(NB + 1) * kU3Rows + 2 * kU3MaxNodes) * sizeof(float) + (2 * kU3Stages + 2 * NB + 6) * sizeof(uint64_t) + 16;
+          (size_t)(NB + 2) * kU3Rows + 2 * kU3MaxNodes) * sizeof(float) + (2 * kU3Stages + 2 * NB + 6) * sizeof(uint64_t) + 16;
 }
 
 #ifdef GNF_DEVTOOLS
@@ -880,6 +947,7 @@
   return gnf::fail(GNF_ERR_UNSUPPORTED, "tensor-core kernels have no host-simulator flavour");
 #else
   if (!x || !h || !net || !ccw || !ccn || !z || !jac || R < 0 || d <= 0 || S < 1 || (R % d) != 0) return fail(GNF_ERR_INVALID, "gnf_umnn_fwd_tc3: bad arguments");
+  if (train < 0 || train > 2) return fail(GNF_ERR_INVALID, "gnf_umnn_fwd_tc3: train must be 0, 1 or 2");
   if (train && !saved) return fail(GNF_ERR_INVALID, "gnf_umnn_fwd_tc3: training needs the saved-activation buffer");
   U3Plan pl;
   if (int e = u3_plan(net, R, &pl)) return e;
@@ -893,6 +961,9 @@
   if (R == 0) return 0;
   float* ws = (float*)work;
   const int NP = pl.NP, L = pl.L, E = pl.E;
+  const U3Saved sv = u3_saved_layout(L, NP, Q, R, train);
+  float* M = (saved && train == 2) ? saved + sv.M : nullptr;
+  float* A = (saved && train == 2) ? saved + sv.A : nullptr;
   U3PackArgs a;
   for (int l = 0; l < GNF_MAX_LAYERS; ++l) { a.W[l] = nullptr; a.b[l] = nullptr; a.nch[l] = pl.nch[l]; a.off_img[l] = (unsigned)pl.off_img[l]; }
   for (int l = 0; l <= L; ++l) { a.W[l] = net->W[l]; a.b[l] = net->b[l]; }
@@ -907,6 +978,8 @@
   zl.add(z, (size_t)R);
   zl.add(zrev, (size_t)R);
   zl.add(logdet, (size_t)(R / d));
+  zl.add(M, (size_t)R * NP);
+  zl.add(A, (size_t)R * NP);
   zero_many(zl, s0);
   float* P = ws + pl.off_P;
   if (int e = gnf_linear_fwd(h, E, net->W[0] + 1, 1 + E, net->b[0], 1, P, NP, R, net->dims[1], E, 0, stream)) return e;
@@ -914,7 +987,10 @@
   U3Params p;
   p.x = x; p.h = h; p.ccw = ccw; p.ccn = ccn; p.P = P; p.image = ws; p.blast = net->b[L];
   p.z = z; p.zrev = zrev; p.jac = jac; p.logdet = logdet; p.saved = saved;
-  p.R = R; p.d = d; p.E = E; p.S = S; p.nodes = nodes; p.L = L; p.N1 = pl.N1; p.train = train; p.order = order ? 1 : 0;
+  p.ysave = saved ? saved + sv.ysave : nullptr;
+  p.bits = (saved && train) ? reinterpret_cast<uint32_t*>(saved + sv.bits) : nullptr;
+  p.M = M; p.A = A;
+  p.R = R; p.d = d; p.E = E; p.S = S; p.nodes = nodes; p.L = L; p.N1 = pl.N1; p.NL = net->dims[L]; p.order = order ? 1 : 0;
   p.Q = Q;
   p.p_smem = ((kU3Rows - 1) / nodes + 2 <= kU3PRows) ? 1 : 0;
   for (int l = 0; l < GNF_MAX_LAYERS; ++l) { p.kp[l] = pl.kp[l]; p.nch[l] = pl.nch[l]; p.off_img[l] = (unsigned)pl.off_img[l]; }
diff --git a/graphical-normalizing-flows_b200/csrc/tc_umnn3.h b/graphical-normalizing-flows_b200/csrc/tc_umnn3.h
--- a/graphical-normalizing-flows_b200/csrc/tc_umnn3.h
+++ b/graphical-normalizing-flows_b200/csrc/tc_umnn3.h
@@ -1,12 +1,35 @@
 #pragma once
 #include "common.cuh"
+
+namespace gnf {
+struct U3Saved {
+  int n_planes;
+  size_t ysave, bits, M, A, total;
+};
+static inline U3Saved u3_saved_layout(int L, int NP, long long Q, int R, int train) {
+  U3Saved s;
+  const size_t plane = (size_t)Q * NP;
+  s.n_planes = train == 2 ? L - 1 : L;
+  s.ysave = (size_t)s.n_planes * plane;
+  s.bits = s.ysave + (size_t)Q;
+  const size_t end = s.bits + (train ? (size_t)L * Q * (NP / 32) : 0);
+  s.M = s.A = 0;
+  s.total = end;
+  if (train == 2) {
+    s.M = align_up(end, 4);
+    s.A = s.M + (size_t)R * NP;
+    s.total = s.A + (size_t)R * NP;
+  }
+  return s;
+}
+}
 
 #ifndef GNF_EMU
 namespace gnf {
 size_t u3_bwd_image_floats(const gnf_mlp_t* net);
 int launch_u3_bwd_chain(const float* x, const gnf_mlp_t* net, int S, const float* ccw, const float* ccn, const float* jac, const float* gz,
-                        const float* gzrev, const float* gjac, const float* glogdet, const float* saved, float* image, float* dplanes, float* D,
-                        float* dx, const gnf_mlp_grad_t* grads, int R, int d, cudaStream_t s, const Branches* br = nullptr, int side = 0,
-                        cudaStream_t pack_stream = nullptr);
+                        const float* gzrev, const float* gjac, const float* glogdet, const float* ysave, const uint32_t* bits, float* image,
+                        float* gq, float* dplanes, float* D, float* dx, const gnf_mlp_grad_t* grads, int R, int d, cudaStream_t s,
+                        const Branches* br = nullptr, int side = 0, cudaStream_t pack_stream = nullptr);
 }
 #endif
diff --git a/graphical-normalizing-flows_b200/csrc/umnn_lw.cu b/graphical-normalizing-flows_b200/csrc/umnn_lw.cu
--- a/graphical-normalizing-flows_b200/csrc/umnn_lw.cu
+++ b/graphical-normalizing-flows_b200/csrc/umnn_lw.cu
@@ -134,7 +134,7 @@
 __global__ void lw_out_bwd_kernel(const float* __restrict__ aL, const float* __restrict__ ysave, const float* __restrict__ wl, int NL,
                                   const float* __restrict__ x, const float* __restrict__ ccw, const float* __restrict__ jac,
                                   const float* __restrict__ gz, const float* __restrict__ gzrev, const float* __restrict__ gjac,
-                                  const float* __restrict__ glogdet, float* __restrict__ dL, float* __restrict__ gq_out, float* __restrict__ dWl,
+                                  const float* __restrict__ glogdet, float* __restrict__ dL, float* __restrict__ dWl,
                                   float* __restrict__ dbl, float* __restrict__ dbprev, LwGeom g) {
   GNF_SMEM(float, red);
   const int C4 = g.NP / 4;
@@ -185,8 +185,7 @@
         o[e] = a[e] > 0.f ? gq * w[e] : 0.f;
         sB[e] += o[e];
       }
-      if (gq_out) { if (c4 == 0) gq_out[q + u * kLwRL] = gq; }
-      else *reinterpret_cast<float4*>(dL + (size_t)(q + u * kLwRL) * g.NP + c) = make_float4(o[0], o[1], o[2], o[3]);
+      *reinterpret_cast<float4*>(dL + (size_t)(q + u * kLwRL) * g.NP + c) = make_float4(o[0], o[1], o[2], o[3]);
       if (c4 == 0) sy += gq;
     }
   }
@@ -214,6 +213,37 @@
       }
     }
     __syncthreads();
+  }
+}
+
+__global__ void lw_top_wgrad_kernel(const float* __restrict__ M, const float* __restrict__ A, int NL, const float* __restrict__ x,
+                                    const float* __restrict__ jac, const float* __restrict__ gz, const float* __restrict__ gzrev,
+                                    const float* __restrict__ gjac, const float* __restrict__ glogdet, float* __restrict__ dWl, LwGeom g) {
+  GNF_SMEM(float, red);
+  const int C4 = g.NP / 4;
+  const int c4 = threadIdx.x % C4, rl = threadIdx.x / C4, c = 4 * c4;
+  float sW[4] = {0.f, 0.f, 0.f, 0.f};
+  for (int r = blockIdx.x * kLwRL + rl; r < g.R; r += gridDim.x * kLwRL) {
+    const float al = lw_gz_total(gz, gzrev, r, g.d) * __ldg(x + r) / 2.f;
+    float ge = gjac ? __ldg(gjac + r) : 0.f;
+    if (glogdet) ge += __ldg(glogdet + r / g.d) / __ldg(jac + r);
+    const float4 m = __ldg(reinterpret_cast<const float4*>(M + (size_t)r * g.NP + c));
+    const float4 a = __ldg(reinterpret_cast<const float4*>(A + (size_t)r * g.NP + c));
+    sW[0] = fmaf(ge, a.x, fmaf(al, m.x, sW[0])); sW[1] = fmaf(ge, a.y, fmaf(al, m.y, sW[1]));
+    sW[2] = fmaf(ge, a.z, fmaf(al, m.z, sW[2])); sW[3] = fmaf(ge, a.w, fmaf(al, m.w, sW[3]));
+  }
+#pragma unroll
+  for (int e = 0; e < 4; ++e) red[rl * g.NP + c + e] = sW[e];
+  __syncthreads();
+  if (rl == 0) {
+#pragma unroll
+    for (int e = 0; e < 4; ++e) {
+      if (c + e < NL) {
+        float s = 0.f;
+        for (int k = 0; k < kLwRL; ++k) s += red[k * g.NP + c + e];
+        atomicAdd(dWl + c + e, s);
+      }
+    }
   }
 }
 
@@ -522,7 +552,7 @@
   const float* ysave = saved + (size_t)L * plane;
   const int out_bwd_per_sm = 65536 / (64 * red_threads) < 1 ? 1 : (65536 / (64 * red_threads) > 4 ? 4 : 65536 / (64 * red_threads));
   GNF_LAUNCH(lw_out_bwd_kernel, lw_blocks(pl.Q, 64, out_bwd_per_sm), red_threads, red_smem, s, saved + (size_t)(L - 1) * plane, ysave, net->W[L],
-             net->dims[L], x, ccw, jac, gz, gzrev, gjac, glogdet, dcur, (float*)nullptr, grads->dW[L], grads->db[L], grads->db[L - 1], g);
+             net->dims[L], x, ccw, jac, gz, gzrev, gjac, glogdet, dcur, grads->dW[L], grads->db[L], grads->db[L - 1], g);
   for (int l = L - 1; l >= 1; --l) {
     const float* a_l = saved + (size_t)(l - 1) * plane;
     if (int e = lw_wgrad_gemm(dcur, NP, a_l, NP, grads->dW[l], net->dims[l], (int)pl.Q, net->dims[l + 1], net->dims[l], passes,
@@ -557,7 +587,7 @@
   if (img == 0) return 0;
   if (!pl.rw) { set_error("umnn tc3 backward: the hidden layers do not fit the resident weight-gradient kernel"); return 0; }
   const size_t plane = (size_t)pl.Q * pl.NP;
-  return ((size_t)R * pl.NP + (size_t)(pl.L - 1) * plane + 2 * (rw_wgrad_partial_floats(pl.NP) + 4) + img + 8) * sizeof(float);
+  return ((size_t)R * pl.NP + (size_t)pl.Q + (size_t)(pl.L - 2) * plane + 2 * (rw_wgrad_partial_floats(pl.NP) + 4) + img + 8) * sizeof(float);
 #endif
 }
 
@@ -583,32 +613,33 @@
     zl.add(grads->db[l], (size_t)net->dims[l + 1]);
   }
   if (R == 0) { zero_many(zl, s); return check_launch("gnf_umnn_bwd_tc3"); }
+  const U3Saved sv = u3_saved_layout(L, NP, pl.Q, R, 2);
   float* ws = (float*)work;
   const size_t plane = (size_t)pl.Q * NP;
   float* D = ws;
-  float* dplanes = ws + (((size_t)R * NP + 3) / 4) * 4;
-  float* part = dplanes + (size_t)(L - 1) * plane;
-  const size_t part_floats = ((rw_wgrad_partial_floats(NP) + 3) / 4) * 4;
+  float* gq = ws + align_up((size_t)R * NP, 4);
+  float* dplanes = gq + align_up((size_t)pl.Q, 4);
+  float* part = dplanes + (size_t)(L - 2) * plane;
+  const size_t part_floats = align_up(rw_wgrad_partial_floats(NP), 4);
   float* image = part + 2 * part_floats;
   LwGeom g;
   g.R = R; g.d = d; g.E = E; g.S = S; g.nodes = pl.nodes; g.NP = NP; g.L = L; g.Q = pl.Q;
   const int red_threads = (NP / 4) * kLwRL;
   const size_t red_smem = ((size_t)kLwRL * NP + kLwRL + 4) * sizeof(float);
-  const float* ysave = saved + (size_t)L * plane;
+  const uint32_t* bits = reinterpret_cast<const uint32_t*>(saved + sv.bits);
+  const uint32_t* bits_top = bits + (size_t)(L - 1) * pl.Q * (NP / 32);
   zl.add(D, (size_t)R * NP);
   zl.add(dx, (size_t)R);
   const Branches& br = branches();
   cudaStream_t pack_stream = br.ok ? br.begin(s, 0) : nullptr;
   zero_many(zl, s);
-  float* gq = dplanes;
-  const uint32_t* bits_top = reinterpret_cast<const uint32_t*>(saved + (size_t)L * plane + pl.Q) + (size_t)(L - 1) * pl.Q * (NP / 32);
-  const int out_bwd_per_sm = 65536 / (64 * red_threads) < 1 ? 1 : (65536 / (64 * red_threads) > 4 ? 4 : 65536 / (64 * red_threads));
-  GNF_LAUNCH(lw_out_bwd_kernel, lw_blocks(pl.Q, 64, out_bwd_per_sm), red_threads, red_smem, s, saved + (size_t)(L - 1) * plane, ysave, net->W[L],
-             net->dims[L], x, ccw, jac, gz, gzrev, gjac, glogdet, dplanes, gq, grads->dW[L], grads->db[L], grads->db[L - 1], g);
-  if (int e = launch_u3_bwd_chain(x, net, S, ccw, ccn, jac, gz, gzrev, gjac, glogdet, saved, image, dplanes + plane, D, dx, grads, R, d, s, &br, 0, pack_stream)) return e;
+  if (int e = launch_u3_bwd_chain(x, net, S, ccw, ccn, jac, gz, gzrev, gjac, glogdet, saved + sv.ysave, bits, image, gq, dplanes, D, dx,
+                                  grads, R, d, s, &br, 0, pack_stream)) return e;
   {
     cudaStream_t s0 = br.begin(s, 0);
     gnf_stream_t st0 = (gnf_stream_t)s0;
+    GNF_LAUNCH(lw_top_wgrad_kernel, lw_blocks(R, 4 * kLwRL, 1), red_threads, red_smem, s0, saved + sv.M, saved + sv.A, net->dims[L], x,
+               jac, gz, gzrev, gjac, glogdet, grads->dW[L], g);
     if (int e = gnf_colsum(D, NP, grads->db[0], R, net->dims[1], 1, st0)) return e;
     if (int e = gnf_linear_wgrad(D, NP, h, E, grads->dW[0] + 1, 1 + E, R, net->dims[1], E, st0)) return e;
     if (int e = gnf_linear_dgrad(D, NP, net->W[0] + 1, 1 + E, nullptr, 0, dh, E, R, net->dims[1], E, st0)) return e;
@@ -616,7 +647,7 @@
   }
   int k = 0;
   for (int l = L - 1; l >= 1; --l, ++k) {
-    const float* dnext = dplanes + (size_t)(L - 1 - l) * plane;
+    const float* dnext = l == L - 1 ? nullptr : dplanes + (size_t)(L - 2 - l) * plane;
     const float* a_l = saved + (size_t)(l - 1) * plane;
     if (k >= 2) br.end(s, 1);
     const RwRankOne top = {gq, net->W[L], bits_top, NP / 32};
@@ -629,10 +660,11 @@
 #endif
 }
 
-size_t gnf_umnn_tc3_saved_floats(const gnf_mlp_t* net, int R, int S) {
+size_t gnf_umnn_tc3_saved_floats(const gnf_mlp_t* net, int R, int S, int train) {
+  if (train < 0 || train > 2) { set_error("gnf_umnn_tc3_saved_floats: train must be 0, 1 or 2"); return 0; }
   LwPlan pl;
-  if (lw_plan(net, R, S, 1, 0, &pl)) return 0;
-  return gnf_umnn_lw_saved_floats(net, R, S, 1) + (size_t)pl.Q * (pl.NP / 32);
-}
-
-}
+  if (lw_plan(net, R, S, train, 0, &pl)) return 0;
+  return u3_saved_layout(pl.L, pl.NP, pl.Q, R, train).total;
+}
+
+}
diff --git a/graphical-normalizing-flows_b200/ops.py b/graphical-normalizing-flows_b200/ops.py
--- a/graphical-normalizing-flows_b200/ops.py
+++ b/graphical-normalizing-flows_b200/ops.py
@@ -907,13 +907,16 @@
             _call("gnf_umnn_fwd_tc", ptr(x), ptr(h), C.byref(net), int(S), ptr(ccw), ptr(ccn), ptr(z), ptr(zrev), ptr(jac),
                   ptr(logdet), R, d, ptr(ws), nbytes, stream_ptr())
         elif lw_passes == 3 and UMNN_FWD_FUSED_TC3 and lib().gnf_umnn_tc3_workspace_bytes(C.byref(net), R) != 0:
+            layout = 0
             if train:
-                saved = torch.empty(lib().gnf_umnn_tc3_saved_floats(C.byref(net), R, int(S)), device=x.device, dtype=torch.float32)
                 fused_bwd = lib().gnf_umnn_bwd_tc3_workspace_bytes(C.byref(net), R, int(S)) != 0
+                layout = 2 if fused_bwd else 1
+                saved = torch.empty(lib().gnf_umnn_tc3_saved_floats(C.byref(net), R, int(S), layout), device=x.device,
+                                    dtype=torch.float32)
             nbytes = lib().gnf_umnn_tc3_workspace_bytes(C.byref(net), R)
             ws = torch.empty((nbytes + 3) // 4, device=x.device, dtype=torch.float32)
             _call("gnf_umnn_fwd_tc3", ptr(x), ptr(h), C.byref(net), int(S), ptr(ccw), ptr(ccn), ptr(z), ptr(zrev), ptr(jac),
-                  ptr(logdet), ptr(saved), int(train), int(train), R, d, ptr(ws), nbytes, stream_ptr())
+                  ptr(logdet), ptr(saved), layout, int(train), R, d, ptr(ws), nbytes, stream_ptr())
             _count(6)
         elif lw_passes is not None:
             saved = torch.empty(lib().gnf_umnn_lw_saved_floats(C.byref(net), R, int(S), int(train)), device=x.device,
diff --git a/include/gnf.h b/include/gnf.h
--- a/include/gnf.h
+++ b/include/gnf.h
@@ -166,7 +166,7 @@
                     void* work, size_t work_bytes, gnf_stream_t stream);
 
 size_t gnf_umnn_tc3_workspace_bytes(const gnf_mlp_t* net, int R);
-size_t gnf_umnn_tc3_saved_floats(const gnf_mlp_t* net, int R, int S);
+size_t gnf_umnn_tc3_saved_floats(const gnf_mlp_t* net, int R, int S, int train);
 int gnf_umnn_fwd_tc3(const float* x, const float* h, const gnf_mlp_t* net, int S, const float* ccw, const float* ccn,
                      float* z, float* zrev, float* jac, float* logdet, float* saved, int train, int order, int R, int d,
                      void* work, size_t work_bytes, gnf_stream_t stream);
```

New measurement: 116,600, median of 6. About the same (+1.0%).
